# spaceml-org/STARCOP

Measured on AMD Instinct MI355X. Metric: 512x512 hyperspectral tiles/sec (train fwd+bwd), higher is better.
Workload: dtype f32; 1 GPU; configs[1]: HyperSTARCOP U-Net (smp.Unet mobilenet_v2, 4ch mag1c+RGB) train step fwd+loss+bwd+Adam, 512x512 tiles, fp32 HIP kernels (3x3 convs: fp32 operands split exactly into 16-bit terms on the matrix cores, fp32 accumulation; see config.precision and DESIGN.md section 2); batch_per_gpu=16, global_batch=16, parallelism=dp1, hipgraph=False, precision=fp32

## Files before the change

### include/starcop_hip.h

```cpp
#ifndef STARCOP_HIP_H
#define STARCOP_HIP_H

#include <stddef.h>
#include <stdint.h>

#ifdef __cplusplus
extern "C" {
#endif

typedef void* sc_stream;

enum sc_status {
  SC_OK = 0,
  SC_ERR_ARG = -1,
  SC_ERR_LAUNCH = -2,
  SC_ERR_NOTPD = -3,
  SC_ERR_NODEV = -4
};

enum sc_src_mode {
  SC_SRC_RAW = 0,
  SC_SRC_AFFINE = 1,
  SC_SRC_BNBWD = 2,
  SC_SRC_NORM = 3
// ... 18 lines not shown
const char* sc_last_error(void);
int sc_version(void);
int sc_device_check(void);

int sc_pack_weights(const float* w_oihw, float* wpk, int Cout, int Cin, int ks,
                    int co_t, int transpose_flip, sc_stream stream);
size_t sc_packed_weight_floats(int Cout, int Cin, int ks, int co_t, int transpose_flip);

typedef struct sc_pack_desc {
  const float* w; float* wpk;
  int32_t Cout, Cin, ks, co_t, transpose_flip, bx3;
  uint64_t total;
} sc_pack_desc;
size_t sc_pack_work_items(int Cout, int Cin, int ks, int co_t, int transpose_flip, int bx3);
int sc_pack_weights_batch(const sc_pack_desc* descs_dev, const uint32_t* block_starts_dev, int n, uint32_t total_blocks,
                          sc_stream stream);

typedef struct sc_bnr_args {
  const float* y;
  const float* cst;
  int32_t act;
  float* rows;
  float* absmax;
} sc_bnr_args;
#define SC_TERMS_F16X2 4
typedef struct sc_conv_args {
  sc_src src[2];
  int32_t nsrc;
  const float* wpk;
  int32_t N, H, W;
  int32_t Cout;
  int32_t ks;
  int32_t co_t;
  float* out0; float* out1;
  int32_t csplit;
  int32_t accum0, accum1;
  const float* add0;
  const float* add1;
  float* stats;
  int32_t terms;
  int32_t down0;
  const float* absmax;
  const float* xbound[2];
  const sc_bnr_args* bnr;
} sc_conv_args;
int sc_conv2d_mfma(const sc_conv_args* a, sc_stream stream);
int sc_pw_stream_variant(const sc_conv_args* a);
int sc_conv1x1_ksplit(const sc_conv_args* a, sc_stream stream);

int sc_pack_weights_bx3(const float* w_oihw, float* wpk, int Cout, int Cin, int co_t, int transpose_flip, int terms,
                        sc_stream stream);
size_t sc_packed_weight_floats_bx3(int Cout, int Cin, int co_t, int transpose_flip, int terms);
int sc_conv3x3_bx3(const sc_conv_args* a, sc_stream stream);

typedef struct sc_wgrad_args {
  sc_src dy;
  sc_src src[2];
  int32_t nsrc;
  int32_t N, H, W, Cout, Cin, ks;
  float* part; size_t part_floats;
  float* dw;
  int32_t terms;
  const float* absmax;
  const float* xbound[2];
} sc_wgrad_args;
size_t sc_wgrad_workspace_floats(int N, int H, int W, int Cout, int Cin, int ks);
int sc_conv2d_wgrad_mfma(const sc_wgrad_args* a, sc_stream stream);
typedef struct sc_wgrad_pending {
  const float* part; float* dw;
  int32_t nparts, taps, Cout, Cin, CoP, CiP;
  uint64_t total;
} sc_wgrad_pending;
int sc_conv2d_wgrad_mfma_deferred(const sc_wgrad_args* a, sc_wgrad_pending* pending_host, sc_stream stream);
int sc_wgrad_reduce_batch(const sc_wgrad_pending* descs_dev, const uint32_t* block_starts_dev, int n, uint32_t total_blocks,
                          sc_stream stream);
#define SC_PACK_THIN16 5
#define SC_PACK_PW3 6
size_t sc_packed_weight_floats_thin16(int Cout, int Cin, int transpose_flip);
int sc_pack_weights_thin16(const float* w_oihw, float* wpk, int Cout, int Cin, int transpose_flip, sc_stream stream);
int sc_conv3x3_thin16(const sc_conv_args* a, sc_stream stream);

#define SC_PACK_SP 7
size_t sc_packed_weight_floats_sp(int Cout, int Cup, int Cskip);
int sc_pack_weights_sp(const float* w_oihw, float* wpk, int Cout, int Cup, int Cskip, int terms, sc_stream stream);
int sc_sp_stat_rows(int N, int H, int W, int Cout);
int sc_conv3x3_sp(const sc_conv_args* a, sc_stream stream);
#define SC_PACK_SPD 8
size_t sc_packed_weight_floats_spd(int Cout, int Cup, int Cskip_tiles );
int sc_spd_vskip_ok(int Cup, int Cskip);
int sc_pack_weights_spd(const float* w_oihw, float* wpk, int Cout, int CinTotal, int Cup, int vskip, int terms, sc_stream stream);
int sc_conv3x3_sp_dgrad(const sc_conv_args* a, sc_stream stream);
size_t sc_sp_wgrad_workspace_bytes(int N, int H, int W, int Cout, int Cup);
int sc_conv3x3_sp_wgrad(const sc_wgrad_args* a, void* ws, size_t ws_bytes, sc_stream stream);
int sc_wgrad_scatter_cols(const float* src, float* dw, int Cout, int Ccols, int CinTotal, int col_off, sc_stream stream);
int sc_sp_variant(const sc_conv_args* a);
int sc_spd_variant(const sc_conv_args* a);
int sc_sp_wgrad_variant(const sc_wgrad_args* a);

size_t sc_wgrad_thin16_workspace_floats(int N, int H, int W, int Cout, int Cin);
int sc_conv3x3_wgrad_thin16(const sc_wgrad_args* a, sc_stream stream);

size_t sc_packed_weight_floats_pw3(int Cout, int Cin, int transpose_flip);
int sc_conv1x1_pw3(const sc_conv_args* a, sc_stream stream);
int sc_conv1x1_pw3_variant(int N, int H, int W, int Cout);
size_t sc_wgrad_pw3_workspace_floats(int N, int H, int W, int Cout, int Cin);
int sc_conv1x1_wgrad_pw3(const sc_wgrad_args* a, sc_wgrad_pending* pending_host, sc_stream stream);
int sc_wgrad_pw3_variant(int N, int H, int W, int Cout, int Cin);

typedef struct sc_irb_args {
  sc_src x;
  const float* wpk_expand;
  const float* cst_expand;
  const float* w_dw;
  const float* cst_dw;
  const float* wpk_project;
  const float* cst_project;
  float* out;
  float* z_absmax;
  int32_t N, Cin, hidden, Cout, H, W, stride, residual;
} sc_irb_args;
int sc_irb_supported(int Cin, int hidden, int Cout, int H, int W, int stride);
int sc_irb_variant(int Cin, int hidden, int Cout, int stride);
int sc_irb_eval(const sc_irb_args* a, sc_stream stream);

typedef struct sc_irt_args {
  sc_src x;
  const float* w_expand;
  const float* w_dw;
  const float* cst_expand;
  int32_t N, Cin, hidden, H, W, stride;
} sc_irt_args;
int sc_irt_supported(int Cin, int hidden, int H, int W, int stride);
int sc_irt_rows(int stage, int N, int H, int W, int stride);
int sc_irt_bwd_rows(int N, int hidden, int H, int W);
size_t sc_irt_bwd_workspace_floats(int N, int Cin, int hidden, int H, int W);
#define SC_IRT_GEO_FIELDS 14
int sc_irt_geometry(int N, int Cin, int hidden, int H, int W, int stride, int* out);
int sc_irt_expand_stats(const sc_irt_args* a, float* stats , sc_stream stream);
int sc_irt_fwd(const sc_irt_args* a, float* d_out , float* stats_d , sc_stream stream);
int sc_irt_bwd(const sc_irt_args* a, const sc_src* dy_d, double* e_sums , double* dw_acc ,
               float* work, sc_stream stream);
int sc_irt_xmoments(const sc_irt_args* a, float* work, sc_stream stream);
int sc_irt_bwd_fix(const sc_irt_args* a, const float* cst_bwd_expand, float* work, float* dx, const float* add0, int accum,
                   sc_stream stream);
int sc_irt_wgrad_finalize(const sc_irt_args* a, const float* cst_bwd_expand, float* work, float* dw_expand, sc_stream stream);

size_t sc_wgrad_bx3_workspace_floats(int N, int H, int W, int Cout, int Cin);
int sc_conv3x3_wgrad_bx3(const sc_wgrad_args* a, sc_stream stream);

int sc_conv3_variant(const sc_conv_args* a);
int sc_thin16_variant(const sc_conv_args* a);
int sc_wgrad3_variant(const sc_wgrad_args* a);
int sc_wgrad_thin16_variant(const sc_wgrad_args* a);

int sc_dwconv3x3_fwd(const sc_src* in, const float* w , float* out,
                     int N, int C, int Hin, int Win, int stride, float* stats ,
                     sc_stream stream);
typedef struct sc_bn_tail {
  const float* gamma; const float* beta;
  float* running_mean; float* running_var;
  float momentum, eps;
  float* cst;
  float* act_bound;
  uint32_t* tickets;
} sc_bn_tail;
int sc_dwconv3x3_fwd_bn(const sc_src* in, const float* w, float* out, int N, int C, int Hin, int Win, int stride, float* stats,
                        const sc_bn_tail* bn, sc_stream stream);
int sc_dwconv3x3_dgrad(const sc_src* dy, const float* w, float* dx, int accum,
                       int N, int C, int Hin, int Win, int stride, sc_stream stream);
int sc_dwconv3x3_wgrad(const sc_src* dy, const sc_src* in, double* dw_acc ,
                       int N, int C, int Hin, int Win, int stride, sc_stream stream);
int sc_dwconv3x3_bwd_fused(const sc_src* dy, const sc_src* in, const float* w, float* dx, double* dw_acc, double* in_sums,
                           int N, int C, int Hin, int Win, int stride, sc_stream stream);
int sc_dw_variant(int op, int N, int C, int Hin, int Win, int stride, int aligned16);
int sc_cast_f64_f32(const double* in, float* out, size_t n, sc_stream stream);
typedef struct sc_cast_desc { const double* in; float* out; uint64_t n; } sc_cast_desc;
int sc_cast_f64_f32_batch(const sc_cast_desc* descs_dev, int n_descs, sc_stream stream);

int sc_stem_conv_fwd(const sc_src* in, const float* w , float* out,
                     int N, int Cin, int Hin, int Win, float* stats ,
                     sc_stream stream);
enum sc_stem_kernel { SC_STEM_K_MFMA4 = 0, SC_STEM_K_VALU4 = 1, SC_STEM_K_VALU8 = 2, SC_STEM_K_VALU16 = 3 };
int sc_stem_fwd_kernel(int Cin, int Win, int out_aligned16);
int sc_stem_wgrad_njb(int Cin);
int sc_stem_wgrad_rows(int N, int Hin, int Win);
size_t sc_stem_wgrad_workspace_floats(int N, int Cin, int Hin, int Win);
int sc_stem_conv_wgrad(const sc_src* dy, const sc_src* in, float* part, size_t part_floats,
                       float* dw, int N, int Cin, int Hin, int Win, sc_stream stream);

int sc_head_conv_fwd(const sc_src* in, const float* w , const float* bias,
                     float* out, int N, int Cin, int H, int W, sc_stream stream);
enum sc_head_kernel { SC_HEAD_K_GENERIC = 0, SC_HEAD_K_FWD16 = 1, SC_HEAD_K_FWD16V = 2 };
int sc_head_fwd_kernel(int Cin, int W, int in_aligned16, int out_aligned16);
int sc_head_conv_fwd_k(const sc_src* in, const float* w , const float* bias ,
                       float* logits , uint8_t* classes ,
                       int N, int Cin, int K, int H, int W, sc_stream stream);
int sc_head_conv_dgrad(const float* dlogits, const float* w, float* gin,
                       int N, int Cin, int H, int W, sc_stream stream);
size_t sc_head_wgrad_workspace_floats(int N, int Cin, int H, int W);
int sc_head_conv_wgrad(const float* dlogits, const sc_src* in, float* part, size_t part_floats,
                       float* dw, float* dbias, int N, int Cin, int H, int W, sc_stream stream);
int sc_head_bwd_bn_rows(int N, int H, int W);
int sc_head_conv_bwd(const float* dlogits, const sc_src* in, const float* w, float* gin, float* part, size_t part_floats,
                     float* dw, float* dbias, int N, int Cin, int H, int W, double* bn_sums, float* bn_absmax, sc_stream stream);

int sc_stat_rows(int kind, int N, int H, int W);
#define SC_BN_FINALIZE_SCRATCH_DOUBLES(C) (64 * 2 * (size_t)(C))
int sc_bn_finalize(const float* stats, int nrows, double count, const float* gamma, const float* beta,
                   float* running_mean, float* running_var, float momentum, float eps,
                   int training, float* cst_fwd, int C, double* scratch, float* act_bound, sc_stream stream);
int sc_bn_bwd_reduce(const float* g, const float* y, const float* cst_fwd, int act,
                     double* sums, int N, int C, int HW, float* absmax, float* act_absmax, sc_stream stream);
int sc_bn_bwd_finalize(const double* sums, int nrows, double count, const float* cst_fwd,
                       float* dgamma, float* dbeta, float* cst_bwd, int C, sc_stream stream);
int sc_bn_bwd_finalize_rows32(const float* rows, int nrows, double count, const float* cst_fwd,
                       float* dgamma, float* dbeta, float* cst_bwd, int C, double* scratch , sc_stream stream);
int sc_bn_bwd_small(const float* g, const float* y, const float* cst_fwd, int act, int N, int C, int HW,
                    float* dgamma, float* dbeta, float* cst_bwd, float* absmax, float* act_absmax, sc_stream stream);
int sc_add_srcs(const sc_src* a, const sc_src* b, float* out, int N, int C, int HW, sc_stream stream);
int sc_stream_wait_stream(sc_stream waiter, sc_stream signaller);

int sc_add_srcs_absmax(const sc_src* a, const sc_src* b, float* out, int N, int C, int HW, float* absmax, sc_stream stream);
int sc_downsum2x2(const float* in, float* out, int accum, int N, int C, int Hout, int Wout,
                  sc_stream stream);
int sc_maxpool2x2(const sc_src* in, float* out, int N, int C, int Hout, int Wout, sc_stream stream);
int sc_upsample_bilinear2x(const sc_src* in, float* out, int N, int C, int Hin, int Win, sc_stream stream);
int sc_maxpool2x2_bwd(const sc_src* in, const float* gpool, float* gin, int accum, int N, int C, int Hout, int Wout,
                      sc_stream stream);
int sc_upsample_bilinear2x_bwd(const float* gout, float* gin, int N, int C, int Hin, int Win, sc_stream stream);
int sc_fill_f64(double* p, double v, size_t n, sc_stream stream);
int sc_apply_src(const sc_src* a, float* out, int N, int C, int HW, sc_stream stream);

int sc_bce_logits_weighted(const float* logits, const float* target, const float* weight,
                           float pos_weight, size_t n, double* loss_sum, float* dlogits,
                           float* loss_px, sc_stream stream);

int sc_adam_step(float* param, const float* grad, float* exp_avg, float* exp_avg_sq, size_t n,
                 float lr, float beta1, float beta2, float eps, float weight_decay,
                 float bias_correction1, float bias_correction2_sqrt, float grad_scale,
                 const float* hp_dev ,
                 sc_stream stream);
int sc_adam_prepare(int64_t* step, const float* lr_dev, float beta1, float beta2, float* hp_dev,
                    sc_stream stream);

int sc_threshold_masks(const float* logits, const float* target, int ge0, float* prediction,
                       int64_t* pred_binary, int64_t* differences, int64_t* tile_count,
                       int N, int HW, sc_stream stream);
int sc_pred_classification(const int64_t* tile_count, int64_t* cls, int N, int H, int W,
                           sc_stream stream);

typedef struct sc_mag1c_args {
  const void* x;
  int32_t x_is_f64;
  const int64_t* xoff;
  const int32_t* P;
  const int32_t* Ppad;
  const int64_t* poff;
  const uint8_t* statmask;
  int32_t G, S;
  int64_t npix;
  const double* templ;
  int32_t num_iter;
  double alpha;
  double cov_update_scaling;
  int32_t albedo_override, zero_override, sparse_override, apply_scaling;
// ... 504 lines not shown
```

### starcop_amd/_lib.py

```python
import ctypes as C
import os
import subprocess

import torch

_HERE = os.path.dirname(os.path.abspath(__file__))
LIB_PATH = os.path.join(_HERE, "libstarcop_hip.so")
CSRC = os.path.join(_HERE, "csrc")

SC_CST = 8
STAT_CONV3, STAT_CONV1, STAT_DW, STAT_STEM, STAT_BNBWD, STAT_CONV1K, STAT_PW3 = 0, 1, 2, 3, 4, 5, 6

SRC_RAW, SRC_AFFINE, SRC_BNBWD, SRC_NORM = 0, 1, 2, 3
ACT_NONE, ACT_RELU, ACT_RELU6 = 0, 1, 2


class StarcopHipError(RuntimeError):
    pass


class sc_src(C.Structure):
    _fields_ = [("x", C.c_void_p), ("aux", C.c_void_p), ("cst", C.c_void_p),
                ("C", C.c_int32), ("mode", C.c_int32), ("act", C.c_int32), ("up", C.c_int32)]

# ... 398 lines not shown
    "sc_dw_variant": (_i, [_i, _i, _i, _i, _i, _i, _i]),
    "sc_wgrad_thin16_workspace_floats": (_sz, [_i, _i, _i, _i, _i]),
    "sc_conv3x3_wgrad_thin16": (_i, [C.POINTER(sc_wgrad_args), _vp]),
    "sc_conv2d_wgrad_mfma_deferred": (_i, [C.POINTER(sc_wgrad_args), C.POINTER(sc_wgrad_pending), _vp]),
    "sc_wgrad_reduce_batch": (_i, [_vp, _vp, _i, C.c_uint32, _vp]),
    "sc_packed_weight_floats_pw3": (_sz, [_i, _i, _i]),
    "sc_conv1x1_pw3": (_i, [C.POINTER(sc_conv_args), _vp]),
    "sc_conv1x1_pw3_variant": (_i, [_i, _i, _i, _i]),
    "sc_wgrad_pw3_workspace_floats": (_sz, [_i, _i, _i, _i, _i]),
    "sc_wgrad_pw3_variant": (_i, [_i, _i, _i, _i, _i]),
    "sc_conv1x1_wgrad_pw3": (_i, [C.POINTER(sc_wgrad_args), C.POINTER(sc_wgrad_pending), _vp]),
    "sc_irb_supported": (_i, [_i, _i, _i, _i, _i, _i]),
    "sc_irb_variant": (_i, [_i, _i, _i, _i]),
    "sc_irb_eval": (_i, [C.POINTER(sc_irb_args), _vp]),
    "sc_irt_supported": (_i, [_i, _i, _i, _i, _i]),
    "sc_irt_rows": (_i, [_i, _i, _i, _i, _i]),
    "sc_irt_bwd_rows": (_i, [_i, _i, _i, _i]),
    "sc_irt_bwd_workspace_floats": (_sz, [_i, _i, _i, _i, _i]),
    "sc_irt_geometry": (_i, [_i, _i, _i, _i, _i, _i, C.POINTER(_i)]),
    "sc_irt_expand_stats": (_i, [C.POINTER(sc_irt_args), _vp, _vp]),
    "sc_irt_fwd": (_i, [C.POINTER(sc_irt_args), _vp, _vp, _vp]),
    "sc_irt_bwd": (_i, [C.POINTER(sc_irt_args), C.POINTER(sc_src), _vp, _vp, _vp, _vp]),
    "sc_irt_xmoments": (_i, [C.POINTER(sc_irt_args), _vp, _vp]),
    "sc_irt_bwd_fix": (_i, [C.POINTER(sc_irt_args), _vp, _vp, _vp, _vp, _i, _vp]),
    "sc_irt_wgrad_finalize": (_i, [C.POINTER(sc_irt_args), _vp, _vp, _vp, _vp]),
    "sc_maxpool2x2": (_i, [C.POINTER(sc_src), _vp, _i, _i, _i, _i, _vp]),
    "sc_upsample_bilinear2x": (_i, [C.POINTER(sc_src), _vp, _i, _i, _i, _i, _vp]),
    "sc_maxpool2x2_bwd": (_i, [C.POINTER(sc_src), _vp, _vp, _i, _i, _i, _i, _i, _vp]),
    "sc_upsample_bilinear2x_bwd": (_i, [_vp, _vp, _i, _i, _i, _i, _vp]),
    "sc_pwreg_param_floats": (_sz, [_i, _i, _i, _i]),
    "sc_pwreg_fwd": (_i, [_vp, _vp, _i, _i, _i, _i, _i, _i, _i, _vp, _vp]),
    "sc_reg_loss": (_i, [_vp, _vp, _sz, _i, _vp, _vp, _vp, _vp]),
    "sc_pwreg_sweep_blocks": (_i, [_i, _i, _i]),
    "sc_pwreg_train_sweep": (_i, [_vp, _vp, _vp, _i, _i, _i, _i, _i, _i, _i, _i, _vp, _vp]),
    "sc_pwreg_finalize": (_i, [_vp, _i, _vp, _i, _i, _i, _i, _d, _vp, _vp, _vp]),
    "sc_panel_minmax": (_i, [_vp, C.POINTER(sc_panel), _i, _vp, _vp]),
    "sc_render_panels": (_i, [_vp, C.POINTER(sc_panel), _i, _vp, _vp, _i, _i, _vp]),
    "sc_component_stats_workspace_bytes": (_sz, [_i, _i, _i, _i, _i]),
    "sc_component_stats": (_i, [C.POINTER(sc_cstats_args), _vp, _sz, _vp]),
    "sc_component_outlines_workspace_bytes": (_sz, [_i, _i, C.c_int64]),
    "sc_component_outlines_rounds": (_i, [C.c_int64]),
    "sc_component_outlines": (_i, [C.POINTER(sc_outline_args), _i, _vp]),
    "sc_rasterize_polygons": (_i, [C.POINTER(sc_rast_args), _vp]),
    "sc_overview_reduce": (_i, [C.POINTER(sc_overview_args), _vp]),
    "sc_tiff_tile_flags": (_i, [C.POINTER(sc_cog_image), _i, _vp, _vp]),
    "sc_tiff_pack_tiles": (_i, [C.POINTER(sc_tiff_pack_args), _vp]),
    "sc_edt_workspace_bytes": (_sz, [_i, _i, _i]),
    "sc_edt": (_i, [C.POINTER(sc_edt_args), _vp, _sz, _vp]),
    "sc_edt_call_workspace_bytes": (_sz, [C.POINTER(sc_edt_args)]),
    "sc_edt_variant": (_i, [_i, _i, _i, _i]),
    "sc_label_keep": (_i, [_vp, _vp, _vp, _i, _i, _i, _i, _vp]),
    "sc_tiff_lzw_decode": (_i, [_vp, _sz, _vp, _sz, C.POINTER(C.c_size_t)]),
    "sc_tiff_unpredict": (_i, [_vp, _i, _i, _i, _i, _i, _i, _vp]),
}
REG_L1, REG_MSE, PWREG_G_FROM_MEMORY = 0, 1, 2
PWREG_MAXC, PWREG_PART_DOUBLES, REG_LOSS_PARTS = 16, 273, 256
PACK_SPD = 8
PACK_SP = 7
PACK_PW3 = 6
PACK_THIN16 = 5
TERMS_F16X2 = 4
SE_CROSS = 0xBA

_lib = None


def build(force=False):
    if force:
        subprocess.run(["make", "-C", CSRC, "clean"], check=True, stdout=subprocess.DEVNULL)
    r = subprocess.run(["make", "-C", CSRC, "-j", "4"], capture_output=True, text=True)
    if r.returncode != 0:
        raise StarcopHipError("building libstarcop_hip.so failed:\n" + r.stdout[-4000:] + r.stderr[-4000:])
    return LIB_PATH


def load():
    global _lib
    if _lib is not None:
        return _lib
    path = os.environ.get("STARCOP_HIP_LIB", LIB_PATH)
    if not os.path.exists(path):
        raise StarcopHipError(
            f"{LIB_PATH} is missing: run `python -c 'import __graft_entry__ as g; g.build()'` "
            "(or `make -C starcop_amd/csrc`).  starcop_amd has no CPU/torch fallback.")
    lib = C.CDLL(path)
    for name, (res, args) in SIGNATURES.items():
        fn = getattr(lib, name)
        fn.restype = res
        fn.argtypes = args
    _lib = lib
    return lib


_EXC = {-1: ValueError, -2: RuntimeError, -3: torch.linalg.LinAlgError, -4: RuntimeError}


def check(rc):
    if rc != 0:
        msg = load().sc_last_error().decode("utf-8", "replace")
        raise _EXC.get(rc, StarcopHipError)(f"libstarcop_hip: {msg} (status {rc})")


_device_ok = {}


def require_device(t=None):
# ... 58 lines not shown
```

### starcop_amd/csrc/conv_bx3.hip

```cpp
#include "sc_split.h"
#include "conv_sp_pack.h"
#include <cstdlib>
#include <type_traits>


namespace {

struct ConvXP {
  SrcD s0, s1;
  const uintx4* wpk;
  int N, H, W, Cout;
  float* out0; float* out1;
  int csplit, accum0, accum1;
  const float* add0; const float* add1;
  float* stats;
  int down0;
  const float* absmax;
  const float* xb0; const float* xb1;
  int xcdmap;
  const float* bnr_y; const float* bnr_cst; float* bnr_rows; float* bnr_absmax; int bnr_act;
};

static inline void set_bnr(ConvXP& p, const sc_bnr_args* b) {
  p.bnr_y = b ? b->y : nullptr; p.bnr_cst = b ? b->cst : nullptr; p.bnr_rows = b ? b->rows : nullptr;
  p.bnr_absmax = b ? b->absmax : nullptr; p.bnr_act = b ? b->act : SC_ACT_NONE;
}

__device__ __forceinline__ void wave_absmax_to(float mx, float* slot) {
#pragma unroll
  for (int o = 32; o > 0; o >>= 1) mx = fmaxf(mx, __shfl_xor(mx, o, 64));
  if ((threadIdx.x & 63) == 0 && mx > __builtin_nontemporal_load(slot)) atomicMax(reinterpret_cast<unsigned*>(slot), __builtin_bit_cast(unsigned, mx));
}

template <int Q, bool HF>
__device__ __forceinline__ void bx3_epilogue_bnr(const ConvXP& p, const floatx16 (&acc)[2][Q], float hinv, int n, int cot, int ty, int tx, int y0,
                                                 int x0, int tiles_x, int wave, int l31, int lhi, int tid, float (&s_red)[4][32 * Q][2]) {
  constexpr int CO_T = 32 * Q;
  const int H = p.H, W = p.W, Cs = p.csplit, c0 = cot * CO_T;
  const int ox = x0 + l31;
  const float blo = sc_act_lo(p.bnr_act), bhi = sc_act_hi(p.bnr_act);
  const float* const bc = p.bnr_cst + (size_t)c0 * SC_CST;
  float mx = 0.f;
  if (p.down0) {
    const unsigned hq32 = (unsigned)((H >> 1) * (W >> 1));
    const size_t cbase = ((size_t)n * Cs + c0) * hq32;
    float* const ob = p.out0 + cbase;
    const float* const yb = p.bnr_y + cbase;
    const int oy = y0 + 2 * wave;
    const bool st = !(l31 & 1) && oy < H && ox < W;
    const unsigned loff = (unsigned)(4 * lhi) * hq32 + (unsigned)(st ? (oy >> 1) * (W >> 1) + (ox >> 1) : 0);
#pragma unroll
    for (int q = 0; q < Q; ++q) {
      float yv[16];
#pragma unroll
      for (int r = 0; r < 16; ++r) {
        const int cu = q * 32 + (r & 3) + 8 * (r >> 2);
        yv[r] = (st && c0 + cu + 4 * lhi < Cs) ? yb[loff + (unsigned)cu * hq32] : 0.f;
      }
#pragma unroll
      for (int r = 0; r < 16; ++r) {
        const int cu = q * 32 + (r & 3) + 8 * (r >> 2);
        const int col = cu + 4 * lhi;
        const bool okc = c0 + col < Cs;
        float v = ((oy < H) && (ox < W)) ? acc[0][q][r] : 0.f;
        v += ((oy + 1 < H) && (ox < W)) ? acc[1][q][r] : 0.f;
        if (HF) v *= hinv;
        v += __builtin_bit_cast(float, __builtin_amdgcn_update_dpp(0, __builtin_bit_cast(int, v), 0xB1, 0xF, 0xF, false));
        const bool ok = st && okc;
        if (ok) ob[loff + (unsigned)cu * hq32] = v;
        const float4 cc = *reinterpret_cast<const float4*>(bc + (size_t)(okc ? col : 0) * SC_CST);
        const float yh = fmaf(yv[r], cc.x, cc.y);
        const float gq = (ok && yh > blo && yh < bhi) ? v : 0.f;
// ... 62 lines not shown
    if (co < Cs && t4 < rows4) {
      const size_t row = ((size_t)n * rows4 + t4) * tiles_x + tx;
      p.bnr_rows[(row * Cs + co) * 2 + k] = s_red[2 * hh][col][k] + s_red[2 * hh + 1][col][k];
    }
  }
}

template <int Q, bool BNB, int NT, bool HF = false>
__global__ __launch_bounds__(256, Q == 2 ? 2 : 3) void k_conv3_bx3(const ConvXP p) {
  static_assert(!HF || NT == 2, "the fp16 mode has two terms");
  constexpr int PR = 10, PC = 34, NPX = PR * PC;
  constexpr bool PAD = (Q == 2);
  constexpr int NPXP = PAD ? 384 : NPX;
  constexpr int CO_T = 32 * Q;
  constexpr int WENT = 6 * NT * CO_T;
  constexpr int NWV = (WENT + 255) / 256;
  constexpr int WENTP = PAD ? NWV * 256 : WENT;
  constexpr int NR = 3;
  constexpr bool W2 = (NT != 3) && !(Q == 1 && BNB);

  __shared__ uintx4 s_p[NT][2][NPXP];
  __shared__ uintx4 s_w[2][WENTP];
  __shared__ float s_red[4][CO_T][2];

  const int tid = threadIdx.x;
  const int lane = tid & 63, wave = tid >> 6;
  const int l31 = lane & 31, lhi = lane >> 5;
  const int H = p.H, W = p.W;
  const int tiles_x = (W + 31) >> 5;
  int n, cot, tile;
  if (p.xcdmap) {
    const int ncot = (p.Cout + CO_T - 1) / CO_T;
    const int per_img = tiles_x * ((H + 7) >> 3);
    const int slot = blockIdx.x >> 3, xcd = blockIdx.x & 7;
    int pt;
    if (p.xcdmap == 3) {
      const int total = per_img * p.N;
      if (ncot >= 8) {
        const int mine = (ncot - xcd + 7) >> 3;
        const int k = slot / total;
        if (k >= mine) return;
        cot = xcd + 8 * k; pt = slot - k * total;
      } else {
        const int g = 8 / ncot;
        const int per = (total + g - 1) / g;
        cot = xcd / g; pt = (xcd - cot * g) * per + slot;
        if (slot >= per || pt >= total) return;
      }
      n = pt / per_img; tile = pt - n * per_img;
    } else {
    if (p.xcdmap == 2) {
      const int total = per_img * p.N, per_xcd = (total + 7) >> 3;
      const int j = slot / ncot;
      pt = xcd * per_xcd + j;
      if (j >= per_xcd || pt >= total) return;
    } else {
      pt = (slot / ncot) * 8 + xcd;
      if (pt >= per_img * p.N) return;
    }
    cot = slot % ncot;
    n = pt / per_img; tile = pt - n * per_img;
    }
  } else {
    n = blockIdx.z; cot = blockIdx.y; tile = blockIdx.x;
  }
  n = __builtin_amdgcn_readfirstlane(n); cot = __builtin_amdgcn_readfirstlane(cot); tile = __builtin_amdgcn_readfirstlane(tile);
  const int ty = __builtin_amdgcn_readfirstlane(tile / tiles_x), tx = tile - ty * tiles_x;
  const int y0 = ty * 8, x0 = tx * 32;
  const int C0 = p.s0.C;
  const int Cin = C0 + p.s1.C;
  const int nk = (Cin + 15) >> 4;
  const uintx4* wbase = p.wpk + (size_t)cot * nk * 3 * WENT;

  const float hsx = !HF ? 1.f : (BNB ? h_grad_scale(p.absmax) : h_act_scale(p.xb0, p.xb1));
  const float hinv = !HF ? 1.f : 1.f / (hsx * SC_H_SW);

  floatx16 acc[2][Q];
#pragma unroll
  for (int pp = 0; pp < 2; ++pp)
#pragma unroll
    for (int q = 0; q < Q; ++q)
#pragma unroll
      for (int r = 0; r < 16; ++r) acc[pp][q][r] = 0.f;

  const int hw = __builtin_amdgcn_readfirstlane(wave >> 1);
  const int sidx = tid & 127;
  unsigned off0[NR], off1[NR];
  unsigned inb = 0;
  {
    const int up0 = p.s0.up, up1 = p.s1.up;
    const int Ws0 = W >> up0, Ws1 = W >> up1;
#pragma unroll
    for (int r = 0; r < NR; ++r) {
      const int e = sidx + 128 * r;
      const int pr = e / PC, pc = e - pr * PC;
      const int y = y0 - 1 + pr, x = x0 - 1 + pc;
      const bool ok = (e < NPX) && (y >= 0) && (y < H) && (x >= 0) && (x < W);
      off0[r] = ok ? (unsigned)((y >> up0) * Ws0 + (x >> up0)) : 0u;
      off1[r] = ok ? (unsigned)((y >> up1) * Ws1 + (x >> up1)) : 0u;
      inb |= ok ? (1u << r) : 0u;
    }
  }
  float xv[NR][8], av[BNB ? NR : 1][8];
  uintx4 wvA[NWV], wvB[W2 ? NWV : 1];
  const float* xb = nullptr; const float* ab = nullptr; const float* cb = nullptr;
  size_t plane = 0; int nch = 0; bool second = false;
  float slo = 0.f, shi = 0.f;
// ... 410 lines not shown
      }
    }
  }
}

template <int Q, bool BNB>
__global__ __launch_bounds__(512, 4) void k_conv3_ws(const ConvXP p) {
  constexpr int NT = 2;
  constexpr bool HF = true;
  constexpr int PR = 10, PC = 34, NPX = PR * PC;
  constexpr int NPXP = NPX;
  constexpr int CO_T = 32 * Q;
  constexpr int WENT = 6 * NT * CO_T;
  constexpr int NWV = (WENT + 255) / 256;
  constexpr int WENTP = NWV * 256;
  constexpr int NR = 3;

  __shared__ uintx4 s_p[2][NT][2][NPXP];
  __shared__ uintx4 s_w[2][WENTP];
  __shared__ float s_red[4][CO_T][2];
  constexpr int WS_BNB_MAXC = 256;
  __shared__ __attribute__((aligned(16))) float s_cst[BNB ? WS_BNB_MAXC * SC_CST : 4];

  const int role = __builtin_amdgcn_readfirstlane((int)threadIdx.x >> 8);
  const int tid = threadIdx.x & 255;
  const int lane = tid & 63, wave = tid >> 6;
  const int l31 = lane & 31, lhi = lane >> 5;
  const int H = p.H, W = p.W;
  const int tiles_x = (W + 31) >> 5;
  int n, cot, tile;
  if (p.xcdmap) {
    const int ncot = (p.Cout + CO_T - 1) / CO_T;
    const int per_img = tiles_x * ((H + 7) >> 3);
    const int slot = blockIdx.x >> 3, xcd = blockIdx.x & 7;
    int pt;
    if (p.xcdmap == 3) {
      const int total = per_img * p.N;
      if (ncot >= 8) {
        const int mine = (ncot - xcd + 7) >> 3;
        const int k = slot / total;
        if (k >= mine) return;
        cot = xcd + 8 * k; pt = slot - k * total;
      } else {
        const int g = 8 / ncot;
        const int per = (total + g - 1) / g;
        cot = xcd / g; pt = (xcd - cot * g) * per + slot;
        if (slot >= per || pt >= total) return;
      }
      n = pt / per_img; tile = pt - n * per_img;
    } else {
    if (p.xcdmap == 2) {
      const int total = per_img * p.N, per_xcd = (total + 7) >> 3;
      const int j = slot / ncot;
      pt = xcd * per_xcd + j;
      if (j >= per_xcd || pt >= total) return;
    } else {
      pt = (slot / ncot) * 8 + xcd;
      if (pt >= per_img * p.N) return;
    }
    cot = slot % ncot;
    n = pt / per_img; tile = pt - n * per_img;
    }
  } else {
    n = blockIdx.z; cot = blockIdx.y; tile = blockIdx.x;
  }
  n = __builtin_amdgcn_readfirstlane(n); cot = __builtin_amdgcn_readfirstlane(cot); tile = __builtin_amdgcn_readfirstlane(tile);
  const int ty = __builtin_amdgcn_readfirstlane(tile / tiles_x), tx = tile - ty * tiles_x;
  const int y0 = ty * 8, x0 = tx * 32;
  const int C0 = p.s0.C;
  const int Cin = C0 + p.s1.C;
  const int nk = (Cin + 15) >> 4;
  const uintx4* wbase = p.wpk + (size_t)cot * nk * 3 * WENT;

  const float hsx = !HF ? 1.f : (BNB ? h_grad_scale(p.absmax) : h_act_scale(p.xb0, p.xb1));
  const float hinv = !HF ? 1.f : 1.f / (hsx * SC_H_SW);

  const int nst = 3 * nk;
  const bool want_stats = p.stats != nullptr;
  if constexpr (BNB) {
    for (int i = (int)threadIdx.x; i < p.s0.C * SC_CST; i += 512) {
      const int f = i & (SC_CST - 1);
      s_cst[i] = p.s0.cst[i] * ((HF && f >= 2 && f <= 4) ? hsx : 1.f);
    }
    __syncthreads();
  }
  if (role == 1) {
  const int hw = __builtin_amdgcn_readfirstlane(wave >> 1);
  const int sidx = tid & 127;
  unsigned off0[NR], off1[NR];
  unsigned inb = 0;
  {
    const int up0 = p.s0.up, up1 = p.s1.up;
    const int Ws0 = W >> up0, Ws1 = W >> up1;
#pragma unroll
    for (int r = 0; r < NR; ++r) {
      const int e = sidx + 128 * r;
      const int pr = e / PC, pc = e - pr * PC;
      const int y = y0 - 1 + pr, x = x0 - 1 + pc;
      const bool ok = (e < NPX) && (y >= 0) && (y < H) && (x >= 0) && (x < W);
      off0[r] = ok ? (unsigned)((y >> up0) * Ws0 + (x >> up0)) : 0u;
      off1[r] = ok ? (unsigned)((y >> up1) * Ws1 + (x >> up1)) : 0u;
      inb |= ok ? (1u << r) : 0u;
    }
  }
  float xv[NR][8], av[BNB ? NR : 1][8];
  uintx4 wr[3][NWV];
  struct Chunk { const float* xb; const float* ab; const float* cb; size_t plane; int nch, cbase; bool second, raw; float slo, shi; };
// ... 306 lines not shown
    }
  }

  if (want_stats) {
    __syncthreads();
    const int rows4 = (H + 3) >> 2;
    for (int i = tid; i < 2 * CO_T * 2; i += 256) {
      const int hh = i / (CO_T * 2), rem = i - hh * (CO_T * 2);
      const int col = rem >> 1, k = rem & 1;
      const int co = cot * CO_T + col;
      const int t4 = 2 * ty + hh;
      if (co < p.Cout && t4 < rows4) {
        const float t = s_red[2 * hh][col][k] + s_red[2 * hh + 1][col][k];
        const size_t row = ((size_t)n * rows4 + t4) * tiles_x + tx;
        p.stats[(row * p.Cout + co) * 2 + k] = t;
      }
    }
  }
}

__device__ __forceinline__ void split_filter(float v, bool half, unsigned short (&t)[3]) {
  if (half) {
    const float vs = __builtin_amdgcn_fmed3f(v * SC_H_SW, -SC_H_MAX, SC_H_MAX);
    const _Float16 h0 = (_Float16)vs;
    const _Float16 h1 = (_Float16)(vs - (float)h0);
    t[0] = __builtin_bit_cast(unsigned short, h0); t[1] = __builtin_bit_cast(unsigned short, h1); t[2] = 0;
    return;
  }
  const __bf16 t0 = (__bf16)v;
  float rr = v - (float)t0;
  const __bf16 t1 = (__bf16)rr;
  rr -= (float)t1;
  const __bf16 t2 = (__bf16)rr;
  t[0] = __builtin_bit_cast(unsigned short, t0); t[1] = __builtin_bit_cast(unsigned short, t1); t[2] = __builtin_bit_cast(unsigned short, t2);
}

template <int CIN, bool BNB, bool UPS = false>
__global__ __launch_bounds__(256, 2) void k_conv3_thin_h(const ConvXP p) {
  constexpr int TW = CIN == 16 ? 64 : 32, PBW = TW / 16, NPB = 2 * PBW;
  constexpr int PR = UPS ? 6 : 10, PC = UPS ? TW / 2 + 2 : TW + 2, NPX = PR * PC;
  constexpr int NH = CIN / 8;
  constexpr int NG = 9 * NH, NS = (NG + 3) / 4;
  constexpr int NPXP = (NPX + 15) & ~15;
  __shared__ uintx4 s_p[2][NH][NPXP];
  __shared__ float s_red[4][TW / 32][16][2];

  const int tid = threadIdx.x, lane = tid & 63, wave = tid >> 6;
  const int l15 = lane & 15, lg = lane >> 4;
  const int H = p.H, W = p.W;
  const int tiles_x = (W + TW - 1) / TW;
  int n, tile;
  if (p.xcdmap) {
    const int per_img = tiles_x * ((H + 7) >> 3), total = per_img * p.N, per_xcd = (total + 7) >> 3;
    const int j = blockIdx.x >> 3, pt = (blockIdx.x & 7) * per_xcd + j;
    if (j >= per_xcd || pt >= total) return;
    n = pt / per_img; tile = pt - n * per_img;
  } else {
    n = blockIdx.z; tile = blockIdx.x;
  }
  n = __builtin_amdgcn_readfirstlane(n); tile = __builtin_amdgcn_readfirstlane(tile);
  const int ty = __builtin_amdgcn_readfirstlane(tile / tiles_x), tx = tile - ty * tiles_x;
  const int y0 = ty * 8, x0 = tx * TW;
  const float hsx = BNB ? h_grad_scale(p.absmax) : h_act_scale(p.xb0, p.xb1);
  const float hinv = 1.f / (hsx * SC_H_SW);

  const SrcD& src = p.s0;
  uintx4 A[NS][2];
#pragma unroll
  for (int s = 0; s < NS; ++s)
#pragma unroll
    for (int t = 0; t < 2; ++t) A[s][t] = p.wpk[(s * 2 + t) * 64 + lane];

  constexpr int WPG = 4 / NH, TPG = 64 * WPG, NR = (NPX + TPG - 1) / TPG;
  const int grp = __builtin_amdgcn_readfirstlane(wave / WPG);
  const int g8 = grp * 8;
  const int e0 = tid - grp * TPG;
  const int up = UPS ? 1 : src.up;
  const int Ws = W >> up;
  const size_t plane = (size_t)(H >> up) * Ws;
  const float slo = BNB ? sc_act_lo(src.act) : h_lo(sc_act_lo(src.act), hsx), shi = BNB ? sc_act_hi(src.act) : h_hi(sc_act_hi(src.act), hsx);
  float xv[NR][8], av[BNB ? NR : 1][8];
  bool okv[NR];
  const float* const xg = src.x + ((size_t)n * CIN + g8) * plane;
  const float* const ag = BNB ? src.aux + ((size_t)n * CIN + g8) * plane : nullptr;
#pragma unroll
  for (int r = 0; r < NR; ++r) {
    const int e = e0 + TPG * r;
    const int pr = e / PC, pc = e - pr * PC;
    const int y = UPS ? (y0 >> 1) - 1 + pr : y0 - 1 + pr, x = UPS ? (x0 >> 1) - 1 + pc : x0 - 1 + pc;
    const bool ok = UPS ? ((e < NPX) && y >= 0 && y < (H >> 1) && x >= 0 && x < Ws) : ((e < NPX) && y >= 0 && y < H && x >= 0 && x < W);
    okv[r] = ok;
    const unsigned off = ok ? (UPS ? (unsigned)(y * Ws + x) : (unsigned)((y >> up) * Ws + (x >> up))) : 0u;
#pragma unroll
    for (int j = 0; j < 8; ++j) {
      xv[r][j] = xg[(size_t)j * plane + off];
      if (BNB) av[r][j] = ag[(size_t)j * plane + off];
    }
  }
  __builtin_amdgcn_sched_barrier(0);
  float4 cc[8]; float c4[8];
#pragma unroll
  for (int j = 0; j < 8; ++j) { cc[j] = make_float4(BNB ? 1.f : hsx, 0.f, 0.f, 0.f); c4[j] = 0.f; }
  if (src.mode != SC_SRC_RAW) {
#pragma unroll
    for (int j = 0; j < 8; ++j) {
      cc[j] = *reinterpret_cast<const float4*>(src.cst + (size_t)(g8 + j) * SC_CST);
      if (BNB) c4[j] = src.cst[(size_t)(g8 + j) * SC_CST + 4];
// ... 106 lines not shown
        }
      }
      return;
    }
  }
#pragma unroll
  for (int r = 0; r < 4; ++r) {
    const int co = 4 * lg + r;
    float sv[TW / 32], sq[TW / 32];
#pragma unroll
    for (int h = 0; h < TW / 32; ++h) { sv[h] = 0.f; sq[h] = 0.f; }
#pragma unroll
    for (int pb = 0; pb < NPB; ++pb) {
      const int oy = y0 + 2 * wave + pb / PBW, ox = x0 + 16 * (pb % PBW) + l15;
      const bool ok = oy < H && ox < W && co < p.Cout;
      const float v = ok ? acc[pb][r] * hinv : 0.f;
      sv[(pb % PBW) >> 1] += v; sq[(pb % PBW) >> 1] = fmaf(v, v, sq[(pb % PBW) >> 1]);
      if (ok) *reinterpret_cast<float*>(reinterpret_cast<char*>(outn) + ((unsigned)co * HWu + (unsigned)(oy * W + ox)) * 4u) = v;
    }
    if (want_stats) {
#pragma unroll
      for (int h = 0; h < TW / 32; ++h) {
#pragma unroll
        for (int o = 8; o > 0; o >>= 1) { sv[h] += __shfl_xor(sv[h], o, 64); sq[h] += __shfl_xor(sq[h], o, 64); }
        if (l15 == 0) { s_red[wave][h][co][0] = sv[h]; s_red[wave][h][co][1] = sq[h]; }
      }
    }
  }
  if (want_stats) {
    __syncthreads();
    const int rows4 = (H + 3) >> 2, tiles32 = (W + 31) >> 5;
    if (tid < 2 * (TW / 32) * 16 * 2) {
      const int hh = tid / ((TW / 32) * 32), h = (tid >> 5) % (TW / 32), col = (tid >> 1) & 15, k = tid & 1;
      const int t4 = 2 * ty + hh, t32 = tx * (TW / 32) + h;
      if (col < p.Cout && t4 < rows4 && t32 < tiles32) {
        const size_t row = ((size_t)n * rows4 + t4) * tiles32 + t32;
        p.stats[(row * p.Cout + col) * 2 + k] = s_red[2 * hh][h][col][k] + s_red[2 * hh + 1][h][col][k];
      }
    }
  }
}

__global__ __launch_bounds__(256, 2) void k_conv3_thin_sp(const ConvXP p) {
  constexpr int PC = 34, NPX = 6 * PC, NPXP = (NPX + 15) & ~15, NH = 4, NR = (NPX + 63) / 64, STEPS3 = 9;
  __shared__ uintx4 s_p[2][NH][NPXP];
  __shared__ float s_red[4][2][16][2];
  const int tid = threadIdx.x, lane = tid & 63, wave = tid >> 6;
  const int l15 = lane & 15, lg = lane >> 4;
  const int H = p.H, W = p.W, Hs = H >> 1, Ws = W >> 1;
  const int tiles_x = (W + 63) >> 6;
  int n, tile;
  if (p.xcdmap) {
    const int per_img = tiles_x * ((H + 7) >> 3), total = per_img * p.N, per_xcd = (total + 7) >> 3;
    const int j = blockIdx.x >> 3, pt = (blockIdx.x & 7) * per_xcd + j;
    if (j >= per_xcd || pt >= total) return;
    n = pt / per_img; tile = pt - n * per_img;
  } else {
    n = blockIdx.z; tile = blockIdx.x;
  }
  n = __builtin_amdgcn_readfirstlane(n); tile = __builtin_amdgcn_readfirstlane(tile);
  const int ty = __builtin_amdgcn_readfirstlane(tile / tiles_x), tx = tile - ty * tiles_x;
  const int y0 = ty * 8, x0 = tx * 64;
  const float hsx = h_act_scale(p.xb0, p.xb1);
  const float hinv = 1.f / (hsx * SC_H_SW);
  const SrcD& src = p.s0;

  const int g8 = wave * 8;
  const size_t plane = (size_t)Hs * Ws;
  const float slo = h_lo(sc_act_lo(src.act), hsx), shi = h_hi(sc_act_hi(src.act), hsx);
  float xv[NR][8];
  bool okv[NR];
  const float* const xg = src.x + ((size_t)n * 32 + g8) * plane;
#pragma unroll
  for (int r = 0; r < NR; ++r) {
    const int e = lane + 64 * r;
    const int pr = e / PC, pc = e - pr * PC;
    const int y = (y0 >> 1) - 1 + pr, x = (x0 >> 1) - 1 + pc;
    const bool ok = (e < NPX) && y >= 0 && y < Hs && x >= 0 && x < Ws;
    okv[r] = ok;
    const unsigned off = ok ? (unsigned)(y * Ws + x) : 0u;
#pragma unroll
    for (int j = 0; j < 8; ++j) xv[r][j] = xg[(size_t)j * plane + off];
  }
  __builtin_amdgcn_sched_barrier(0);
  float2 cc[8];
#pragma unroll
  for (int j = 0; j < 8; ++j) cc[j] = make_float2(hsx, 0.f);
  if (src.mode != SC_SRC_RAW) {
#pragma unroll
    for (int j = 0; j < 8; ++j) {
      cc[j] = *reinterpret_cast<const float2*>(src.cst + (size_t)(g8 + j) * SC_CST);
      cc[j].x *= hsx; cc[j].y *= hsx;
    }
  }
#pragma unroll
  for (int r = 0; r < NR; ++r) {
    const int e = lane + 64 * r;
    uintx4 t0, t1;
#pragma unroll
    for (int jp = 0; jp < 4; ++jp) {
      const float v0 = okv[r] ? sc_pro_affine_h(xv[r][2 * jp], cc[2 * jp].x, cc[2 * jp].y, slo, shi) : 0.f;
      const float v1 = okv[r] ? sc_pro_affine_h(xv[r][2 * jp + 1], cc[2 * jp + 1].x, cc[2 * jp + 1].y, slo, shi) : 0.f;
      unsigned a0, a1;
      split2h<false>(v0, v1, a0, a1);
      t0[jp] = a0; t1[jp] = a1;
    }
    if (e < NPX) { s_p[0][wave][e] = t0; s_p[1][wave][e] = t1; }
// ... 37 lines not shown
        }
      }

  const size_t HWs = (size_t)H * W;
  const bool want_stats = p.stats != nullptr;
  float* const outn = p.out0 + (size_t)n * p.Cout * HWs;
  const unsigned HWu = (unsigned)HWs;
#pragma unroll
  for (int r = 0; r < 4; ++r) {
    const int co = 4 * lg + r;
#pragma unroll
    for (int q = 0; q < 2; ++q) {
      float sv = 0.f, sq = 0.f;
      const int ox = x0 + 32 * q + 2 * l15;
#pragma unroll
      for (int py = 0; py < 2; ++py) {
        const int oy = y0 + 2 * wave + py;
        const bool ok = oy < H && ox < W && co < p.Cout;
        const float v0 = ok ? acc[q][2 * py][r] * hinv : 0.f, v1 = ok ? acc[q][2 * py + 1][r] * hinv : 0.f;
        sv += v0 + v1; sq = fmaf(v0, v0, fmaf(v1, v1, sq));
        if (ok) *reinterpret_cast<float2*>(reinterpret_cast<char*>(outn) + ((unsigned)co * HWu + (unsigned)(oy * W + ox)) * 4u) = make_float2(v0, v1);
      }
      if (want_stats) {
        sv = row_sum16(sv); sq = row_sum16(sq);
        if (l15 == 0) { s_red[wave][q][co][0] = sv; s_red[wave][q][co][1] = sq; }
      }
    }
  }
  if (want_stats) {
    __syncthreads();
    const int rows4 = (H + 3) >> 2, tiles32 = (W + 31) >> 5;
    if (tid < 2 * 2 * 16 * 2) {
      const int hh = tid / 64, h = (tid >> 5) & 1, col = (tid >> 1) & 15, k = tid & 1;
      const int t4 = 2 * ty + hh, t32 = 2 * tx + h;
      if (col < p.Cout && t4 < rows4 && t32 < tiles32) {
        const size_t row = ((size_t)n * rows4 + t4) * tiles32 + t32;
        p.stats[(row * p.Cout + col) * 2 + k] = s_red[2 * hh][h][col][k] + s_red[2 * hh + 1][h][col][k];
      }
    }
  }
}

__global__ __launch_bounds__(256, 2) void k_conv3_thin_spd(const ConvXP p) {
  constexpr int PR = 10, PC = 66, NPX = PR * PC, PCH = 34, NPL = PR * PCH, NPLP = (NPL + 15) & ~15;
  constexpr int TPG = 128, NR = (NPX + TPG - 1) / TPG;
  __shared__ uintx4 s_p[2][2][2][NPLP];
  const int tid = threadIdx.x, lane = tid & 63, wave = tid >> 6;
  const int l15 = lane & 15, lg = lane >> 4;
  const int H = p.H, W = p.W, Hs = H >> 1, Ws = W >> 1;
  const int tiles_x = (W + 63) >> 6;
  int n, tile;
  if (p.xcdmap) {
    const int per_img = tiles_x * ((H + 7) >> 3), total = per_img * p.N, per_xcd = (total + 7) >> 3;
    const int j = blockIdx.x >> 3, pt = (blockIdx.x & 7) * per_xcd + j;
    if (j >= per_xcd || pt >= total) return;
    n = pt / per_img; tile = pt - n * per_img;
  } else {
    n = blockIdx.z; tile = blockIdx.x;
  }
  n = __builtin_amdgcn_readfirstlane(n); tile = __builtin_amdgcn_readfirstlane(tile);
  const int ty = __builtin_amdgcn_readfirstlane(tile / tiles_x), tx = tile - ty * tiles_x;
  const int y0 = ty * 8, x0 = tx * 64;
  const float hsx = h_grad_scale(p.absmax);
  const float hinv = 1.f / (hsx * SC_H_SW);
  const SrcD& src = p.s0;

  const int grp = __builtin_amdgcn_readfirstlane(wave >> 1);
  const int g8 = grp * 8;
  const int e0 = tid - grp * TPG;
  const size_t plane = (size_t)H * W;
  const float slo = sc_act_lo(src.act), shi = sc_act_hi(src.act);
  float xv[NR][8], av[NR][8];
  bool okv[NR];
  const float* const xg = src.x + ((size_t)n * 16 + g8) * plane;
  const float* const ag = src.aux + ((size_t)n * 16 + g8) * plane;
#pragma unroll
  for (int r = 0; r < NR; ++r) {
    const int e = e0 + TPG * r;
    const int pr = e / PC, pc = e - pr * PC;
    const int y = y0 - 1 + pr, x = x0 - 1 + pc;
    const bool ok = (e < NPX) && y >= 0 && y < H && x >= 0 && x < W;
    okv[r] = ok;
    const unsigned off = ok ? (unsigned)(y * W + x) : 0u;
#pragma unroll
    for (int j = 0; j < 8; ++j) { xv[r][j] = xg[(size_t)j * plane + off]; av[r][j] = ag[(size_t)j * plane + off]; }
  }
  __builtin_amdgcn_sched_barrier(0);
  float4 cc[8]; float c4[8];
#pragma unroll
  for (int j = 0; j < 8; ++j) {
    cc[j] = *reinterpret_cast<const float4*>(src.cst + (size_t)(g8 + j) * SC_CST);
    c4[j] = src.cst[(size_t)(g8 + j) * SC_CST + 4];
  }
#pragma unroll
  for (int r = 0; r < NR; ++r) {
    const int e = e0 + TPG * r;
    const int pr = e / PC, pc = e - pr * PC;
    uintx4 t0, t1;
#pragma unroll
    for (int jp = 0; jp < 4; ++jp) {
      float v[2];
#pragma unroll
      for (int h = 0; h < 2; ++h) {
        const int j = 2 * jp + h;
        const float t = sc_pro_bnbwd(xv[r][j], av[r][j], cc[j].x, cc[j].y, cc[j].z, cc[j].w, c4[j], slo, shi);
        v[h] = okv[r] ? t * hsx : 0.f;
      }
// ... 907 lines not shown
  const int blocks = (int)((total + 255) / 256 > 4096 ? 4096 : (total + 255) / 256);
  hipLaunchKernelGGL(k_pack_weights_bx3, dim3(blocks), dim3(256), 0, (hipStream_t)stream, w,
                     reinterpret_cast<unsigned short*>(wpk), Cout, Cin, co_t, transpose_flip, nchunk,
                     terms == SC_TERMS_F16X2 ? 2 : terms, terms == SC_TERMS_F16X2 ? 1 : 0, total);
  SC_LAUNCH_OK("sc_pack_weights_bx3");
  return SC_OK;
}

static int conv3_bx3_check(const sc_conv_args* a) {
  SC_REQUIRE(a != nullptr, "sc_conv3x3_bx3: null args");
  SC_REQUIRE(a->ks == 3, "sc_conv3x3_bx3: ks must be 3 (got %d)", a->ks);
  SC_REQUIRE(a->co_t == 32 || a->co_t == 64, "sc_conv3x3_bx3: co_t must be 32 or 64 (got %d)", a->co_t);
  SC_REQUIRE(a->nsrc == 1 || a->nsrc == 2, "sc_conv3x3_bx3: nsrc must be 1 or 2");
  const int C0 = a->src[0].C, C1 = a->nsrc == 2 ? a->src[1].C : 0;
  SC_REQUIRE(C0 > 0 && C1 >= 0 && (a->nsrc == 1 || (C0 % 16 == 0 && C1 > 0)),
             "sc_conv3x3_bx3: a concat needs the first source's channels to be a multiple of 16 (got %d,%d)", C0, C1);
  SC_REQUIRE(a->N > 0 && a->H > 0 && a->W > 0 && a->Cout > 0, "sc_conv3x3_bx3: bad shape");
  SC_REQUIRE(a->csplit > 0 && a->csplit <= a->Cout, "sc_conv3x3_bx3: bad csplit");
  SC_REQUIRE(a->csplit == a->Cout || (a->add0 == nullptr && a->add1 == nullptr), "sc_conv3x3_bx3: add tensors need a single output");
  SC_REQUIRE(((uintptr_t)a->wpk & 15) == 0, "sc_conv3x3_bx3: packed filters must be 16-byte aligned");
  for (int s = 0; s < a->nsrc; ++s) {
    SC_REQUIRE(a->src[s].up == 0 || (a->H % 2 == 0 && a->W % 2 == 0), "sc_conv3x3_bx3: upsampled source needs even H,W");
    SC_REQUIRE(a->src[s].up == 0 || a->src[s].up == 1, "sc_conv3x3_bx3: up must be 0 or 1");
    SC_REQUIRE(a->src[s].mode == SC_SRC_RAW || a->src[s].cst != nullptr, "sc_conv3x3_bx3: source %d needs constants", s);
    SC_REQUIRE(a->src[s].mode != SC_SRC_NORM, "sc_conv3x3_bx3: NORM sources are the stem's");
    SC_REQUIRE(a->src[s].mode != SC_SRC_BNBWD || a->src[s].aux != nullptr, "sc_conv3x3_bx3: BNBWD source needs aux");
    SC_REQUIRE(a->src[s].mode != SC_SRC_BNBWD || a->nsrc == 1, "sc_conv3x3_bx3: a BNBWD source cannot be part of a concat");
  }
  SC_REQUIRE(!a->down0 || (a->H % 2 == 0 && a->W % 2 == 0 && a->stats == nullptr && a->add0 == nullptr && a->add1 == nullptr),
             "sc_conv3x3_bx3: down0 (2x2-summed half-resolution out0) needs even H, W and no stats/add tensors");
  SC_REQUIRE(a->terms >= 0 && a->terms <= 4, "sc_conv3x3_bx3: terms must be 0 (= 3), 1, 2, 3 or SC_TERMS_F16X2 (got %d)", a->terms);
  if (a->bnr) {
    SC_REQUIRE(a->src[0].mode == SC_SRC_BNBWD && a->bnr->y && a->bnr->cst && a->bnr->rows, "sc_conv3x3_bx3: bnr needs a BNBWD source and y / cst / rows");
    SC_REQUIRE(!a->accum0 && !a->add0 && !a->add1 && !a->stats, "sc_conv3x3_bx3: bnr: out0 must receive the complete gradient (no accum0 / add / stats)");
    SC_REQUIRE(a->csplit == a->Cout || a->csplit % a->co_t == 0, "sc_conv3x3_bx3: bnr: csplit must fall on a cout-tile boundary");
  }
  return SC_OK;
}

static int conv3_bx3_variant_of(const sc_conv_args* a) {
  const int C0 = a->src[0].C, C1 = a->nsrc == 2 ? a->src[1].C : 0;
  const int bnb = a->src[0].mode == SC_SRC_BNBWD ? 1 : 0;
  const int m = a->terms == SC_TERMS_F16X2 ? 4 : (a->terms == 1 || a->terms == 2 ? a->terms : 3);
  constexpr int ws_env = 1;
  static const int ws_env_min = [] { const char* e = getenv("STARCOP_BX3_WS_MINCHUNKS"); return e ? atoi(e) : 16; }();
  const int ws = (m == 4 && ws_env && (C0 + C1 + 15) / 16 >= ws_env_min && (!bnb || a->src[0].C <= 256) && !a->bnr) ? 1 : 0;
  return 1000 * ws + 100 * (a->co_t / 32) + 10 * bnb + m;
}

extern "C" int sc_conv3_variant(const sc_conv_args* a) {
  return conv3_bx3_check(a) == SC_OK ? conv3_bx3_variant_of(a) : -1;
}

extern "C" int sc_conv3x3_bx3(const sc_conv_args* a, sc_stream stream) {
  if (const int rc = conv3_bx3_check(a)) return rc;
  const int C0 = a->src[0].C, C1 = a->nsrc == 2 ? a->src[1].C : 0;
  ConvXP p;
  p.s0 = to_srcd(a->src[0]);
  p.s1 = a->nsrc == 2 ? to_srcd(a->src[1]) : empty_srcd();
  p.wpk = reinterpret_cast<const uintx4*>(a->wpk); p.N = a->N; p.H = a->H; p.W = a->W; p.Cout = a->Cout;
  p.out0 = a->out0; p.out1 = a->out1; p.csplit = a->csplit; p.accum0 = a->accum0; p.accum1 = a->accum1;
  p.add0 = a->add0; p.add1 = a->add1; p.stats = a->stats;
  p.down0 = a->down0 ? 1 : 0;
  const int co_tiles = (a->Cout + a->co_t - 1) / a->co_t;
  dim3 grid(((a->W + 31) / 32) * ((a->H + 7) / 8), co_tiles, a->N);
  constexpr int xcdmap_env = 2;
  p.xcdmap = xcdmap_env >= 2 ? 2 : ((xcdmap_env && co_tiles > 1) ? 1 : 0);
  {
    constexpr long big_env = 0L;
    const long nkc = (C0 + C1 + 15) / 16;
    const long wbytes = (long)co_tiles * nkc * 3 * 6 * (a->terms == SC_TERMS_F16X2 || a->terms == 2 ? 2 : (a->terms == 1 ? 1 : 3)) * a->co_t * 16;
    if (xcdmap_env >= 2 && big_env > 0 && wbytes > big_env && (co_tiles >= 8 || co_tiles == 1 || co_tiles == 2 || co_tiles == 4)) p.xcdmap = 3;
  }
  if (p.xcdmap == 3) {
    const long total = (long)grid.x * a->N;
    const long slots = co_tiles >= 8 ? (long)((co_tiles + 7) / 8) * total : (total + (8 / co_tiles) - 1) / (8 / co_tiles);
    SC_REQUIRE(slots * 8 < (1L << 31), "sc_conv3x3_bx3: grid too large");
    grid = dim3((unsigned)(slots * 8));
  } else if (p.xcdmap) {
    const long pt8 = ((long)grid.x * a->N + 7) / 8 * 8;
    SC_REQUIRE(pt8 * co_tiles < (1L << 31), "sc_conv3x3_bx3: grid too large");
    grid = dim3((unsigned)(pt8 * co_tiles));
  }
  hipStream_t st = (hipStream_t)stream;
  p.absmax = a->absmax; p.xb0 = a->xbound[0]; p.xb1 = a->xbound[1];
  set_bnr(p, a->bnr);
#define SC_BX3_CASE(Q, B, M, NT, HF) \
  case 100 * Q + 10 * B + M: hipLaunchKernelGGL((k_conv3_bx3<Q, B != 0, NT, HF>), grid, dim3(256), 0, st, p); break;
#define SC_BX3_CASES(M, NT, HF) SC_BX3_CASE(1, 0, M, NT, HF) SC_BX3_CASE(1, 1, M, NT, HF) SC_BX3_CASE(2, 0, M, NT, HF) SC_BX3_CASE(2, 1, M, NT, HF)
#define SC_BX3_WS_CASE(Q, B) \
  case 1000 + 100 * Q + 10 * B + 4: hipLaunchKernelGGL((k_conv3_ws<Q, B != 0>), grid, dim3(512), 0, st, p); break;
  switch (conv3_bx3_variant_of(a)) {
    SC_BX3_CASES(1, 1, false)
    SC_BX3_CASES(2, 2, false)
    SC_BX3_CASES(3, 3, false)
    SC_BX3_CASES(4, 2, true)
    SC_BX3_WS_CASE(1, 0) SC_BX3_WS_CASE(1, 1) SC_BX3_WS_CASE(2, 0) SC_BX3_WS_CASE(2, 1)
    default: SC_REQUIRE(false, "sc_conv3x3_bx3: no kernel for variant %d", conv3_bx3_variant_of(a));
  }
#undef SC_BX3_WS_CASE
#undef SC_BX3_CASES
#undef SC_BX3_CASE
  SC_LAUNCH_OK("sc_conv3x3_bx3");
  return SC_OK;
}

static bool wgrad3_pipe_reduces(const WgradXPlan& pl) {
  const int npair = pl.nci * pl.wm, cit = 32 * pl.nci, xcp = 8 * 40 + 8;
  return pl.kp == 1 || 3 * npair * 3072 <= 2 * cit * xcp / 2;
}

static size_t wgrad_bx3_workspace_of(const WgradXPlan& pl) {
  const size_t E = (size_t)9 * pl.CoP * pl.CiP;
  const int nparts = pl.nsl * pl.kp;
  return (size_t)nparts * E + sc_reduce_scratch_floats(nparts, E);
}
extern "C" size_t sc_wgrad_bx3_workspace_floats(int N, int H, int W, int Cout, int Cin) {
  const size_t a = wgrad_bx3_workspace_of(plan_wgrad_bx3(N, H, W, Cout, Cin, false));
  const size_t b = wgrad_bx3_workspace_of(plan_wgrad_bx3(N, H, W, Cout, Cin, true));
  return a > b ? a : b;
}

static int wgrad3_bx3_check(const sc_wgrad_args* a) {
  SC_REQUIRE(a != nullptr, "sc_conv3x3_wgrad_bx3: null args");
  SC_REQUIRE(a->ks == 3, "sc_conv3x3_wgrad_bx3: ks must be 3");
  SC_REQUIRE(a->nsrc == 1 || a->nsrc == 2, "sc_conv3x3_wgrad_bx3: nsrc must be 1 or 2");
// ... 141 lines not shown
  SC_REQUIRE(w && wpk && ((uintptr_t)wpk & 15) == 0, "sc_pack_weights_thin16: bad pointer");
  SC_REQUIRE(thin16_shape_ok(Cout, Cin, transpose_flip), "sc_pack_weights_thin16: needs <= 16 output and 16 or 32 input channels (got %d, %d, flip %d)",
             Cout, Cin, transpose_flip);
  const size_t total = (size_t)thin_steps(Cout, Cin, transpose_flip) * 512;
  hipLaunchKernelGGL(k_pack_weights_thin, dim3((unsigned)((total + 255) / 256)), dim3(256), 0, (hipStream_t)stream, w,
                     reinterpret_cast<unsigned short*>(wpk), Cout, Cin, transpose_flip, total);
  SC_LAUNCH_OK("sc_pack_weights_thin16");
  return SC_OK;
}

static int thin16_check(const sc_conv_args* a) {
  SC_REQUIRE(a != nullptr && a->ks == 3 && a->nsrc == 1, "sc_conv3x3_thin16: one source, ks = 3");
  const int Cin = a->src[0].C;
  const sc_src& s = a->src[0];
  if (a->down0) {
    SC_REQUIRE(Cin == 16 && a->Cout == 32 && a->csplit == 32 && s.mode == SC_SRC_BNBWD && s.aux && s.cst && s.up == 0,
               "sc_conv3x3_thin16(down0): needs a 16-channel BatchNorm-backward source and 32 output channels (got %d, %d)", Cin, a->Cout);
    SC_REQUIRE(a->H % 2 == 0 && a->W % 2 == 0 && a->N > 0 && a->N <= 65535 && a->out0 && !a->add0 && !a->add1 && !a->stats && !a->bnr && !a->out1,
               "sc_conv3x3_thin16(down0): even H, W; one output, no add / statistics / bnr epilogue");
    SC_REQUIRE(a->terms == SC_TERMS_F16X2 && ((uintptr_t)a->wpk & 15) == 0, "sc_conv3x3_thin16(down0): terms must be SC_TERMS_F16X2, filters 16-byte aligned");
    SC_REQUIRE((size_t)16 * a->H * a->W < ((size_t)1 << 30), "sc_conv3x3_thin16(down0): one image of the gradient must stay below 2^30 elements");
    return SC_OK;
  }
  SC_REQUIRE(a->Cout >= 1 && a->Cout <= 16 && (Cin == 16 || Cin == 32), "sc_conv3x3_thin16: needs <= 16 output and 16 or 32 input channels (got %d, %d)",
             a->Cout, Cin);
  SC_REQUIRE(a->N > 0 && a->N <= 65535 && a->H > 0 && a->W > 0, "sc_conv3x3_thin16: bad shape");
  SC_REQUIRE(a->csplit == a->Cout && !a->accum0 && !a->add0 && !a->add1 && !a->down0 && a->out0,
             "sc_conv3x3_thin16: a single plain output only (no split / add / accumulate / down-sum epilogue)");
  SC_REQUIRE(a->terms == SC_TERMS_F16X2, "sc_conv3x3_thin16: terms must be SC_TERMS_F16X2");
  SC_REQUIRE(((uintptr_t)a->wpk & 15) == 0, "sc_conv3x3_thin16: packed filters must be 16-byte aligned");
  SC_REQUIRE(s.up == 0 || (s.up == 1 && a->H % 2 == 0 && a->W % 2 == 0), "sc_conv3x3_thin16: upsampled source needs even H, W");
  SC_REQUIRE(s.mode == SC_SRC_RAW || s.cst != nullptr, "sc_conv3x3_thin16: source needs constants");
  SC_REQUIRE(s.mode != SC_SRC_NORM && (s.mode != SC_SRC_BNBWD || s.aux != nullptr), "sc_conv3x3_thin16: unsupported source");
  SC_REQUIRE((size_t)a->Cout * a->H * a->W < ((size_t)1 << 30), "sc_conv3x3_thin16: one image of the output must stay below 2^30 elements");
  SC_REQUIRE(!a->bnr || (s.mode == SC_SRC_BNBWD && a->bnr->y && a->bnr->cst && a->bnr->rows && !a->stats),
             "sc_conv3x3_thin16: bnr needs a BNBWD source, y / cst / rows and no stats");
  return SC_OK;
}

static int thin16_variant_of(const sc_conv_args* a) {
  const sc_src& s = a->src[0];
  if (a->down0) return 2110;
  static const bool sp_off = [] { const char* e = getenv("STARCOP_THIN_SP"); return e && atoi(e) == 0; }();
  static const bool ups_off = [] { const char* e = getenv("STARCOP_THIN_UPS"); return e && atoi(e) == 0; }();
  const bool bnb = s.mode == SC_SRC_BNBWD;
  if (s.C == 32 && s.up == 1 && !bnb && !sp_off) return 1200;
  return 100 * (s.C / 16) + 10 * (bnb ? 1 : 0) + (s.C == 32 && s.up == 1 && !bnb && !ups_off ? 1 : 0);
}

extern "C" int sc_thin16_variant(const sc_conv_args* a) {
  return thin16_check(a) == SC_OK ? thin16_variant_of(a) : -1;
}

extern "C" int sc_conv3x3_thin16(const sc_conv_args* a, sc_stream stream) {
  if (const int rc = thin16_check(a)) return rc;
  const int Cin = a->src[0].C;
  const sc_src& s = a->src[0];
  const int variant = thin16_variant_of(a);
  if (variant == 2110) {
    ConvXP p{};
    p.s0 = to_srcd(s); p.s1 = empty_srcd();
    p.wpk = reinterpret_cast<const uintx4*>(a->wpk); p.N = a->N; p.H = a->H; p.W = a->W; p.Cout = a->Cout;
    p.out0 = a->out0; p.csplit = a->Cout; p.accum0 = a->accum0; p.absmax = a->absmax;
    set_bnr(p, nullptr);
    const long total = (long)((a->W + 63) / 64) * ((a->H + 7) / 8) * a->N, per_xcd = (total + 7) / 8;
    p.xcdmap = 2;
    hipLaunchKernelGGL(k_conv3_thin_spd, dim3((unsigned)(per_xcd * 8)), dim3(256), 0, (hipStream_t)stream, p);
    SC_LAUNCH_OK("sc_conv3x3_thin16(down0)");
    return SC_OK;
  }
  ConvXP p{};
  p.s0 = to_srcd(s); p.s1 = empty_srcd();
  p.wpk = reinterpret_cast<const uintx4*>(a->wpk); p.N = a->N; p.H = a->H; p.W = a->W; p.Cout = a->Cout;
  p.out0 = a->out0; p.csplit = a->Cout; p.stats = a->stats; p.absmax = a->absmax; p.xb0 = a->xbound[0]; p.xb1 = a->xbound[1];
  set_bnr(p, a->bnr);
  const int tw = (Cin == 16 || variant == 1200) ? 64 : 32;
  dim3 grid(((a->W + tw - 1) / tw) * ((a->H + 7) / 8), 1, a->N);
  constexpr int xcdmap_env = 2;
  p.xcdmap = xcdmap_env ? 2 : 0;
  if (p.xcdmap) {
    const long total = (long)grid.x * a->N, per_xcd = (total + 7) / 8;
    grid = dim3((unsigned)(per_xcd * 8));
  }
  hipStream_t st = (hipStream_t)stream;
  switch (variant) {
    case 1200: hipLaunchKernelGGL(k_conv3_thin_sp, grid, dim3(256), 0, st, p); break;
    case 100: hipLaunchKernelGGL((k_conv3_thin_h<16, false>), grid, dim3(256), 0, st, p); break;
    case 110: hipLaunchKernelGGL((k_conv3_thin_h<16, true>), grid, dim3(256), 0, st, p); break;
    case 201: hipLaunchKernelGGL((k_conv3_thin_h<32, false, true>), grid, dim3(256), 0, st, p); break;
    case 200: hipLaunchKernelGGL((k_conv3_thin_h<32, false>), grid, dim3(256), 0, st, p); break;
    case 210: hipLaunchKernelGGL((k_conv3_thin_h<32, true>), grid, dim3(256), 0, st, p); break;
    default: SC_REQUIRE(false, "sc_conv3x3_thin16: no kernel for variant %d", variant);
  }
  SC_LAUNCH_OK("sc_conv3x3_thin16");
  return SC_OK;
}

extern "C" size_t sc_pack_work_items(int Cout, int Cin, int ks, int co_t, int transpose_flip, int bx3) {
  if (bx3 == SC_PACK_THIN16) return (size_t)thin_steps(Cout, Cin, transpose_flip) * 512;
  if (bx3 == SC_PACK_SPD) return spd_pack_items(Cout, co_t, (transpose_flip & 3) == 3 ? Cin - co_t : 0);
  if (bx3 == SC_PACK_SP) return sp_pack_items(Cout, co_t, Cin - co_t);
  if (bx3 == SC_PACK_PW3) {
    const int M = transpose_flip ? Cin : Cout, K = transpose_flip ? Cout : Cin;
    return (size_t)(((M + 31) / 32 + 3) / 4 * 4) * ((K + 15) / 16) * 512;
  }
  if (bx3) {
    const int M = transpose_flip ? Cin : Cout, K = transpose_flip ? Cout : Cin;
    return (size_t)((M + co_t - 1) / co_t) * ((K + 15) / 16) * 9 * 2 * co_t * 8;
  }
  return sc_packed_weight_floats(Cout, Cin, ks, co_t, transpose_flip);
}

extern "C" int sc_pack_weights_batch(const sc_pack_desc* descs_dev, const uint32_t* block_starts_dev, int n, uint32_t total_blocks,
                                     sc_stream stream) {
  SC_REQUIRE(descs_dev && block_starts_dev && n > 0 && total_blocks > 0, "sc_pack_weights_batch: bad argument");
  hipLaunchKernelGGL(k_pack_batch, dim3(total_blocks), dim3(256), 0, (hipStream_t)stream,
                     reinterpret_cast<const PackDesc*>(descs_dev), block_starts_dev, n);
  SC_LAUNCH_OK("sc_pack_weights_batch");
  return SC_OK;
}
```

### starcop_amd/csrc/conv_sp.hip

```cpp
#include "sc_split.h"
#include "conv_sp_pack.h"
#include <cstdlib>
#include <type_traits>

namespace {

#ifndef SP_INTERLEAVE
#define SP_INTERLEAVE 4
#endif

struct ConvSPP {
  SrcD s0, s1;
  const uintx4* wpk;
  int N, Hl, Wl, Cout;
  float* out;
  float* stats;
  const float* xb0; const float* xb1;
};

constexpr int SP_SMEM_W = 2 * SP_WST * 16;
#ifndef SP_PC16
#define SP_PC16 18
#endif
template <int TW> constexpr int sp_pc() { return TW == 16 ? SP_PC16 : TW + 2; }
template <int TW> constexpr int sp_npx() { return (256 / TW + 2) * sp_pc<TW>(); }
template <int TW> constexpr int sp_smem_bytes() { return SP_SMEM_W + 2 * 2 * 2 * sp_npx<TW>() * 16 + 8 * 32 * 2 * 4; }

template <int TW, bool BF, int NPP = 2>
__global__ __launch_bounds__(512, 2) void k_conv3_sp(const ConvSPP p) {
  static_assert(NPP == 1 || NPP == 2, "one or two pixel groups per wave");
  constexpr int NT = BF ? 1 : 2;
  constexpr int NM = BF ? 4 : 12;
  constexpr int TH = 128 * NPP / TW;
  constexpr int PC = sp_pc<TW>(), NPX = sp_npx<TW>();
  constexpr int NPXU = (TH + 2) * PC;
  constexpr int NR = (NPXU + 127) / 128;
  constexpr int WST = SP_WST / 2 * NT;
  constexpr int NWV = WST / 512;
  static_assert(NPXU <= NPX && NPXU <= 128 * NR, "staging rounds of 128 threads per channel quarter");

  extern __shared__ __attribute__((aligned(16))) unsigned char smem[];
  uintx4* const s_w = reinterpret_cast<uintx4*>(smem);
  uintx4* const s_p = reinterpret_cast<uintx4*>(smem + SP_SMEM_W);
  float* const s_red = reinterpret_cast<float*>(smem + SP_SMEM_W + 2 * NT * 2 * NPX * 16);

  const int tid = threadIdx.x;
  const int lane = tid & 63, wave = __builtin_amdgcn_readfirstlane(tid >> 6);
  const int l31 = lane & 31, lhi = lane >> 5;
  const int py = wave >> 2, wq = wave & 3;
  const int Hl = p.Hl, Wl = p.Wl;
  const int tiles_x = (Wl + TW - 1) / TW, tiles_y = (Hl + TH - 1) / TH;
  const int ncot = (p.Cout + 31) >> 5;
  int n, cot, tile;
  {
    const int per_img = tiles_x * tiles_y;
    const int total = per_img * p.N, per_xcd = (total + 7) >> 3;
    const int slot = blockIdx.x >> 3, xcd = blockIdx.x & 7;
    const int j = slot / ncot;
    const int pt = xcd * per_xcd + j;
    if (j >= per_xcd || pt >= total) return;
    cot = slot - j * ncot;
    n = pt / per_img; tile = pt - n * per_img;
  }
  n = __builtin_amdgcn_readfirstlane(n); cot = __builtin_amdgcn_readfirstlane(cot); tile = __builtin_amdgcn_readfirstlane(tile);
  const int ty = __builtin_amdgcn_readfirstlane(tile / tiles_x), tx = tile - ty * tiles_x;
  const int y0 = ty * TH, x0 = tx * TW;
  const int C0 = p.s0.C, C1 = p.s1.C;
  const int nku = (C0 + 15) >> 4, nkt = nku + 4 * ((C1 + 15) >> 4);
  const uintx4* wbase = p.wpk + (size_t)cot * nkt * WST;

  const float hsx = BF ? 1.f : h_act_scale(p.xb0, p.xb1);
  const float hinv = BF ? 1.f : 1.f / (hsx * SP_SW);

  floatx16 acc[NPP][2];
#pragma unroll
  for (int i = 0; i < 2 * NPP; ++i)
#pragma unroll
    for (int r = 0; r < 16; ++r) acc[i >> 1][i & 1][r] = 0.f;

  const int q4 = __builtin_amdgcn_readfirstlane(tid >> 7);
  const int hw = q4 >> 1, sub = q4 & 1;
  const int sidx = tid & 127;
  unsigned pyx[NR];
#pragma unroll
  for (int r = 0; r < NR; ++r) {
    const int e = sidx + 128 * r;
    const int pr = e / PC, pc = e - pr * PC;
    const int y = y0 - 1 + pr, x = x0 - 1 + pc;
    const bool ok = (e < NPXU) && (y >= 0) && (y < Hl) && (x >= 0) && (x < Wl);
    pyx[r] = ok ? ((unsigned)y << 16) | (unsigned)x : 0xFFFFFFFFu;
  }
  float xv[NR][4];
  uintx4 wv[NWV];
  float cs0[4], cs1[4];
  float slo = 0.f, shi = 0.f;
  int nch = 0;

  auto request = [&](int kc) __attribute__((always_inline)) {
    const uintx4* wsrc = wbase + (size_t)kc * WST;
#pragma unroll
    for (int j = 0; j < NWV; ++j) wv[j] = wsrc[tid + 512 * j];
    const bool second = kc >= nku;
    const int c4 = kc - nku;
    const SrcD& s = second ? p.s1 : p.s0;
    const int cbase = (second ? (c4 >> 2) : kc) * 16 + hw * 8 + sub * 4;
    const size_t plane = second ? (size_t)4 * Hl * Wl : (size_t)Hl * Wl;
    const unsigned qoff = second ? (unsigned)(((c4 >> 1) & 1) * 2 * Wl + (c4 & 1)) : 0u;
    nch = s.C - cbase;
    const int cb0 = nch > 0 ? cbase : 0;
    const float* xb = s.x + ((size_t)n * s.C + cb0) * plane;
    const int jmax = nch > 0 ? nch - 1 : 0;
#pragma unroll
// ... 149 lines not shown
#pragma unroll
  for (int pp = 0; pp < NPP; ++pp) {
    const int g = NPP * wq + pp;
    const int i = y0 + (TW == 32 ? g : 2 * g + (l31 >> 4)), j = x0 + (TW == 32 ? l31 : (l31 & 15));
    okp[pp] = i < Hl && j < Wl;
    loff[pp] = (unsigned)(4 * lhi) * hw32 + (unsigned)(okp[pp] ? (2 * i + py) * W + 2 * j : 0);
  }
#pragma unroll
  for (int r = 0; r < 16; ++r) {
    const int cu = (r & 3) + 8 * (r >> 2);
    const int col = cu + 4 * lhi;
    const bool okc = cot * 32 + col < p.Cout;
    float sv = 0.f, sq = 0.f;
#pragma unroll
    for (int pp = 0; pp < NPP; ++pp) {
      floatx2 v = {acc[pp][0][r] * hinv, acc[pp][1][r] * hinv};
      if (okp[pp] && okc) *reinterpret_cast<floatx2*>(ob + loff[pp] + (unsigned)cu * hw32) = v;
      else v = floatx2{0.f, 0.f};
      sv += v[0] + v[1];
      sq = fmaf(v[0], v[0], fmaf(v[1], v[1], sq));
    }
    if (want_stats) {
      const float s = half_sum32(sv);
      const float ss = half_sum32(sq);
      if (l31 == SC_HALF_SUM_LANE) { s_red[(wave * 32 + col) * 2 + 0] = s; s_red[(wave * 32 + col) * 2 + 1] = ss; }
    }
  }
  if (want_stats) {
    __syncthreads();
    if (tid < 64) {
      const int col = tid >> 1, k = tid & 1;
      const int co = cot * 32 + col;
      if (co < p.Cout) {
        float t = 0.f;
#pragma unroll
        for (int w8 = 0; w8 < 8; ++w8) t += s_red[(w8 * 32 + col) * 2 + k];
        const size_t row = (size_t)n * (tiles_x * tiles_y) + tile;
        p.stats[(row * p.Cout + co) * 2 + k] = t;
      }
    }
  }
}

struct ConvSPD {
  SrcD dy;
  const uintx4* wpk;
  int N, Hl, Wl, Cup;
  float* out;
  int accum;
  const float* absmax;
  float* out_skip;
  int Cskip, accum_skip;
  int skip_mode, ntu, nts;
};

template <int TW, bool BF, int NPP = 2>
__global__ __launch_bounds__(512, 2) void k_conv3_spd(const ConvSPD p) {
  static_assert(NPP == 1 || NPP == 2, "one or two pixel groups per wave (see k_conv3_sp)");
  constexpr int NT = BF ? 1 : 2;
  constexpr int NM = BF ? 4 : 12;
  constexpr int TH = 128 * NPP / TW;
  constexpr int PC = sp_pc<TW>(), NPX = sp_npx<TW>();
  constexpr int NPXU = (TH + 2) * PC;
  constexpr int NR = (NPXU + 127) / 128;
  static_assert(NPXU <= NPX && (NPP == 2 || NR == 2), "staging rounds");
  constexpr int WST = SP_WST / 2 * NT;
  constexpr int NWV = WST / 512;

  extern __shared__ __attribute__((aligned(16))) unsigned char smem[];
  uintx4* const s_w = reinterpret_cast<uintx4*>(smem);
  uintx4* const s_p = reinterpret_cast<uintx4*>(smem + SP_SMEM_W);

  const int tid = threadIdx.x;
  const int lane = tid & 63, wave = __builtin_amdgcn_readfirstlane(tid >> 6);
  const int l31 = lane & 31, lhi = lane >> 5;
  const int hh = wave >> 2, wq = wave & 3;
  const int Hl = p.Hl, Wl = p.Wl;
  const int tiles_x = (Wl + TW - 1) / TW, tiles_y = (Hl + TH - 1) / TH;
  const int ncot = p.ntu + p.nts;
  int n, cot, tile;
  {
    const int per_img = tiles_x * tiles_y;
    const int total = per_img * p.N, per_xcd = (total + 7) >> 3;
    const int slot = blockIdx.x >> 3, xcd = blockIdx.x & 7;
    const int j = slot / ncot;
    const int pt = xcd * per_xcd + j;
    if (j >= per_xcd || pt >= total) return;
    cot = slot - j * ncot;
    n = pt / per_img; tile = pt - n * per_img;
  }
  n = __builtin_amdgcn_readfirstlane(n); cot = __builtin_amdgcn_readfirstlane(cot); tile = __builtin_amdgcn_readfirstlane(tile);
  const int ty = __builtin_amdgcn_readfirstlane(tile / tiles_x), tx = tile - ty * tiles_x;
  const int y0 = ty * TH, x0 = tx * TW;
  const int Co = p.dy.C;
  const int nkt = 4 * ((Co + 15) >> 4);
  const uintx4* wbase = p.wpk + (size_t)cot * nkt * WST;

  const float hsx = BF ? 1.f : h_grad_scale(p.absmax);
  const float hinv = BF ? 1.f : 1.f / (hsx * SP_SW);

  floatx16 acc[NPP][2];
#pragma unroll
  for (int i = 0; i < 2 * NPP; ++i)
#pragma unroll
    for (int r = 0; r < 16; ++r) acc[i >> 1][i & 1][r] = 0.f;

  const int q4 = __builtin_amdgcn_readfirstlane(tid >> 7);
  const int hw = q4 >> 1, sub = q4 & 1;
  const int sidx = tid & 127;
  unsigned pyx[NR];
#pragma unroll
  for (int r = 0; r < NR; ++r) {
    const int e = sidx + 128 * r;
    const int pr = e / PC, pc = e - pr * PC;
    const int y = y0 - 1 + pr, x = x0 - 1 + pc;
    const bool ok = (e < NPXU) && (y >= 0) && (y < Hl) && (x >= 0) && (x < Wl);
    pyx[r] = ok ? ((unsigned)y << 16) | (unsigned)x : 0xFFFFFFFFu;
  }
  float xv[NR][4], av[NR][4];
  uintx4 wv[NWV];
  float cs0[4], cs1[4], cs2[4], cs3[4], cs4[4];
  const float slo = sc_act_lo(p.dy.act), shi = sc_act_hi(p.dy.act);
  int nch = 0;
  const size_t plane = (size_t)4 * Hl * Wl;

  auto request = [&](int kc) __attribute__((always_inline)) {
    const uintx4* wsrc = wbase + (size_t)kc * WST;
#pragma unroll
    for (int j = 0; j < NWV; ++j) wv[j] = wsrc[tid + 512 * j];
    const int cbase = (kc >> 2) * 16 + hw * 8 + sub * 4;
    const unsigned qoff = (unsigned)(((kc >> 1) & 1) * 2 * Wl + (kc & 1));
    nch = Co - cbase;
    const int cb0 = nch > 0 ? cbase : 0;
    const size_t o0 = ((size_t)n * Co + cb0) * plane;
    const float* xb = p.dy.x + o0;
    const float* ab = p.dy.aux + o0;
    const int jmax = nch > 0 ? nch - 1 : 0;
#pragma unroll
    for (int r = 0; r < NR; ++r) {
// ... 232 lines not shown
                     reinterpret_cast<unsigned short*>(wpk), Cout, Cup, Cskip, terms == 1 ? 1 : 0, total);
  SC_LAUNCH_OK("sc_pack_weights_sp");
  return SC_OK;
}

static inline int sp_groups_per_wave(int N, int Hl, int Wl, int ctiles) {
  const long wgs2 = Wl >= 32 ? (long)N * ((Wl + 31) / 32) * ((Hl + 7) / 8) * ctiles : (long)N * ((Wl + 15) / 16) * ((Hl + 15) / 16) * ctiles;
  static const int force = [] { const char* e = getenv("STARCOP_SP_NPP"); return e ? atoi(e) : 0; }();
  if (force == 1 || force == 2) return force;
  return wgs2 <= 128 ? 1 : 2;
}

extern "C" int sc_sp_stat_rows(int N, int H, int W, int Cout) {
  const int Hl = H / 2, Wl = W / 2;
  const int TW = Wl >= 32 ? 32 : 16, TH = 128 * sp_groups_per_wave(N, Hl, Wl, (Cout + 31) / 32) / TW;
  return N * ((Wl + TW - 1) / TW) * ((Hl + TH - 1) / TH);
}

static int conv3_sp_check(const sc_conv_args* a) {
  SC_REQUIRE(a != nullptr, "sc_conv3x3_sp: null args");
  SC_REQUIRE(a->ks == 3 && (a->nsrc == 1 || a->nsrc == 2), "sc_conv3x3_sp: ks = 3, one (up-sampled) or two (up-sampled, skip) sources");
  SC_REQUIRE(a->src[0].up == 1, "sc_conv3x3_sp: src[0] must be the half-resolution tensor (up = 1)");
  SC_REQUIRE(a->nsrc == 1 || a->src[1].up == 0, "sc_conv3x3_sp: src[1] is the full-resolution skip tensor (up = 0)");
  for (int s = 0; s < a->nsrc; ++s) {
    SC_REQUIRE(a->src[s].mode == SC_SRC_RAW || a->src[s].mode == SC_SRC_AFFINE, "sc_conv3x3_sp: RAW or AFFINE sources");
    SC_REQUIRE(a->src[s].mode == SC_SRC_RAW || a->src[s].cst != nullptr, "sc_conv3x3_sp: source %d needs constants", s);
    SC_REQUIRE(a->src[s].C > 0, "sc_conv3x3_sp: source %d has no channels", s);
  }
  SC_REQUIRE(a->N > 0 && a->H > 0 && a->W > 0 && a->Cout > 0, "sc_conv3x3_sp: bad shape");
  SC_REQUIRE(a->H % 2 == 0 && a->W % 2 == 0, "sc_conv3x3_sp: even output size");
  SC_REQUIRE(a->terms == SC_TERMS_F16X2 || a->terms == 1, "sc_conv3x3_sp: terms = SC_TERMS_F16X2 (two fp16 terms) or 1 (one bf16 term)");
  SC_REQUIRE(a->csplit == a->Cout && a->out1 == nullptr && a->add0 == nullptr && a->add1 == nullptr && !a->down0 && !a->accum0,
             "sc_conv3x3_sp: a single plain output");
  SC_REQUIRE(((uintptr_t)a->wpk & 15) == 0 && ((uintptr_t)a->out0 & 7) == 0, "sc_conv3x3_sp: alignment");
  SC_REQUIRE((size_t)32 * a->H * a->W < (1ull << 32), "sc_conv3x3_sp: plane too large");
  return SC_OK;
}

static int sp_variant_code(int N, int Hl, int Wl, int ctiles, int terms) {
  return 100 * (Wl >= 32 ? 2 : 1) + 10 * sp_groups_per_wave(N, Hl, Wl, ctiles) + (terms == 1 ? 1 : 4);
}
static int conv3_sp_variant_of(const sc_conv_args* a) { return sp_variant_code(a->N, a->H / 2, a->W / 2, (a->Cout + 31) / 32, a->terms); }

extern "C" int sc_sp_variant(const sc_conv_args* a) {
  return conv3_sp_check(a) == SC_OK ? conv3_sp_variant_of(a) : -1;
}

#define SC_SP_CASE(K, TW, NPP, M) \
  case 100 * (TW / 16) + 10 * NPP + M: kern = K<TW, M == 1, NPP>; break;
#define SC_SP_CASES(K) \
  SC_SP_CASE(K, 16, 1, 1) SC_SP_CASE(K, 16, 1, 4) SC_SP_CASE(K, 16, 2, 1) SC_SP_CASE(K, 16, 2, 4) \
  SC_SP_CASE(K, 32, 1, 1) SC_SP_CASE(K, 32, 1, 4) SC_SP_CASE(K, 32, 2, 1) SC_SP_CASE(K, 32, 2, 4)

extern "C" int sc_conv3x3_sp(const sc_conv_args* a, sc_stream stream) {
  if (const int rc = conv3_sp_check(a)) return rc;
  ConvSPP p;
  p.s0 = to_srcd(a->src[0]);
  p.s1 = a->nsrc == 2 ? to_srcd(a->src[1]) : p.s0;
  if (a->nsrc != 2) p.s1.C = 0;
  if (p.s0.mode == SC_SRC_RAW) p.s0.cst = sc_identity_cst_table(p.s0.C);
  if (p.s1.mode == SC_SRC_RAW) p.s1.cst = sc_identity_cst_table(p.s1.C);
  SC_REQUIRE(p.s0.cst != nullptr && p.s1.cst != nullptr, "sc_conv3x3_sp: identity constants unavailable");
  p.wpk = reinterpret_cast<const uintx4*>(a->wpk);
  p.N = a->N; p.Hl = a->H / 2; p.Wl = a->W / 2; p.Cout = a->Cout;
  p.out = a->out0; p.stats = a->stats;
  p.xb0 = a->xbound[0]; p.xb1 = a->nsrc == 2 ? a->xbound[1] : nullptr;
  const int variant = conv3_sp_variant_of(a);
  const int TW = 16 * (variant / 100), TH = 128 * ((variant / 10) % 10) / TW;
  const long tiles = (long)((p.Wl + TW - 1) / TW) * ((p.Hl + TH - 1) / TH) * a->N;
  const long ncot = (a->Cout + 31) / 32;
  const long grid = (tiles + 7) / 8 * 8 * ncot;
  SC_REQUIRE(grid < (1L << 31), "sc_conv3x3_sp: grid too large");
  void (*kern)(ConvSPP) = nullptr;
  switch (variant) {
    SC_SP_CASES(k_conv3_sp)
    default: SC_REQUIRE(false, "sc_conv3x3_sp: no kernel for variant %d", variant);
  }
  const int lds = TW == 32 ? sp_smem_bytes<32>() : sp_smem_bytes<16>();
  if (int rc = sc_lds_limit(kern, lds, "sc_conv3x3_sp")) return rc;
  hipLaunchKernelGGL(kern, dim3((unsigned)grid), dim3(512), lds, (hipStream_t)stream, p);
  SC_LAUNCH_OK("sc_conv3x3_sp");
  return SC_OK;
}

extern "C" size_t sc_packed_weight_floats_spd(int Cout, int Cup, int Cskip_tiles) {
  return (size_t)((Cup + 127) / 128 + (Cskip_tiles + 31) / 32) * 4 * ((Cout + 15) / 16) * SP_WST * 4;
}

extern "C" int sc_spd_vskip_ok(int Cup, int Cskip) { return Cup > 0 && Cup <= 64 && Cskip > 0 && Cskip <= 16; }

extern "C" int sc_pack_weights_spd(const float* w, float* wpk, int Cout, int CinTotal, int Cup, int vskip, int terms, sc_stream stream) {
  SC_REQUIRE(w && wpk && Cout > 0 && Cup > 0 && Cup <= CinTotal, "sc_pack_weights_spd: bad argument");
  SC_REQUIRE(terms == SC_TERMS_F16X2 || terms == 1, "sc_pack_weights_spd: terms must be SC_TERMS_F16X2 or 1 (one bf16 term)");
  SC_REQUIRE(vskip >= 0 && vskip <= 2, "sc_pack_weights_spd: vskip must be 0 (up-sampled channels only), 1 (virtual skip channels) or 2 (skip tiles)");
  SC_REQUIRE(vskip != 1 || sc_spd_vskip_ok(Cup, CinTotal - Cup), "sc_pack_weights_spd: virtual skip channels need Cup <= 64 and 1..16 skip channels");
  SC_REQUIRE(vskip != 2 || CinTotal > Cup, "sc_pack_weights_spd: skip tiles need skip channels");
  SC_REQUIRE(((uintptr_t)wpk & 15) == 0, "sc_pack_weights_spd: destination must be 16-byte aligned");
  const size_t total = spd_pack_items(Cout, Cup, vskip == 2 ? CinTotal - Cup : 0);
  hipLaunchKernelGGL(k_pack_weights_spd, dim3((unsigned)((total + 255) / 256)), dim3(256), 0, (hipStream_t)stream, w,
                     reinterpret_cast<unsigned short*>(wpk), Cout, CinTotal, Cup, vskip, terms == 1 ? 1 : 0, total);
  SC_LAUNCH_OK("sc_pack_weights_spd");
  return SC_OK;
}

static int conv3_spd_check(const sc_conv_args* a) {
  SC_REQUIRE(a != nullptr, "sc_conv3x3_sp_dgrad: null args");
  SC_REQUIRE(a->ks == 3 && a->nsrc == 1, "sc_conv3x3_sp_dgrad: ks = 3, one source (the layer's output gradient)");
  SC_REQUIRE(a->src[0].mode == SC_SRC_BNBWD && a->src[0].aux != nullptr && a->src[0].cst != nullptr && a->src[0].up == 0,
             "sc_conv3x3_sp_dgrad: the source is the full-resolution SC_SRC_BNBWD operand (g, y, constants)");
  SC_REQUIRE(a->N > 0 && a->H > 0 && a->W > 0 && a->Cout > 0 && a->src[0].C > 0, "sc_conv3x3_sp_dgrad: bad shape");
  SC_REQUIRE(a->H % 2 == 0 && a->W % 2 == 0, "sc_conv3x3_sp_dgrad: even gradient size");
  SC_REQUIRE(a->terms == SC_TERMS_F16X2 || a->terms == 1, "sc_conv3x3_sp_dgrad: terms = SC_TERMS_F16X2 (two fp16 terms) or 1 (one bf16 term)");
  SC_REQUIRE(a->add0 == nullptr && a->add1 == nullptr && a->stats == nullptr && a->csplit > 0 && a->csplit <= a->Cout,
             "sc_conv3x3_sp_dgrad: outputs are out0 [N, csplit, H/2, W/2] (+ out1 [N, Cout - csplit, H, W]); no add / stats");
  SC_REQUIRE((a->csplit == a->Cout) == (a->out1 == nullptr), "sc_conv3x3_sp_dgrad: out1 exactly when csplit < Cout");
  SC_REQUIRE(((uintptr_t)a->wpk & 15) == 0, "sc_conv3x3_sp_dgrad: alignment");
  SC_REQUIRE((size_t)128 * (a->H / 2) * (a->W / 2) < (1ull << 32) && (size_t)a->H * a->W < (1ull << 31), "sc_conv3x3_sp_dgrad: plane too large");
  return SC_OK;
}

static int spd_skip_mode(const sc_conv_args* a) {
  return a->out1 == nullptr ? 0 : (sc_spd_vskip_ok(a->csplit, a->Cout - a->csplit) ? 1 : 2);
}
static int spd_skip_tiles(const sc_conv_args* a) { return spd_skip_mode(a) == 2 ? (a->Cout - a->csplit + 31) / 32 : 0; }

static int conv3_spd_variant_of(const sc_conv_args* a) {
  return 1000 * spd_skip_mode(a) + sp_variant_code(a->N, a->H / 2, a->W / 2, (a->csplit + 127) / 128 + spd_skip_tiles(a), a->terms);
}

extern "C" int sc_spd_variant(const sc_conv_args* a) {
  return conv3_spd_check(a) == SC_OK ? conv3_spd_variant_of(a) : -1;
}

extern "C" int sc_conv3x3_sp_dgrad(const sc_conv_args* a, sc_stream stream) {
  if (const int rc = conv3_spd_check(a)) return rc;
  ConvSPD p;
  p.dy = to_srcd(a->src[0]);
  p.wpk = reinterpret_cast<const uintx4*>(a->wpk);
  p.N = a->N; p.Hl = a->H / 2; p.Wl = a->W / 2; p.Cup = a->csplit;
  p.out = a->out0; p.accum = a->accum0; p.absmax = a->absmax;
  p.out_skip = a->out1; p.Cskip = a->Cout - a->csplit; p.accum_skip = a->accum1;
  const int variant = conv3_spd_variant_of(a);
  p.skip_mode = variant / 1000;
  p.ntu = (a->csplit + 127) / 128;
  p.nts = spd_skip_tiles(a);
  const int TW = 16 * ((variant / 100) % 10), TH = 128 * ((variant / 10) % 10) / TW;
  const long tiles = (long)((p.Wl + TW - 1) / TW) * ((p.Hl + TH - 1) / TH) * a->N;
  const long ncot = p.ntu + p.nts;
  const long grid = (tiles + 7) / 8 * 8 * ncot;
  SC_REQUIRE(grid < (1L << 31), "sc_conv3x3_sp_dgrad: grid too large");
  void (*kern)(ConvSPD) = nullptr;
  switch (variant % 1000) {
    SC_SP_CASES(k_conv3_spd)
    default: SC_REQUIRE(false, "sc_conv3x3_sp_dgrad: no kernel for variant %d", variant);
  }
  const int lds = TW == 32 ? sp_smem_bytes<32>() : sp_smem_bytes<16>();
  if (int rc = sc_lds_limit(kern, lds, "sc_conv3x3_sp_dgrad")) return rc;
  hipLaunchKernelGGL(kern, dim3((unsigned)grid), dim3(512), lds, (hipStream_t)stream, p);
  SC_LAUNCH_OK("sc_conv3x3_sp_dgrad");
  return SC_OK;
}
#undef SC_SP_CASES
#undef SC_SP_CASE
```

### starcop_amd/csrc/conv_valu.hip

```cpp
#include <type_traits>
#include "sc_common.h"
#include "sc_scene.h"
#ifndef SC_HEAD_RB
#define SC_HEAD_RB 18
#endif

namespace {

__device__ __forceinline__ float load_src(const SrcD& s, size_t idx, int c) {
  const float x = s.x[idx];
  if (s.mode == SC_SRC_RAW) return x;
  const float4 c0 = *reinterpret_cast<const float4*>(s.cst + (size_t)c * SC_CST);
  const float c4 = s.cst[(size_t)c * SC_CST + 4];
  const float au = (s.mode == SC_SRC_BNBWD) ? s.aux[idx] : 0.f;
  return sc_prologue(s.mode, s.act, x, au, c0, c4);
}

template <int NV>
__device__ __forceinline__ void block_sum(float (&v)[NV], float* s_tmp ) {
  const int lane = threadIdx.x & 63, wave = threadIdx.x >> 6;
#pragma unroll
  for (int k = 0; k < NV; ++k) {
    const float s = wave_sum(v[k]);
    if (lane == 0) s_tmp[wave * NV + k] = s;
// ... 1281 lines not shown
          const int ci = rc / PR, r = rc - ci * PR;
          const int y = y0 - 1 + r;
          const bool oky = (y >= 0) && (y < H);
          const float* row = in.x + ((size_t)n * CIN + pass * CP + ci) * H * W + (size_t)(oky ? y : 0) * W;
          va[u] = row[oka ? xa : 0];
          vb[u] = row[okb ? xb : 0];
        }
#pragma unroll
        for (int u = 0; u < RB; ++u) {
          const int rr = rr0 + 4 * u;
          if (rr < NROW) {
            const int ci = rr / PR, r = rr - ci * PR;
            const int y = y0 - 1 + r;
            const bool oky = (y >= 0) && (y < H);
            const int cg = pass * CP + ci;
            const float sc = s_sc[cg * 2], sh = s_sc[cg * 2 + 1];
            s_in[(ci * PR + r) * PC + lane] = (oky && oka) ? sc_pro_affine(va[u], sc, sh, lo, hi) : 0.f;
            if (lane < 2) s_in[(ci * PR + r) * PC + 64 + lane] = (oky && okb) ? sc_pro_affine(vb[u], sc, sh, lo, hi) : 0.f;
          }
        }
      }
    }
    __syncthreads();
#pragma unroll 2
    for (int ci = 0; ci < CP; ++ci) {
      const float4* wp = reinterpret_cast<const float4*>(&s_w[(pass * CP + ci) * 12]);
      const float4 w0 = wp[0], w1 = wp[1], w2 = wp[2];
      const float wk[9] = {w0.x, w0.y, w0.z, w0.w, w1.x, w1.y, w1.z, w1.w, w2.x};
#pragma unroll
      for (int kh = 0; kh < 3; ++kh) {
        const float* rp = &s_in[(ci * PR + py + kh) * PC + 4 * pxg];
        const float4 a = *reinterpret_cast<const float4*>(rp);
        const float2 b = *reinterpret_cast<const float2*>(rp + 4);
        const float v[6] = {a.x, a.y, a.z, a.w, b.x, b.y};
#pragma unroll
        for (int kw = 0; kw < 3; ++kw)
#pragma unroll
          for (int o = 0; o < 4; ++o) acc[o] = fmaf(wk[kh * 3 + kw], v[o + kw], acc[o]);
      }
    }
  }
  const int y = y0 + py, x = x0 + 4 * pxg;
  if (y >= H) return;
  float* op = out + (size_t)n * H * W + (size_t)y * W + x;
  if (x + 3 < W && ((W & 3) == 0) && ((uintptr_t)op & 15) == 0) {
    *reinterpret_cast<float4*>(op) = make_float4(acc[0], acc[1], acc[2], acc[3]);
  } else {
#pragma unroll
    for (int o = 0; o < 4; ++o) if (x + o < W) op[o] = acc[o];
  }
}

__global__ __launch_bounds__(256, 4) void k_head_fwd16v(const SrcD in, const float* __restrict__ w, const float* __restrict__ bias,
                                                      float* __restrict__ out, int H, int W) {
  constexpr int CIN = 16, CP = 8, TR = 16, TC = 64, PR = TR + 2, PC = 68, NROW = CP * PR, QW = NROW / 16, NHALO = NROW * 2;
  static_assert(NROW % 16 == 0 && NHALO <= 512, "four waves x QW requests of four rows; two halo elements per thread");
  __shared__ __attribute__((aligned(16))) float s_in[NROW * PC + 4];
  __shared__ __attribute__((aligned(16))) float s_w[CIN * 12];
  __shared__ float s_sc[CIN * 2];
  const int n = blockIdx.z;
  const int tiles_x = (W + TC - 1) / TC;
  const int ty = blockIdx.x / tiles_x, tx = blockIdx.x - ty * tiles_x;
  const int y0 = ty * TR, x0 = tx * TC;
  const float lo = sc_act_lo(in.act), hi = sc_act_hi(in.act);
  const bool raw = in.mode == SC_SRC_RAW;
  const int lane = threadIdx.x & 63, wave = threadIdx.x >> 6;
  const int lr = lane >> 4, xg = x0 + 4 * (lane & 15);
  const bool okx = xg < W;
  const float* plane0 = in.x + (size_t)n * CIN * H * W;
  float4 v[QW];
  float hv[2];
  auto issue = [&](int pass) {
#pragma unroll
    for (int u = 0; u < QW; ++u) {
      const int rr = 4 * (wave + 4 * u) + lr, ci = rr / PR, y = y0 - 1 + rr - ci * PR;
      const bool oky = (y >= 0) && (y < H);
      v[u] = *reinterpret_cast<const float4*>(plane0 + ((size_t)(pass * CP + ci) * H + (oky ? y : 0)) * W + (okx ? xg : 0));
    }
#pragma unroll
    for (int h = 0; h < 2; ++h) {
      const int e = threadIdx.x + 256 * h, ec = e < NHALO ? e : 0, rr = ec >> 1, ci = rr / PR, y = y0 - 1 + rr - ci * PR;
      const int x = (ec & 1) ? x0 + TC : x0 - 1;
      const bool ok = (y >= 0) && (y < H) && (x >= 0) && (x < W);
      hv[h] = plane0[((size_t)(pass * CP + ci) * H + (ok ? y : 0)) * W + (ok ? x : 0)];
    }
  };
  auto commit = [&](int pass) {
#pragma unroll
    for (int u = 0; u < QW; ++u) {
      const int rr = 4 * (wave + 4 * u) + lr, ci = rr / PR, y = y0 - 1 + rr - ci * PR;
      const bool ok = (y >= 0) && (y < H) && okx;
      const float sc = s_sc[(pass * CP + ci) * 2], sh = s_sc[(pass * CP + ci) * 2 + 1];
      float4 t;
      t.x = ok ? sc_pro_affine(v[u].x, sc, sh, lo, hi) : 0.f; t.y = ok ? sc_pro_affine(v[u].y, sc, sh, lo, hi) : 0.f;
      t.z = ok ? sc_pro_affine(v[u].z, sc, sh, lo, hi) : 0.f; t.w = ok ? sc_pro_affine(v[u].w, sc, sh, lo, hi) : 0.f;
      *reinterpret_cast<float4*>(&s_in[rr * PC + 4 + 4 * (lane & 15)]) = t;
    }
#pragma unroll
    for (int h = 0; h < 2; ++h) {
      const int e = threadIdx.x + 256 * h;
      if (e < NHALO) {
        const int rr = e >> 1, ci = rr / PR, y = y0 - 1 + rr - ci * PR;
        const int x = (e & 1) ? x0 + TC : x0 - 1;
        const bool ok = (y >= 0) && (y < H) && (x >= 0) && (x < W);
        const float sc = s_sc[(pass * CP + ci) * 2], sh = s_sc[(pass * CP + ci) * 2 + 1];
        s_in[rr * PC + ((e & 1) ? PC : 3)] = ok ? sc_pro_affine(hv[h], sc, sh, lo, hi) : 0.f;
      }
    }
  };
  issue(0);
  if (threadIdx.x < CIN * 12) { const int c = threadIdx.x / 12, t = threadIdx.x - 12 * c; s_w[threadIdx.x] = t < 9 ? w[c * 9 + t] : 0.f; }
  if (threadIdx.x >= 224 && threadIdx.x < 224 + CIN * 2) {
    const int i = threadIdx.x - 224, c = i >> 1, h = i & 1;
    s_sc[i] = raw ? (h ? 0.f : 1.f) : in.cst[(size_t)c * SC_CST + h];
  }
// ... 373 lines not shown
  if constexpr (MO::prob_out) {
    long long off;
    if (head_mosaic_px(mo, core, y, x, off)) {
      const long long r = (long long)core.dst_row + y - core.core_y0, c = (long long)core.dst_col + x - core.core_x0;
      float p;
      uint32_t m;
      head_prob_px(mo, acc[0], r, c, p, m);
      if (mo.prob) mo.prob[r * mo.prob_pitch + c] = p;
      if (mo.mosaic) mo.mosaic[off] = (uint8_t)m;
    }
  } else if (MOS) {
    long long off;
    if (head_mosaic_px(mo, core, y, x, off)) mo.mosaic[off] = (uint8_t)head_argmax<KT, 1>(acc, K);
  } else if (classes) {
    classes[(size_t)n * HW + pix] = (uint8_t)head_argmax<KT, 1>(acc, K);
  }
}

__global__ __launch_bounds__(256) void k_head_dgrad(const float* __restrict__ dl, const float* __restrict__ w,
                                                    float* __restrict__ gin, int Cin, int H, int W) {
  constexpr int PR = HT_R + 2, PC = HT_C + 2;
  __shared__ float s_dl[PR * PC];
  __shared__ float s_w[HEAD_MAXCI * 9];
  const int n = blockIdx.z;
  const int tiles_x = (W + HT_C - 1) / HT_C;
  const int ty = blockIdx.x / tiles_x, tx = blockIdx.x - ty * tiles_x;
  const int y0 = ty * HT_R, x0 = tx * HT_C;
  for (int i = threadIdx.x; i < Cin * 9; i += 256) s_w[i] = w[i];
  for (int i = threadIdx.x; i < PR * PC; i += 256) {
    const int r = i / PC, cc = i - r * PC;
    const int y = y0 - 1 + r, x = x0 - 1 + cc;
    s_dl[i] = (y >= 0 && y < H && x >= 0 && x < W) ? dl[(size_t)n * H * W + (size_t)y * W + x] : 0.f;
  }
  __syncthreads();
  const int py = threadIdx.x >> 5, px = threadIdx.x & 31;
  const int y = y0 + py, x = x0 + px;
  if (y >= H || x >= W) return;
  float d[9];
#pragma unroll
  for (int t = 0; t < 9; ++t) d[t] = s_dl[(py + 2 - t / 3) * PC + px + 2 - (t % 3)];
  for (int ci = 0; ci < Cin; ++ci) {
    float acc = 0.f;
#pragma unroll
    for (int t = 0; t < 9; ++t) acc = fmaf(s_w[ci * 9 + t], d[t], acc);
    gin[((size_t)n * Cin + ci) * H * W + (size_t)y * W + x] = acc;
  }
}

constexpr int HB_ROW = 16 * 9 + 1, HB_MAXWG = 1024;
constexpr int HB_R = 32, HB_PF = 4;
template <bool BNS>
__global__ __launch_bounds__(256) void k_head_bwd16(const float* __restrict__ dl, const SrcD in, const float* __restrict__ w,
                                                    float* __restrict__ gin, float* __restrict__ rows, int N, int H, int W,
                                                    double* __restrict__ bn_sums, float* __restrict__ bn_absmax) {
  constexpr int CIN = 16, PR = HB_R + 2, PC = 64 + 2;
  __shared__ float s_dl[PR * PC];
  const int wave = __builtin_amdgcn_readfirstlane(threadIdx.x >> 6), lane = threadIdx.x & 63;
  const int c0 = wave * 4;
  float wk[4][9], sc[4], sh[4], mu[4], is[4];
  float b1[4] = {0.f, 0.f, 0.f, 0.f}, b2[4] = {0.f, 0.f, 0.f, 0.f}, bmx = 0.f;
#pragma unroll
  for (int j = 0; j < 4; ++j) {
    sc[j] = 1.f; sh[j] = 0.f; mu[j] = 0.f; is[j] = 1.f;
    if (in.mode != SC_SRC_RAW) { sc[j] = in.cst[(size_t)(c0 + j) * SC_CST]; sh[j] = in.cst[(size_t)(c0 + j) * SC_CST + 1]; }
    if (BNS) { mu[j] = in.cst[(size_t)(c0 + j) * SC_CST + 2]; is[j] = in.cst[(size_t)(c0 + j) * SC_CST + 3]; }
#pragma unroll
    for (int t = 0; t < 9; ++t) wk[j][t] = w[(c0 + j) * 9 + t];
  }
  const float lo = sc_act_lo(in.act), hi = sc_act_hi(in.act);
  float prod[4][9], bsum = 0.f;
#pragma unroll
  for (int j = 0; j < 4; ++j)
#pragma unroll
    for (int t = 0; t < 9; ++t) prod[j][t] = 0.f;
  const int tiles_x = (W + 63) / 64, tiles_y = (H + HB_R - 1) / HB_R;
  const int T = N * tiles_x * tiles_y;
  const size_t HW = (size_t)H * W;
  for (int tile = blockIdx.x; tile < T; tile += gridDim.x) {
    const int n = tile / (tiles_x * tiles_y), tt = tile - n * tiles_x * tiles_y;
    const int y0 = (tt / tiles_x) * HB_R, x0 = (tt % tiles_x) * 64;
    __syncthreads();
    for (int i = threadIdx.x; i < PR * PC; i += 256) {
      const int r = i / PC, cc = i - r * PC;
      const int y = y0 - 1 + r, x = x0 - 1 + cc;
      s_dl[i] = (y >= 0 && y < H && x >= 0 && x < W) ? dl[(size_t)n * HW + (size_t)y * W + x] : 0.f;
    }
    __syncthreads();
    const int x = x0 + lane;
    const bool xok = x < W;
    const float* xb = in.x + ((size_t)n * CIN + c0) * HW + (xok ? x : 0);
    float* gb = gin + ((size_t)n * CIN + c0) * HW + x;
    float xq[HB_PF][4];
#pragma unroll
    for (int u = 0; u < HB_PF; ++u) {
      const int yc = (y0 + u < H) ? y0 + u : H - 1;
#pragma unroll
      for (int j = 0; j < 4; ++j) xq[u][j] = xb[(size_t)j * HW + (size_t)yc * W];
    }
    for (int r0 = 0; r0 < HB_R; r0 += HB_PF) {
#pragma unroll
      for (int u = 0; u < HB_PF; ++u) {
        const int r = r0 + u, y = y0 + r;
        float d[9];
#pragma unroll
        for (int kh = 0; kh < 3; ++kh)
#pragma unroll
          for (int kw = 0; kw < 3; ++kw) d[kh * 3 + kw] = s_dl[(r + 2 - kh) * PC + lane + 2 - kw];
        const bool ok = xok && y < H;
        if (wave == 0) bsum += ok ? d[4] : 0.f;
        const int yn = (y + HB_PF < H) ? y + HB_PF : H - 1;
#pragma unroll
        for (int j = 0; j < 4; ++j) {
          float g = 0.f;
#pragma unroll
          for (int t = 0; t < 9; ++t) g = fmaf(wk[j][t], d[t], g);
          if (ok) gb[(size_t)j * HW + (size_t)y * W] = g;
          if (BNS) {
            const float yh = fmaf(xq[u][j], sc[j], sh[j]);
            const float gq = (ok && yh > lo && yh < hi) ? g : 0.f;
            b1[j] += gq;
            b2[j] = fmaf(gq, (xq[u][j] - mu[j]) * is[j], b2[j]);
            bmx = fmaxf(bmx, fabsf(gq * sc[j]));
          }
          const float xa = ok ? sc_pro_affine(xq[u][j], sc[j], sh[j], lo, hi) : 0.f;
#pragma unroll
          for (int t = 0; t < 9; ++t) prod[j][t] = fmaf(xa, d[t], prod[j][t]);
          xq[u][j] = xb[(size_t)j * HW + (size_t)yn * W];
        }
      }
    }
  }
#pragma unroll
  for (int j = 0; j < 4; ++j)
#pragma unroll
    for (int t = 0; t < 9; ++t) {
      const float v = wave_sum(prod[j][t]);
      if (lane == 0) rows[(size_t)blockIdx.x * HB_ROW + (c0 + j) * 9 + t] = v;
    }
  if (wave == 0) {
    bsum = wave_sum(bsum);
    if (lane == 0) rows[(size_t)blockIdx.x * HB_ROW + CIN * 9] = bsum;
  }
  if (BNS) {
#pragma unroll
    for (int j = 0; j < 4; ++j) {
      const float s1 = wave_sum(b1[j]), s2 = wave_sum(b2[j]);
      if (lane == 0) {
        bn_sums[((size_t)blockIdx.x * CIN + c0 + j) * 2] = (double)s1;
        bn_sums[((size_t)blockIdx.x * CIN + c0 + j) * 2 + 1] = (double)s2;
      }
    }
    if (bn_absmax) {
#pragma unroll
      for (int o = 32; o > 0; o >>= 1) bmx = fmaxf(bmx, __shfl_xor(bmx, o, 64));
      if (lane == 0 && bmx > __builtin_nontemporal_load(bn_absmax)) atomicMax(reinterpret_cast<unsigned*>(bn_absmax), __builtin_bit_cast(unsigned, bmx));
    }
  }
}
__global__ __launch_bounds__(256) void k_head_bwd_reduce(const float* __restrict__ rows, int nrows, float* __restrict__ dw, float* __restrict__ dbias) {
  __shared__ double s_tmp[4];
  const int col = blockIdx.x;
  double v = 0.0;
  for (int r = threadIdx.x; r < nrows; r += 256) v += (double)rows[(size_t)r * HB_ROW + col];
  v = wave_sum_d(v);
  if ((threadIdx.x & 63) == 0) s_tmp[threadIdx.x >> 6] = v;
  __syncthreads();
  if (threadIdx.x == 0) {
    v = (s_tmp[0] + s_tmp[1]) + (s_tmp[2] + s_tmp[3]);
    if (col < 16 * 9) dw[col] = (float)v;
    else if (dbias) dbias[0] = (float)v;
  }
}

__global__ __launch_bounds__(256) void k_sum_f32_to_f64(const float* __restrict__ x, size_t n, double* acc) {
  __shared__ float s_tmp[4];
  float v[1] = {0.f};
  for (size_t i = blockIdx.x * (size_t)256 + threadIdx.x; i < n; i += (size_t)gridDim.x * 256) v[0] += x[i];
  block_sum<1>(v, s_tmp);
  if (threadIdx.x == 0) atomicAdd(acc, (double)v[0]);
}

__global__ void k_cast_f64_f32(const double* __restrict__ in, float* __restrict__ out, size_t n) {
  for (size_t i = blockIdx.x * (size_t)blockDim.x + threadIdx.x; i < n; i += (size_t)gridDim.x * blockDim.x) out[i] = (float)in[i];
}

int stem_blocks(int N, int Hout, int Wout) {
  long T = (long)N * ((Wout + 31) / 32) * ((Hout + 3) / 4);
  return (int)(T < 1024 ? T : 1024);
}
int head_blocks(int N, int H, int W) {
  long T = (long)N * ((W + HT_C - 1) / HT_C) * ((H + HT_R - 1) / HT_R);
  return (int)(T < 1024 ? T : 1024);
}

}

#define SC_DW_DISPATCH4(KERNEL, CODE_, GRID, ...)                                                                       \
  do {                                                                                                                  \
    switch (CODE_) {                                                                                                    \
      case 1641: hipLaunchKernelGGL((KERNEL<1, 64, 8, true>), GRID, dim3(256), 0, st, __VA_ARGS__); break;              \
      case 1640: hipLaunchKernelGGL((KERNEL<1, 64, 8, false>), GRID, dim3(256), 0, st, __VA_ARGS__); break;             \
      case 1321: hipLaunchKernelGGL((KERNEL<1, 32, 4, true>), GRID, dim3(256), 0, st, __VA_ARGS__); break;              \
// ... 102 lines not shown
}

extern "C" int sc_dwconv3x3_wgrad(const sc_src* dy, const sc_src* in, double* dw_acc, int N, int C, int Hin, int Win,
                                  int stride, sc_stream stream) {
  SC_REQUIRE(dy && in && dy->C == C && in->C == C, "sc_dwconv3x3_wgrad: source channels != C");
  SC_REQUIRE(stride == 1 || stride == 2, "sc_dwconv3x3_wgrad: stride must be 1 or 2");
  SC_REQUIRE((in->mode == SC_SRC_RAW || in->mode == SC_SRC_AFFINE) && in->up == 0 && dy->mode != SC_SRC_NORM && dy->up == 0,
             "sc_dwconv3x3_wgrad: unsupported source mode");
  const int Hout = (Hin - 1) / stride + 1, Wout = (Win - 1) / stride + 1;
  hipStream_t st = (hipStream_t)stream;
  const long T = (long)N * dw_tiles(Hout, Wout);
  const long want = 4096 / C > 0 ? 4096 / C : 1;
  dim3 grid((unsigned)(T < want ? T : want), C);
  SC_DW_DISPATCH(k_dw_wgrad, dw_variant(2, N, C, Hin, Win, stride, true, true), grid, to_srcd(*dy), to_srcd(*in), dw_acc, N, C, Hin, Win, Hout, Wout, 0);
  SC_LAUNCH_OK("sc_dwconv3x3_wgrad");
  return SC_OK;
}

extern "C" int sc_dwconv3x3_bwd_fused(const sc_src* dy, const sc_src* in, const float* w, float* dx, double* dw_acc,
                                      double* in_sums, int N, int C, int Hin, int Win, int stride, sc_stream stream) {
  SC_REQUIRE(dy && in && w && dx && dw_acc && dy->C == C && in->C == C, "sc_dwconv3x3_bwd_fused: bad argument");
  SC_REQUIRE(stride == 1 || stride == 2, "sc_dwconv3x3_bwd_fused: stride must be 1 or 2");
  SC_REQUIRE((in->mode == SC_SRC_RAW || in->mode == SC_SRC_AFFINE) && in->up == 0 && dy->mode != SC_SRC_NORM && dy->up == 0,
             "sc_dwconv3x3_bwd_fused: unsupported source mode");
  SC_REQUIRE(dy->mode != SC_SRC_BNBWD || dy->aux != nullptr, "sc_dwconv3x3_bwd_fused: BNBWD source needs aux");
  SC_REQUIRE(!in_sums || in->mode == SC_SRC_AFFINE, "sc_dwconv3x3_bwd_fused: BatchNorm-backward sums need an affine (BatchNorm'd) input");
  SC_REQUIRE(stride == 1 || (Hin % 2 == 0 && Win % 2 == 0), "sc_dwconv3x3_bwd_fused: stride 2 needs even input sizes");
  const int Hout = (Hin - 1) / stride + 1, Wout = (Win - 1) / stride + 1;
  hipStream_t st = (hipStream_t)stream;
  const long planes8 = ((long)N * C + 7) / 8 * 8;
  SC_REQUIRE(planes8 * dw_tiles(Hin, Win) < (1L << 31), "sc_dwconv3x3_bwd_fused: grid too large");
  dim3 grid((unsigned)(planes8 * dw_tiles(Hin, Win)));
  const int variant = dw_variant(3, N, C, Hin, Win, stride, ((((uintptr_t)dy->x) | ((uintptr_t)dy->aux) | ((uintptr_t)in->x)) & 15) == 0,
                                 ((uintptr_t)dx & 15) == 0);
  if (variant >= 9000) {
    if (variant == 9016) hipLaunchKernelGGL(k_dw_bwd_plane<16>, dim3((unsigned)((long)N * C / 4)), dim3(256), 0, st, to_srcd(*dy), to_srcd(*in), w, dx, dw_acc, in_sums, C);
    else hipLaunchKernelGGL(k_dw_bwd_plane<32>, dim3((unsigned)((long)N * C / 4)), dim3(256), 0, st, to_srcd(*dy), to_srcd(*in), w, dx, dw_acc, in_sums, C);
    SC_LAUNCH_OK("sc_dwconv3x3_bwd_fused");
    return SC_OK;
  }
  SC_DW_DISPATCH4(k_dw_bwd, variant, grid, to_srcd(*dy), to_srcd(*in), w, dx, dw_acc, in_sums, N * C, C, Hin, Win, Hout, Wout);
  SC_LAUNCH_OK("sc_dwconv3x3_bwd_fused");
  return SC_OK;
}

extern "C" int sc_head_bwd_bn_rows(int N, int H, int W) {
  const long T = (long)N * ((W + 63) / 64) * ((H + HB_R - 1) / HB_R);
  return (int)(T < HB_MAXWG ? T : HB_MAXWG);
}

extern "C" int sc_head_conv_bwd(const float* dlogits, const sc_src* in, const float* w, float* gin, float* part, size_t part_floats,
                                float* dw, float* dbias, int N, int Cin, int H, int W, double* bn_sums, float* bn_absmax,
                                sc_stream stream) {
  SC_REQUIRE(dlogits && in && w && gin && part && dw && in->C == Cin, "sc_head_conv_bwd: bad argument");
  SC_REQUIRE(Cin == 16, "sc_head_conv_bwd: Cin must be 16 (use sc_head_conv_dgrad + sc_head_conv_wgrad otherwise)");
  SC_REQUIRE((in->mode == SC_SRC_RAW || in->mode == SC_SRC_AFFINE) && in->up == 0, "sc_head_conv_bwd: unsupported source mode");
  SC_REQUIRE(part_floats >= sc_head_wgrad_workspace_floats(N, Cin, H, W), "sc_head_conv_bwd: workspace too small");
  SC_REQUIRE(N > 0 && H > 0 && W > 0, "sc_head_conv_bwd: bad shape");
  hipStream_t st = (hipStream_t)stream;
  const long T = (long)N * ((W + 63) / 64) * ((H + HB_R - 1) / HB_R);
  const int nwg = (int)(T < HB_MAXWG ? T : HB_MAXWG);
  SC_REQUIRE(!bn_sums || in->mode == SC_SRC_AFFINE, "sc_head_conv_bwd: the fused BatchNorm-backward sums need the AFFINE source of that BatchNorm");
  if (bn_sums) hipLaunchKernelGGL(k_head_bwd16<true>, dim3(nwg), dim3(256), 0, st, dlogits, to_srcd(*in), w, gin, part, N, H, W, bn_sums, bn_absmax);
  else hipLaunchKernelGGL(k_head_bwd16<false>, dim3(nwg), dim3(256), 0, st, dlogits, to_srcd(*in), w, gin, part, N, H, W, (double*)nullptr, (float*)nullptr);
  SC_LAUNCH_OK("sc_head_conv_bwd");
  hipLaunchKernelGGL(k_head_bwd_reduce, dim3(HB_ROW), dim3(256), 0, st, part, nwg, dw, dbias);
  SC_LAUNCH_OK("sc_head_conv_bwd(reduce)");
  return SC_OK;
}

__global__ __launch_bounds__(256) void k_cast_f64_f32_batch(const sc_cast_desc* __restrict__ descs) {
  const sc_cast_desc d = descs[blockIdx.x];
  for (size_t i = (size_t)blockIdx.y * 256 + threadIdx.x; i < d.n; i += (size_t)gridDim.y * 256) d.out[i] = (float)d.in[i];
}
extern "C" int sc_cast_f64_f32_batch(const sc_cast_desc* descs_dev, int n_descs, sc_stream stream) {
  SC_REQUIRE(descs_dev != nullptr && n_descs > 0, "sc_cast_f64_f32_batch: no descriptors");
  hipLaunchKernelGGL(k_cast_f64_f32_batch, dim3(n_descs, 8), dim3(256), 0, (hipStream_t)stream, descs_dev);
  SC_LAUNCH_OK("sc_cast_f64_f32_batch");
  return SC_OK;
}

extern "C" int sc_cast_f64_f32(const double* in, float* out, size_t n, sc_stream stream) {
  if (n == 0) return SC_OK;
  const int blocks = (int)((n + 255) / 256 > 1024 ? 1024 : (n + 255) / 256);
  hipLaunchKernelGGL(k_cast_f64_f32, dim3(blocks), dim3(256), 0, (hipStream_t)stream, in, out, n);
  SC_LAUNCH_OK("sc_cast_f64_f32");
  return SC_OK;
}

extern "C" int sc_stem_conv_fwd(const sc_src* in, const float* w, float* out, int N, int Cin, int Hin, int Win,
                                float* stats, sc_stream stream) {
  SC_REQUIRE(in && in->C == Cin, "sc_stem_conv_fwd: source channels != Cin");
  SC_REQUIRE(Cin >= 1 && Cin <= STEM_MAXCI_FWD, "sc_stem_conv_fwd: Cin must be in [1,%d] (got %d)", STEM_MAXCI_FWD, Cin);
  SC_REQUIRE(!stats || Cin <= STEM_MAXCI, "sc_stem_conv_fwd: statistics rows need Cin <= %d (got %d): the wide stem is inference only", STEM_MAXCI, Cin);
  SC_REQUIRE(in->mode != SC_SRC_BNBWD && in->up == 0, "sc_stem_conv_fwd: unsupported source mode");
  const int Hout = (Hin - 1) / 2 + 1, Wout = (Win - 1) / 2 + 1;
  dim3 grid(((Wout + 31) / 32) * ((Hout + 7) / 8), 1, N);
  switch (sc_stem_fwd_kernel(Cin, Win, ((uintptr_t)out & 15) == 0)) {
    case SC_STEM_K_MFMA4: hipLaunchKernelGGL(k_stem_fwd4m, grid, dim3(256), 0, (hipStream_t)stream, to_srcd(*in), w, out, Cin, Hin, Win, Hout, Wout, stats); break;
    case SC_STEM_K_VALU4: hipLaunchKernelGGL(k_stem_fwd<4>, grid, dim3(256), 0, (hipStream_t)stream, to_srcd(*in), w, out, Cin, Hin, Win, Hout, Wout, stats); break;
    case SC_STEM_K_VALU8: hipLaunchKernelGGL(k_stem_fwd<STEM_MAXCI>, grid, dim3(256), 0, (hipStream_t)stream, to_srcd(*in), w, out, Cin, Hin, Win, Hout, Wout, stats); break;
    default: hipLaunchKernelGGL(k_stem_fwd16, grid, dim3(256), 0, (hipStream_t)stream, to_srcd(*in), w, out, Cin, Hin, Win, Hout, Wout); break;
  }
  SC_LAUNCH_OK("sc_stem_conv_fwd");
  return SC_OK;
}

extern "C" int sc_stem_fwd_kernel(int Cin, int Win, int out_aligned16) {
  if (Cin < 1 || Cin > STEM_MAXCI_FWD) return SC_ERR_ARG;
  const int Wout = (Win - 1) / 2 + 1;
  static const bool mfma_off = [] { const char* e = getenv("STARCOP_STEM_MFMA"); return e && atoi(e) == 0; }();
  if (Cin <= 4) return (!mfma_off && Wout % 4 == 0 && out_aligned16) ? SC_STEM_K_MFMA4 : SC_STEM_K_VALU4;
  return Cin <= STEM_MAXCI ? SC_STEM_K_VALU8 : SC_STEM_K_VALU16;
}

extern "C" int sc_stem_wgrad_njb(int Cin) {
  if (Cin < 1 || Cin > STEM_MAXCI) return SC_ERR_ARG;
  return (Cin * 9 + 15) / 16 <= 3 ? 3 : 5;
}

extern "C" int sc_stem_wgrad_rows(int N, int Hin, int Win) {
  if (N < 1 || Hin < 1 || Win < 1) return SC_ERR_ARG;
  return stem_blocks(N, (Hin - 1) / 2 + 1, (Win - 1) / 2 + 1);
}

extern "C" size_t sc_stem_wgrad_workspace_floats(int N, int Cin, int Hin, int Win) {
  const int nb = sc_stem_wgrad_rows(N, Hin, Win);
  if (nb < 0) return 0;
  const size_t E = (size_t)STEM_CO * Cin * 9;
  return (size_t)nb * E + sc_reduce_scratch_floats(nb, E);
}

extern "C" int sc_stem_conv_wgrad(const sc_src* dy, const sc_src* in, float* part, size_t part_floats, float* dw, int N,
                                  int Cin, int Hin, int Win, sc_stream stream) {
  SC_REQUIRE(dy && in && in->C == Cin && dy->C == STEM_CO, "sc_stem_conv_wgrad: bad source channels");
  SC_REQUIRE(Cin >= 1 && Cin <= STEM_MAXCI, "sc_stem_conv_wgrad: Cin must be in [1,%d]", STEM_MAXCI);
  SC_REQUIRE(N > 0 && Hin > 0 && Win > 0, "sc_stem_conv_wgrad: bad shape");
  SC_REQUIRE(part_floats >= sc_stem_wgrad_workspace_floats(N, Cin, Hin, Win), "sc_stem_conv_wgrad: workspace too small");
  const int Hout = (Hin - 1) / 2 + 1, Wout = (Win - 1) / 2 + 1;
  const int nb = sc_stem_wgrad_rows(N, Hin, Win);
  const size_t E = (size_t)STEM_CO * Cin * 9;
  hipStream_t st = (hipStream_t)stream;
  if (sc_stem_wgrad_njb(Cin) == 3) hipLaunchKernelGGL((k_stem_wgrad<3>), dim3(nb), dim3(256), 0, st, to_srcd(*dy), to_srcd(*in), part, N, Cin, Hin, Win, Hout, Wout);
  else hipLaunchKernelGGL((k_stem_wgrad<5>), dim3(nb), dim3(256), 0, st, to_srcd(*dy), to_srcd(*in), part, N, Cin, Hin, Win, Hout, Wout);
  SC_LAUNCH_OK("sc_stem_conv_wgrad");
  return sc_reduce_rows(part, nb, E, part + (size_t)nb * E, dw, st);
}

extern "C" int sc_head_fwd_kernel(int Cin, int W, int in_aligned16, int out_aligned16) {
  if (Cin < 1 || Cin > HEAD_MAXCI || W < 1) return SC_ERR_ARG;
  if (Cin != 16) return SC_HEAD_K_GENERIC;
  return (W % 4 == 0 && in_aligned16 && out_aligned16) ? SC_HEAD_K_FWD16V : SC_HEAD_K_FWD16;
}

extern "C" int sc_head_conv_fwd(const sc_src* in, const float* w, const float* bias, float* out, int N, int Cin,
                                int H, int W, sc_stream stream) {
  SC_REQUIRE(in && in->C == Cin, "sc_head_conv_fwd: source channels != Cin");
  SC_REQUIRE(Cin >= 1 && Cin <= HEAD_MAXCI, "sc_head_conv_fwd: Cin must be in [1,%d]", HEAD_MAXCI);
  SC_REQUIRE((in->mode == SC_SRC_RAW || in->mode == SC_SRC_AFFINE) && in->up == 0, "sc_head_conv_fwd: unsupported source mode");
  dim3 grid(((W + HT_C - 1) / HT_C) * ((H + HT_R - 1) / HT_R), 1, N);
  dim3 g16(((W + 63) / 64) * ((H + 15) / 16), 1, N);
  switch (sc_head_fwd_kernel(Cin, W, ((uintptr_t)in->x & 15) == 0, ((uintptr_t)out & 15) == 0)) {
    case SC_HEAD_K_FWD16V: hipLaunchKernelGGL(k_head_fwd16v, g16, dim3(256), 0, (hipStream_t)stream, to_srcd(*in), w, bias, out, H, W); break;
    case SC_HEAD_K_FWD16: hipLaunchKernelGGL(k_head_fwd16, g16, dim3(256), 0, (hipStream_t)stream, to_srcd(*in), w, bias, out, H, W); break;
    default: hipLaunchKernelGGL((k_head_fwd<0>), grid, dim3(256), 0, (hipStream_t)stream, to_srcd(*in), w, bias, out, Cin, H, W); break;
  }
  SC_LAUNCH_OK("sc_head_conv_fwd");
  return SC_OK;
}

template <int KT>
static void launch_head_fwdk16(bool vec, dim3 grid, hipStream_t st, const SrcD& s, const float* w, const float* bias, float* logits,
                               uint8_t* classes, int K, int H, int W, int lvec, int cvec, const HeadMosaic& mo) {
  if (mo.win) {
    if (vec) hipLaunchKernelGGL((k_head_fwdk16<KT, true, true>), grid, dim3(256), 0, st, s, w, bias, logits, classes, K, H, W, lvec, cvec, mo);
    else hipLaunchKernelGGL((k_head_fwdk16<KT, false, true>), grid, dim3(256), 0, st, s, w, bias, logits, classes, K, H, W, lvec, cvec, mo);
  } else {
    if (vec) hipLaunchKernelGGL((k_head_fwdk16<KT, true, false>), grid, dim3(256), 0, st, s, w, bias, logits, classes, K, H, W, lvec, cvec, mo);
    else hipLaunchKernelGGL((k_head_fwdk16<KT, false, false>), grid, dim3(256), 0, st, s, w, bias, logits, classes, K, H, W, lvec, cvec, mo);
  }
}

static void launch_head_fwdk(const sc_src* in, const float* w, const float* bias, float* logits, uint8_t* classes, const HeadMosaic& mo,
                             int N, int Cin, int K, int H, int W, hipStream_t st) {
  if (Cin == 16) {
    dim3 g16(((W + 63) / 64) * ((H + 15) / 16), 1, N);
    const bool w4 = W % 4 == 0;
    const bool vec = w4 && ((uintptr_t)in->x & 15) == 0;
    const int lvec = w4 && ((uintptr_t)logits & 15) == 0, cvec = w4 && ((uintptr_t)classes & 3) == 0;
    if (K <= 2) launch_head_fwdk16<2>(vec, g16, st, to_srcd(*in), w, bias, logits, classes, K, H, W, lvec, cvec, mo);
    else if (K <= 4) launch_head_fwdk16<4>(vec, g16, st, to_srcd(*in), w, bias, logits, classes, K, H, W, lvec, cvec, mo);
    else launch_head_fwdk16<8>(vec, g16, st, to_srcd(*in), w, bias, logits, classes, K, H, W, lvec, cvec, mo);
  } else {
    dim3 grid(((W + HT_C - 1) / HT_C) * ((H + HT_R - 1) / HT_R), 1, N);
    if (mo.win) hipLaunchKernelGGL(k_head_fwdk<true>, grid, dim3(256), 0, st, to_srcd(*in), w, bias, logits, classes, Cin, K, H, W, mo);
    else hipLaunchKernelGGL(k_head_fwdk<false>, grid, dim3(256), 0, st, to_srcd(*in), w, bias, logits, classes, Cin, K, H, W, mo);
  }
}

extern "C" int sc_head_conv_fwd_k(const sc_src* in, const float* w, const float* bias, float* logits, uint8_t* classes, int N,
                                  int Cin, int K, int H, int W, sc_stream stream) {
  SC_REQUIRE(in && in->C == Cin, "sc_head_conv_fwd_k: source channels != Cin");
  SC_REQUIRE(Cin >= 1 && Cin <= HEAD_MAXCI, "sc_head_conv_fwd_k: Cin must be in [1,%d]", HEAD_MAXCI);
  SC_REQUIRE(K >= 1 && K <= HEADK_MAXK, "sc_head_conv_fwd_k: K must be in [1,%d] (got %d)", HEADK_MAXK, K);
  SC_REQUIRE((in->mode == SC_SRC_RAW || in->mode == SC_SRC_AFFINE) && in->up == 0, "sc_head_conv_fwd_k: unsupported source mode");
  SC_REQUIRE(logits || classes, "sc_head_conv_fwd_k: at least one of logits / classes must be given");
  SC_REQUIRE(w && N > 0 && H > 0 && W > 0, "sc_head_conv_fwd_k: bad argument");
  hipStream_t st = (hipStream_t)stream;
  if (K == 1) {
    if (classes && hipMemsetAsync(classes, 0, (size_t)N * H * W, st) != hipSuccess) { sc_set_error("sc_head_conv_fwd_k: memset failed"); return SC_ERR_LAUNCH; }
    return logits ? sc_head_conv_fwd(in, w, bias, logits, N, Cin, H, W, stream) : SC_OK;
  }
  launch_head_fwdk(in, w, bias, logits, classes, HeadMosaic{nullptr, nullptr, 0, 0, 0}, N, Cin, K, H, W, st);
  SC_LAUNCH_OK("sc_head_conv_fwd_k");
  return SC_OK;
}
// ... 94 lines not shown
```

### starcop_amd/csrc/elementwise.hip

```cpp
#include <stdarg.h>
#include <string.h>
#include "sc_common.h"
#include <atomic>
#include <mutex>
#include <set>
#include <utility>

static thread_local char g_err[512] = "";
void sc_set_error(const char* fmt, ...) {
  va_list ap;
  va_start(ap, fmt);
  vsnprintf(g_err, sizeof(g_err), fmt, ap);
  va_end(ap);
}
extern "C" const char* sc_last_error(void) { return g_err; }

int sc_lds_limit(const void* kernel, size_t bytes, const char* who) {
  if (bytes <= 64 * 1024) return SC_OK;
  static std::mutex mu;
  static std::set<std::pair<int, const void*>> done;
  int dev = 0;
  hipError_t e = hipGetDevice(&dev);
  if (e == hipSuccess) {
    std::lock_guard<std::mutex> lock(mu);
// ... 71 lines not shown
  if (training) {
    double v[2] = {0.0, 0.0};
    int r = threadIdx.x;
    for (; r + 7 * NT < nrows; r += 8 * NT) {
      TS t[8][2];
#pragma unroll
      for (int k = 0; k < 8; ++k) { t[k][0] = stats[((size_t)(r + NT * k) * C + c) * 2]; t[k][1] = stats[((size_t)(r + NT * k) * C + c) * 2 + 1]; }
#pragma unroll
      for (int k = 0; k < 8; ++k) { v[0] += (double)t[k][0]; v[1] += (double)t[k][1]; }
    }
    for (; r < nrows; r += NT) {
      v[0] += (double)stats[((size_t)r * C + c) * 2]; v[1] += (double)stats[((size_t)r * C + c) * 2 + 1];
    }
    {
      const int lane = threadIdx.x & 63, wave = threadIdx.x >> 6;
#pragma unroll
      for (int k = 0; k < 2; ++k) {
        const double sw = wave_sum_d(v[k]);
        if (lane == 0) s_tmp[wave * 2 + k] = sw;
      }
      __syncthreads();
#pragma unroll
      for (int k = 0; k < 2; ++k) {
        double t = 0.0;
#pragma unroll
        for (int w = 0; w < NW; ++w) t += s_tmp[w * 2 + k];
        v[k] = t;
      }
    }
    mean = v[0] / count;
    var = v[1] / count - mean * mean;
    if (var < 0.0) var = 0.0;
  } else {
    mean = (double)running_mean[c];
    var = (double)running_var[c];
  }
  if (threadIdx.x != 0) return;
  bn_write_channel(mean, var, count, training, gamma, beta, running_mean, running_var, momentum, eps, cst, c, act_bound);
}

__device__ __forceinline__ void block_absmax_to(float m, float factor, float* slot, float* s_m) {
#pragma unroll
  for (int o = 32; o > 0; o >>= 1) m = fmaxf(m, __shfl_xor(m, o, 64));
  if ((threadIdx.x & 63) == 0) s_m[threadIdx.x >> 6] = m;
  __syncthreads();
  if (threadIdx.x == 0) {
    const float t = fmaxf(fmaxf(s_m[0], s_m[1]), fmaxf(s_m[2], s_m[3])) * fabsf(factor);
    if (t > __builtin_nontemporal_load(slot)) atomicMax(reinterpret_cast<unsigned*>(slot), __builtin_bit_cast(unsigned, t));
  }
}

__global__ __launch_bounds__(256) void k_bn_bwd_reduce(const float* __restrict__ g, const float* __restrict__ y,
                                                       const float* __restrict__ cst, int act, double* __restrict__ sums, int C, int HW,
                                                       float* __restrict__ absmax, float* __restrict__ act_absmax) {
  __shared__ double s_tmp[8];
  __shared__ float s_m[4];
  const int c = blockIdx.y, n = blockIdx.z;
  const float scale = cst[(size_t)c * SC_CST], shift = cst[(size_t)c * SC_CST + 1];
  const float mean = cst[(size_t)c * SC_CST + 2], invstd = cst[(size_t)c * SC_CST + 3];
  const float lo = sc_act_lo(act), hi = sc_act_hi(act);
  const size_t base = ((size_t)n * C + c) * HW;
  const int start = blockIdx.x * 4096;
  const int end = min(start + 4096, HW);
  float s1 = 0.f, s2 = 0.f, mx = 0.f, ax = 0.f;
  if ((HW & 3) == 0) {
    for (int i = start + threadIdx.x * 4; i < end; i += 1024) {
      const float4 yv = *reinterpret_cast<const float4*>(y + base + i);
      const float4 gv = *reinterpret_cast<const float4*>(g + base + i);
      const float ya[4] = {yv.x, yv.y, yv.z, yv.w}, ga[4] = {gv.x, gv.y, gv.z, gv.w};
#pragma unroll
      for (int k = 0; k < 4; ++k) {
        const float yh = fmaf(ya[k], scale, shift);
        const float gb = (yh > lo && yh < hi) ? ga[k] : 0.f;
        s1 += gb;
        s2 = fmaf(gb, (ya[k] - mean) * invstd, s2);
        mx = fmaxf(mx, fabsf(gb));
        ax = fmaxf(ax, fabsf(yh));
      }
    }
  } else {
    for (int i = start + threadIdx.x; i < end; i += 256) {
      const float yv = y[base + i], gv = g[base + i];
      const float yh = fmaf(yv, scale, shift);
      const float gb = (yh > lo && yh < hi) ? gv : 0.f;
      s1 += gb;
      s2 = fmaf(gb, (yv - mean) * invstd, s2);
      mx = fmaxf(mx, fabsf(gb));
      ax = fmaxf(ax, fabsf(yh));
    }
  }
  double v[2] = {(double)s1, (double)s2};
  block_sum_d<2>(v, s_tmp);
  if (threadIdx.x < 2) sums[(stat_row() * C + c) * 2 + threadIdx.x] = v[threadIdx.x];
  if (absmax) block_absmax_to(mx, scale, absmax, s_m);
  if (act_absmax) {
    __syncthreads();
    block_absmax_to(act == SC_ACT_RELU6 ? fminf(ax, 6.f) : ax, 1.f, act_absmax, s_m);
  }
}

__global__ __launch_bounds__(256) void k_bn_bwd_small(const float* __restrict__ g, const float* __restrict__ y,
                                                      const float* __restrict__ cst, int act, int N, int C, int HW, double count,
                                                      float* __restrict__ dgamma, float* __restrict__ dbeta, float* __restrict__ cst_bwd,
                                                      float* __restrict__ absmax, float* __restrict__ act_absmax) {
  __shared__ double s_tmp[8];
  __shared__ float s_m[4];
  float mx = 0.f, ax = 0.f;
  const int c = blockIdx.x;
  const float scale = cst[(size_t)c * SC_CST], shift = cst[(size_t)c * SC_CST + 1];
  const float mean = cst[(size_t)c * SC_CST + 2], invstd = cst[(size_t)c * SC_CST + 3];
  const float lo = sc_act_lo(act), hi = sc_act_hi(act);
  double v[2] = {0.0, 0.0};
  auto acc4 = [&](const float4& yv, const float4& gv, float& s1, float& s2) {
    const float ya[4] = {yv.x, yv.y, yv.z, yv.w}, ga[4] = {gv.x, gv.y, gv.z, gv.w};
#pragma unroll
    for (int k = 0; k < 4; ++k) {
      const float yh = fmaf(ya[k], scale, shift);
      const float gb = (yh > lo && yh < hi) ? ga[k] : 0.f;
      s1 += gb;
      s2 = fmaf(gb, (ya[k] - mean) * invstd, s2);
      mx = fmaxf(mx, fabsf(gb));
      ax = fmaxf(ax, fabsf(yh));
    }
  };
  if ((HW & 3) == 0) {
    const int q = HW >> 2, total = N * q;
    int it = threadIdx.x;
    for (; it + 3 * 256 < total; it += 4 * 256) {
      float4 yv[4], gv[4];
#pragma unroll
      for (int u = 0; u < 4; ++u) {
        const int item = it + 256 * u, n = item / q, i = (item - n * q) * 4;
        const size_t o = ((size_t)n * C + c) * HW + i;
        yv[u] = *reinterpret_cast<const float4*>(y + o);
        gv[u] = *reinterpret_cast<const float4*>(g + o);
      }
      float s1 = 0.f, s2 = 0.f;
#pragma unroll
      for (int u = 0; u < 4; ++u) acc4(yv[u], gv[u], s1, s2);
      v[0] += (double)s1; v[1] += (double)s2;
    }
    for (; it < total; it += 256) {
      const int n = it / q, i = (it - n * q) * 4;
      const size_t o = ((size_t)n * C + c) * HW + i;
      float s1 = 0.f, s2 = 0.f;
      acc4(*reinterpret_cast<const float4*>(y + o), *reinterpret_cast<const float4*>(g + o), s1, s2);
// ... 332 lines not shown
  const float* cur = part;
  int np = nparts;
  while (np > max_rows) {
    const int nn = (np + 15) / 16;
    hipLaunchKernelGGL(k_reduce16, dim3((unsigned)((E + 255) / 256), nn), dim3(256), 0, st, cur, np, E, scratch);
    SC_LAUNCH_OK("sc_reduce16");
    cur = scratch; scratch += (size_t)nn * E; np = nn;
  }
  *rows_out = cur; *nrows_out = np;
  return SC_OK;
}

int sc_reduce_rows(const float* part, int nparts, size_t E, float* scratch, float* out, hipStream_t st) {
  const float* cur; int np;
  int rc = sc_reduce_rows_partial(part, nparts, E, scratch, &cur, &np, 16, st);
  if (rc != SC_OK) return rc;
  hipLaunchKernelGGL(k_reduce16, dim3((unsigned)((E + 255) / 256), 1), dim3(256), 0, st, cur, np, E, out);
  SC_LAUNCH_OK("sc_reduce16(final)");
  return SC_OK;
}

extern "C" int sc_stat_rows(int kind, int N, int H, int W) {
  switch (kind) {
    case SC_STAT_CONV3: return N * ((W + 31) / 32) * ((H + 3) / 4);
    case SC_STAT_CONV1: return N * ((H * W + 127) / 128);
    case SC_STAT_CONV1K: return N * ((H * W + 31) / 32);
    case SC_STAT_DW: return N * ((W + sc_dw_tile_w(W) - 1) / sc_dw_tile_w(W)) * ((H + sc_dw_tile_h(W) - 1) / sc_dw_tile_h(W));
    case SC_STAT_STEM: return N * ((W + 31) / 32) * ((H + 7) / 8);
    case SC_STAT_BNBWD: return N * ((H * W + 4095) / 4096);
    case SC_STAT_PW3: return (int)(((long)N * H * W + 31) / 32);
    default: return -1;
  }
}

extern "C" int sc_bn_finalize(const float* stats, int nrows, double count, const float* gamma, const float* beta,
                              float* running_mean, float* running_var, float momentum, float eps, int training,
                              float* cst_fwd, int C, double* scratch, float* act_bound, sc_stream stream) {
  SC_REQUIRE(C > 0 && cst_fwd && gamma && beta && running_mean && running_var, "sc_bn_finalize: null argument");
  SC_REQUIRE(!training || (stats && count > 0 && nrows > 0), "sc_bn_finalize: training needs stats rows and count");
  if (training && nrows >= 4096 && scratch && 2 * C <= 1024) {
    hipLaunchKernelGGL(k_bn_rows_prereduce, dim3(BN_PRE_S), dim3(1024), 0, (hipStream_t)stream, stats, nrows, C, scratch);
    hipLaunchKernelGGL((k_bn_finalize<4, double>), dim3(C), dim3(256), 0, (hipStream_t)stream, (const double*)scratch, BN_PRE_S, count, gamma,
                       beta, running_mean, running_var, momentum, eps, training, cst_fwd, C, act_bound);
  } else if (training && nrows >= 4096)
    hipLaunchKernelGGL((k_bn_finalize<16>), dim3(C), dim3(1024), 0, (hipStream_t)stream, stats, nrows, count, gamma, beta,
                       running_mean, running_var, momentum, eps, training, cst_fwd, C, act_bound);
  else
    hipLaunchKernelGGL((k_bn_finalize<4>), dim3(C), dim3(256), 0, (hipStream_t)stream, stats, nrows, count, gamma, beta,
                       running_mean, running_var, momentum, eps, training, cst_fwd, C, act_bound);
  SC_LAUNCH_OK("sc_bn_finalize");
  return SC_OK;
}

extern "C" int sc_bn_bwd_reduce(const float* g, const float* y, const float* cst_fwd, int act, double* sums, int N, int C,
                                int HW, float* absmax, float* act_absmax, sc_stream stream) {
  SC_REQUIRE(g && y && cst_fwd && sums && N > 0 && C > 0 && HW > 0, "sc_bn_bwd_reduce: bad argument");
  dim3 grid((HW + 4095) / 4096, C, N);
  hipLaunchKernelGGL(k_bn_bwd_reduce, grid, dim3(256), 0, (hipStream_t)stream, g, y, cst_fwd, act, sums, C, HW, absmax, act_absmax);
  SC_LAUNCH_OK("sc_bn_bwd_reduce");
  return SC_OK;
}

extern "C" int sc_bn_bwd_small(const float* g, const float* y, const float* cst_fwd, int act, int N, int C, int HW,
                               float* dgamma, float* dbeta, float* cst_bwd, float* absmax, float* act_absmax, sc_stream stream) {
  SC_REQUIRE(g && y && cst_fwd && cst_bwd && N > 0 && C > 0 && HW > 0, "sc_bn_bwd_small: bad argument");
  hipLaunchKernelGGL(k_bn_bwd_small, dim3(C), dim3(256), 0, (hipStream_t)stream, g, y, cst_fwd, act, N, C, HW,
                     (double)N * HW, dgamma, dbeta, cst_bwd, absmax, act_absmax);
  SC_LAUNCH_OK("sc_bn_bwd_small");
  return SC_OK;
}

extern "C" int sc_bn_bwd_finalize(const double* sums, int nrows, double count, const float* cst_fwd, float* dgamma,
                                  float* dbeta, float* cst_bwd, int C, sc_stream stream) {
  SC_REQUIRE(sums && cst_fwd && cst_bwd && C > 0 && count > 0 && nrows > 0, "sc_bn_bwd_finalize: bad argument");
  hipLaunchKernelGGL(k_bn_bwd_finalize<double>, dim3(C), dim3(256), 0, (hipStream_t)stream, sums, nrows, count, cst_fwd,
                     dgamma, dbeta, cst_bwd, C);
  SC_LAUNCH_OK("sc_bn_bwd_finalize");
  return SC_OK;
}

extern "C" int sc_bn_bwd_finalize_rows32(const float* rows, int nrows, double count, const float* cst_fwd, float* dgamma,
                                         float* dbeta, float* cst_bwd, int C, double* scratch, sc_stream stream) {
  SC_REQUIRE(rows && cst_fwd && cst_bwd && C > 0 && count > 0 && nrows > 0, "sc_bn_bwd_finalize_rows32: bad argument");
  if (nrows >= 4096 && scratch && 2 * C <= 1024) {
    hipLaunchKernelGGL(k_bn_rows_prereduce, dim3(BN_PRE_S), dim3(1024), 0, (hipStream_t)stream, rows, nrows, C, scratch);
    hipLaunchKernelGGL(k_bn_bwd_finalize<double>, dim3(C), dim3(256), 0, (hipStream_t)stream, (const double*)scratch, BN_PRE_S, count, cst_fwd,
                       dgamma, dbeta, cst_bwd, C);
  } else
  hipLaunchKernelGGL(k_bn_bwd_finalize<float>, dim3(C), dim3(256), 0, (hipStream_t)stream, rows, nrows, count, cst_fwd,
                     dgamma, dbeta, cst_bwd, C);
  SC_LAUNCH_OK("sc_bn_bwd_finalize_rows32");
  return SC_OK;
}

extern "C" int sc_stream_wait_stream(sc_stream waiter, sc_stream signaller) {
  constexpr int NEV = 64, MAXDEV = 16;
  static hipEvent_t rings[MAXDEV][NEV];
  static std::once_flag once[MAXDEV];
  static bool oks[MAXDEV] = {};
  static std::atomic<unsigned> next{0};
  int dev = 0;
  if (hipGetDevice(&dev) != hipSuccess || dev < 0 || dev >= MAXDEV) {
    sc_set_error("sc_stream_wait_stream: device index outside [0, %d)", MAXDEV);
    return SC_ERR_LAUNCH;
  }
  std::call_once(once[dev], [dev] {
    bool ok = true;
    for (int i = 0; i < NEV; ++i) ok = ok && hipEventCreateWithFlags(&rings[dev][i], hipEventDisableTiming | hipEventDisableSystemFence) == hipSuccess;
    oks[dev] = ok;
  });
  if (!oks[dev]) {
    sc_set_error("sc_stream_wait_stream: hipEventCreateWithFlags failed");
    return SC_ERR_LAUNCH;
// ... 135 lines not shown
```

### starcop_amd/network.py

```python
import collections
import ctypes as C
import math
import os

import torch
import torch.nn as nn

from . import _lib, scene
from ._lib import (ACT_NONE, ACT_RELU, ACT_RELU6, SC_CST, sc_irb_args, sc_irt_args, SRC_AFFINE, SRC_BNBWD, SRC_NORM, SRC_RAW, STAT_BNBWD, sc_wgrad_pending,
                   PACK_PW3, PACK_SP, PACK_SPD, PACK_THIN16, STAT_PW3, STAT_CONV1, STAT_CONV1K, STAT_CONV3, STAT_DW, STAT_STEM, TERMS_F16X2, check, make_src, ptr,
                   sc_conv_args, sc_wgrad_args, stream)

MBV2_SETTINGS = ((1, 16, 1, 1), (6, 24, 2, 2), (6, 32, 3, 2), (6, 64, 4, 2),
                 (6, 96, 3, 1), (6, 160, 3, 2), (6, 320, 1, 1))
DECODER_CHANNELS = (256, 128, 64, 32, 16)
BN_EPS, BN_MOMENTUM = 1e-5, 0.1
HeadMosaic = collections.namedtuple("HeadMosaic", "win win_host classes prob mask valid fill_bits nodata", defaults=(None,) * 4 + (0, 0.0))


def _conv_bn_act(cin, cout, k, stride=1, groups=1, act="relu6"):
    return nn.Sequential(nn.Conv2d(cin, cout, k, stride, (k - 1) // 2, groups=groups, bias=False),
                         nn.BatchNorm2d(cout, eps=BN_EPS, momentum=BN_MOMENTUM),
                         nn.ReLU6() if act == "relu6" else nn.ReLU())

# ... 689 lines not shown
        if tab[1] is not None:
            side = None
            if need_bwd and self.overlap_wgrad and not torch.cuda.is_current_stream_capturing():
                main = torch.cuda.current_stream()
                if self._side_stream is None or self._side_stream.device != main.device:
                    self._side_stream = torch.cuda.Stream(device=main.device)
                side = self._side_stream
            if side is not None:
                sh = C.c_void_p(side.cuda_stream)
                check(lib.sc_stream_wait_stream(sh, st))
                check(lib.sc_pack_weights_batch(ptr(tab[1][0]), ptr(tab[1][1]), tab[1][2], tab[1][3], sh))
                self._late_pack_stream = sh
            else:
                check(lib.sc_pack_weights_batch(ptr(tab[1][0]), ptr(tab[1][1]), tab[1][2], tab[1][3], st))
        self._pack_version = (ver, bool(need_bwd), need_irb)

    def _src_of(self, plan, t, up=0, x_cst=None):
        if t.kind == "input":
            if x_cst is None:
                return make_src(plan.buf["x"], t.C, SRC_RAW)
            return make_src(plan.buf["x"], t.C, SRC_NORM, cst=x_cst)
        if t.kind == "raw":
            return make_src(plan.buf[t.name], t.C, SRC_AFFINE, act=t.act, up=up, cst=plan.cst[t.name])
        return make_src(plan.buf[t.name], t.C, SRC_RAW, up=up)

    def _xbound(self, plan, t):
        if t.kind == "fin" and t.name in plan.fin_slot:
            return C.c_void_p(plan.fin_amax.data_ptr() + 4 * plan.fin_slot[t.name])
        slot = plan.act_slot.get(t.name) if t.kind == "raw" else None
        return C.c_void_p(plan.act_amax.data_ptr() + 4 * slot) if slot is not None else None

    def _dy_src(self, plan, t):
        return make_src(plan.grad[t.name], t.C, SRC_BNBWD, act=t.act, cst=plan.cstb[t.name], aux=plan.buf[t.name])

    def _forward_impl(self, x, x_cst, training, need_grad, _recheck=0, head="logits", mosaic=None):
        if training and (self.classes > self.MAX_TRAIN_CLASSES or self.in_channels > self.MAX_TRAIN_IN_CHANNELS):
            raise NotImplementedError(
                f"HyperStarcopUNet(in_channels={self.in_channels}, classes={self.classes}) runs in eval mode only: training needs two "
                f"kernels that do not exist -- the stem weight gradient above {self.MAX_TRAIN_IN_CHANNELS} input channels "
                f"(sc_stem_conv_wgrad) and the backward of the K-class head (sc_head_conv_bwd is the 1-class head's)")
        _lib.require_device(x)
        lib = _lib.load()
        if x.dim() != 4 or x.shape[1] != self.in_channels:
            raise ValueError(f"HyperStarcopUNet: expected (N,{self.in_channels},H,W) input, got {tuple(x.shape)}")
        N, _, H, W = x.shape
        if H % 32 or W % 32:
            raise RuntimeError(f"Wrong input shape height={H}, width={W}. Expected image height and width "
                               "divisible by 32.")
        self._ensure_flat()
        x = x.contiguous().float()
        plan = self._get_plan(N, H, W, need_grad, want_logits=head == "logits", want_classes=head == "classes")
        plan.buf["x"] = x
        plan.x_cst = x_cst
        plan.generation = getattr(plan, "generation", 0) + 1
        self._pack_all(need_grad)
        st = stream()
        eval_key = None
        if not training:
            eval_key = (tuple(p._version for p in self.parameters()), tuple(b._version for b in self.buffers()), self._stat_epoch)
        eval_cst_ok = (eval_key is not None and getattr(plan, "eval_cst_key", None) == eval_key
                       and not torch.cuda.is_current_stream_capturing())
        if training:
            self._stat_epoch += 1
            plan.eval_cst_key = None
        if not training and not eval_cst_ok:
            for t in self._tensors.values():
                if t.bn is not None:
                    bn = t.bn
                    check(lib.sc_bn_finalize(None, 0, 1.0, ptr(bn.weight), ptr(bn.bias), ptr(bn.running_mean), ptr(bn.running_var),
                                             float(bn.momentum), float(bn.eps), 0, ptr(plan.cst[t.name]), t.C, None, None, st))
        skip = set()
        for i, op in enumerate(self._ops):
            if i in skip:
                continue
            ty, o = op["type"], op["out"]
            Ho, Wo = H >> o.shift, W >> o.shift
            if i in plan.irt:
                if training:
                    self._irt_forward(plan, i, st)
                    skip.add(plan.irt[i])
                    continue
                a_irt = self._irt_args(plan, i)
                td = self._ops[plan.irt[i]]["out"]
                self._cur_op = td.name + ":fwd"
                tok = self._pb("k_irt_* (fused expand+dw)")
                check(lib.sc_irt_fwd(C.byref(a_irt), ptr(plan.buf[td.name]), None, st))
                self._pe(tok)
                skip.add(plan.irt[i])
                continue
            if not training and i in plan.irb:
                i_dw, i_pr, i_add = plan.irb[i]
                op_d, op_p = self._ops[i_dw], self._ops[i_pr]
                tin, te, td, tp = op["ins"][0], o, op_d["out"], op_p["out"]
                ent_e, ent_p = self._wpk[i], self._wpk[i_pr]
                pe = ent_e["pf"] if "pw3" in self._pw_need.get((i, 0), ()) else ent_e["pfi"]
                pp_ = ent_p["pf"] if "pw3" in self._pw_need.get((i_pr, 0), ()) else ent_p["pfi"]
                a = sc_irb_args()
                a.x = self._src_of(plan, tin)
                a.wpk_expand, a.cst_expand = pe.data_ptr(), plan.cst[te.name].data_ptr()
                a.w_dw, a.cst_dw = op_d["conv"].weight.data_ptr(), plan.cst[td.name].data_ptr()
                a.wpk_project = pp_.data_ptr()
                a.N, a.Cin, a.hidden, a.Cout = N, op["conv"].in_channels, op["conv"].out_channels, op_p["conv"].out_channels
                a.H, a.W, a.stride = H >> tin.shift, W >> tin.shift, self._ir_blocks[i][2]
                if i_add is not None:
                    tz = self._ops[i_add]["out"]
                    a.residual, a.cst_project = 1, plan.cst[tp.name].data_ptr()
# ... 26 lines not shown
                        cu_ = op["ins"][0].C
                        fle = 2.0 * N * (Ho // 2) * (Wo // 2) * 16 * (-(-conv.out_channels // 32) * 32) * (cu_ + 4 * (conv.in_channels - cu_))
                    tok = self._pb("k_conv3_thin_h (fwd+dgrad)" if ent["tf"] is not None else
                                   self._bx3_family("fwd") if ent["bx3_f"] else f"k_conv_mfma<{conv.kernel_size[0]}> (fwd+dgrad)",
                                   fl, 4.0 * (N * src_elems + N * o.C * Ho * Wo + conv.weight.numel()), fle)
                else:
                    tok = self._pb({"stem": "k_stem_*", "dw": "k_dw_*", "head": "k_head_*", "add": "elementwise/bn"}[ty])
            if ty == "stem":
                s = self._src_of(plan, op["ins"][0], x_cst=x_cst)
                check(lib.sc_stem_conv_fwd(C.byref(s), ptr(conv.weight), ptr(plan.buf[o.name]), N, conv.in_channels,
                                           H, W, stats, st))
            elif ty == "dw":
                tin = op["ins"][0]
                s = self._src_of(plan, tin)
                check(lib.sc_dwconv3x3_fwd(C.byref(s), ptr(conv.weight), ptr(plan.buf[o.name]), N, o.C,
                                           H >> tin.shift, W >> tin.shift, op["stride"], stats, st))
            elif ty in ("pw", "conv3"):
                if ty == "conv3" and self._late_pack_stream is not None:
                    check(lib.sc_stream_wait_stream(st, self._late_pack_stream))
                    self._late_pack_stream = None
                a = sc_conv_args()
                ins = op["ins"]
                a.nsrc = len(ins)
                a.src[0] = self._src_of(plan, ins[0], up=1 if op.get("up") else 0)
                if len(ins) == 2:
                    a.src[1] = self._src_of(plan, ins[1])
                a.wpk = ent["f"].data_ptr()
                a.N, a.H, a.W, a.Cout = N, Ho, Wo, o.C
                a.ks, a.co_t = conv.kernel_size[0], ent["cot_f"]
                a.out0 = plan.buf[o.name].data_ptr(); a.out1 = None
                a.csplit, a.accum0, a.accum1 = o.C, 0, 0
                a.add0 = None; a.add1 = None
                a.stats = plan.stats_v[o.name].data_ptr() if stats is not None else None
                a.terms = ent["terms_f"]
                if ty == "conv3":
                    for k_, t_ in enumerate(ins):
                        a.xbound[k_] = self._xbound(plan, t_)
                if ty == "pw" and _use_pw3(0, N, Ho * Wo, conv.in_channels, conv.out_channels):
                    fconv = lib.sc_conv1x1_pw3
                    a.wpk = ent["pf"].data_ptr()
                elif use_sp:
                    fconv = lib.sc_conv3x3_sp
                    a.wpk = ent["sp"].data_ptr()
                    srows = lib.sc_sp_stat_rows(N, Ho, Wo, o.C)
                elif ent["tf"] is not None:
                    fconv = lib.sc_conv3x3_thin16
                    a.wpk = ent["tf"].data_ptr()
                elif ent["bx3_f"]:
                    fconv = lib.sc_conv3x3_bx3
                elif _use_ksplit(N, Ho * Wo, conv.in_channels, conv.out_channels, a.ks):
                    fconv = lib.sc_conv1x1_ksplit
                else:
                    fconv = lib.sc_conv2d_mfma
                check(fconv(C.byref(a), st))
            elif ty == "add":
                sa = self._src_of(plan, op["ins"][0])
                sb = self._src_of(plan, op["ins"][1])
                check(lib.sc_add_srcs_absmax(C.byref(sa), C.byref(sb), ptr(plan.buf[o.name]), N, o.C, Ho * Wo,
                                             plan.fin_amax.data_ptr() + 4 * plan.fin_slot[o.name], st))
            elif ty == "head":
                s = self._src_of(plan, op["ins"][0])
                if head == "mosaic":
                    mos = mosaic.classes
                    check(lib.sc_head_conv_fwd_k_mosaic(C.byref(s), ptr(conv.weight), ptr(conv.bias), ptr(mos), mos.shape[0], mos.shape[1],
                                                        mos.stride(0), mosaic.win, mosaic.win_host,
                                                        N, conv.in_channels, self.classes, Ho, Wo, st))
                elif head == "probmosaic":
                    prob, mask, valid = mosaic.prob, mosaic.mask, mosaic.valid
                    ref = prob if prob is not None else mask
                    check(lib.sc_head_conv_fwd_mosaic_prob(
                        C.byref(s), ptr(conv.weight), ptr(conv.bias), ptr(prob), prob.stride(0) if prob is not None else 0,
                        ptr(mask), mask.stride(0) if mask is not None else 0, ref.shape[0], ref.shape[1],
                        ptr(valid), valid.stride(0) if valid is not None else 0, valid.stride(1) if valid is not None else 0,
                        mosaic.fill_bits, mosaic.nodata, mosaic.win, mosaic.win_host,
                        N, conv.in_channels, Ho, Wo, st))
                elif self.classes == 1 and head == "logits":
                    check(lib.sc_head_conv_fwd(C.byref(s), ptr(conv.weight), ptr(conv.bias), ptr(plan.buf[o.name]),
                                               N, conv.in_channels, Ho, Wo, st))
                else:
                    check(lib.sc_head_conv_fwd_k(C.byref(s), ptr(conv.weight), ptr(conv.bias),
                                                 ptr(plan.buf[o.name]) if head == "logits" else None,
                                                 ptr(plan.classes) if head == "classes" else None,
                                                 N, conv.in_channels, self.classes, Ho, Wo, st))
            self._pe(tok)
            if o.bn is not None and training:
                bn = o.bn
                check(lib.sc_bn_finalize(stats, srows, float(N * Ho * Wo), ptr(bn.weight), ptr(bn.bias),
                                         ptr(bn.running_mean), ptr(bn.running_var), float(bn.momentum), float(bn.eps),
                                         1 if training else 0, ptr(plan.cst[o.name]), o.C, ptr(plan.bn_scratch),
                                         self._xbound(plan, o), st))
        if self._late_pack_stream is not None:
            check(lib.sc_stream_wait_stream(st, self._late_pack_stream))
            self._late_pack_stream = None
        if training:
            torch._foreach_add_(self._nbt_list(), 1)
        else:
            plan.eval_cst_key = eval_key
        plan.training = training
        if (not training and self.precision == "fp32" and self.range_check_every and plan.act_slot
                and not torch.cuda.is_current_stream_capturing()):
            plan.n_eval += 1
            if _recheck or plan.n_eval % self.range_check_every == 1 or self.range_check_every == 1:
                before = plan.act_amax.clone()
                self._record_activation_range(plan)
                used = torch.where(before * 2 > self.FP16_MAX_ACT,
                                   torch.exp2(torch.floor(torch.log2(self.FP16_MAX_ACT / before.clamp_min(1e-30)))), torch.full_like(before, 2.0))
                if bool((plan.act_amax * used > 2 * self.FP16_MAX_ACT).any()):
                    import warnings
                    worst = float((plan.act_amax * used).max()) / 2.0
                    if _recheck < 6:
                        if _recheck == 0:
                            self._inference_clamped += 1
                            warnings.warn(f"HyperStarcopUNet (inference, precision='fp32'): an activation of {worst:.4g} (in units of the "
                                          f"operand scale in force) exceeded the fp16 range of the split convolutions "
                                          f"({self.FP16_MAX_ACT:g}) and was clamped; the forward is redone with the adapted scale.  "
                                          f"Forwards between two checks (range_check_every={self.range_check_every}) are not re-examined: "
                                          f"set range_check_every=1 for data of unknown range")
                        return self._forward_impl(x, x_cst, training, need_grad, _recheck=_recheck + 1, head=head, mosaic=mosaic)
                    self._inference_unrepaired += 1
                    warnings.warn(f"HyperStarcopUNet (inference, precision='fp32'): activations still outside the fp16 range after 6 "
                                  f"re-runs with adapted scales ({worst:.4g}); the returned logits carry operands clamped to "
                                  f"+-65504/scale.  split_range_report()['ok'] is now False; use precision='fp32-x3' for this input")
        return plan

    def _irt_args(self, plan, i_e):
        i_dw = plan.irt[i_e]
        op, cv_d = self._ops[i_e], self._ops[i_dw]["conv"]
        cv, tin, te = op["conv"], op["ins"][0], op["out"]
        a = sc_irt_args()
        a.x = self._src_of(plan, tin)
        a.w_expand, a.w_dw, a.cst_expand = cv.weight.data_ptr(), cv_d.weight.data_ptr(), plan.cst[te.name].data_ptr()
# ... 1 lines not shown
        a.H, a.W, a.stride = plan.H >> tin.shift, plan.W >> tin.shift, self._ops[i_dw]["stride"]
        return a

    def _irt_forward(self, plan, i_e, st):
        lib = _lib.load()
        i_dw = plan.irt[i_e]
        te, td = self._ops[i_e]["out"], self._ops[i_dw]["out"]
        a = self._irt_args(plan, i_e)
        cnt_e = float(plan.N * a.H * a.W)
        Hd_, Wd_ = plan.H >> td.shift, plan.W >> td.shift
        self._cur_op = te.name + ":fwd"
        tok = self._pb("k_irt_* (fused expand+dw)")
        check(lib.sc_irt_expand_stats(C.byref(a), ptr(plan.stats_v[te.name]), st))
        self._pe(tok)
        bn = te.bn
        check(lib.sc_bn_finalize(ptr(plan.stats_v[te.name]), plan.irt_rows[te.name], cnt_e, ptr(bn.weight), ptr(bn.bias), ptr(bn.running_mean),
                                 ptr(bn.running_var), float(bn.momentum), float(bn.eps), 1, ptr(plan.cst[te.name]), te.C,
                                 ptr(plan.bn_scratch), None, st))
        self._cur_op = td.name + ":fwd"
        tok = self._pb("k_irt_* (fused expand+dw)")
        check(lib.sc_irt_fwd(C.byref(a), ptr(plan.buf[td.name]), ptr(plan.stats_v[td.name]), st))
        self._pe(tok)
        bn = td.bn
        check(lib.sc_bn_finalize(ptr(plan.stats_v[td.name]), plan.irt_rows[td.name], float(plan.N * Hd_ * Wd_), ptr(bn.weight), ptr(bn.bias),
                                 ptr(bn.running_mean), ptr(bn.running_var), float(bn.momentum), float(bn.eps), 1, ptr(plan.cst[td.name]), td.C,
                                 ptr(plan.bn_scratch), None, st))

    def _nbt_list(self):
        nbt = getattr(self, "_nbt", None)
        if nbt is None or nbt[0].device != self._pflat.device:
            nbt = [t.bn.num_batches_tracked for t in self._tensors.values() if t.bn is not None]
            self._nbt = nbt
        return nbt

    overlap_wgrad = True
    fuse_irt = _IRT != "0"
    split_bf16 = True
    bn_small_max = 16384
    precision = "fp32"
    _TERMS = {"fp32": (TERMS_F16X2, TERMS_F16X2), "fp32-x3": (3, 3), "fp32-bwd2": (3, 2), "fp32-2": (2, 2), "bf16": (1, 1)}

    def _bx3_family(self, which):
        tf_, tb_ = self._terms
        return "k_conv3_bx3 (fwd+dgrad)" if tf_ == tb_ else f"k_conv3_bx3 ({which})"

    @property
    def _terms(self):
        if self.precision not in self._TERMS:
            raise ValueError(f"precision must be one of {sorted(self._TERMS)} (got {self.precision!r})")
        return self._TERMS[self.precision]
    _side_stream = None
    _late_pack_stream = None

    def _backward_impl(self, plan, dlogits, on_tail_ready=None, only_ops=None, exchange_follows=None):
        lib = _lib.load()
        st = stream()
        main = torch.cuda.current_stream()
        side = sd = None
        if self.overlap_wgrad:
            if self._side_stream is None or self._side_stream.device != main.device:
                self._side_stream = torch.cuda.Stream(device=main.device)
            side = self._side_stream
            sd = C.c_void_p(side.cuda_stream)

        def wgrad_launch(fn):
            if side is None:
                fn(st)
            else:
                check(lib.sc_stream_wait_stream(sd, st))
                fn(sd)

        N, H, W = plan.N, plan.H, plan.W
        if not getattr(plan, "training", False):
            raise RuntimeError("HyperStarcopUNet.backward: gradients need a train-mode forward (BatchNorm batch "
                               "statistics); call .train() first")
        dlogits = dlogits.contiguous()
        plan.dw_acc.zero_()
        half_bwd = self._terms[1] == TERMS_F16X2
        gmax_slot = {}
        if half_bwd:
            plan.gmax.zero_()
        written = set()
        res_of, n_cons, prod_idx, dw_offs, last_dw = self._res_of, self._n_cons, self._prod_idx, self._dw_offs, self._last_dw
        gv = self._grad_view
        reduced = set()
        pw_pending = []

        def bn_backward(t, slot=None):
            Ho, Wo = H >> t.shift, W >> t.shift
            amax = None
            if slot is not None:
                amax = plan.gmax.data_ptr() + 4 * slot
                gmax_slot[t.name] = amax
            if t.name in reduced:
                check(lib.sc_bn_bwd_finalize(ptr(plan.dwsums[t.name]), plan.dwrows[t.name], float(N * Ho * Wo), ptr(plan.cst[t.name]),
                                             ptr(gv(t.bn.weight)), ptr(gv(t.bn.bias)), ptr(plan.cstb[t.name]), t.C, st))
                return
            aslot = plan.act_slot.get(t.name)
            aact = plan.act_amax.data_ptr() + 4 * aslot if aslot is not None else None
            if N * Ho * Wo <= self.bn_small_max and t.C >= 64:
                check(lib.sc_bn_bwd_small(ptr(plan.grad[t.name]), ptr(plan.buf[t.name]), ptr(plan.cst[t.name]), t.act, N, t.C,
                                          Ho * Wo, ptr(gv(t.bn.weight)), ptr(gv(t.bn.bias)), ptr(plan.cstb[t.name]), amax, aact, st))
                return
            check(lib.sc_bn_bwd_reduce(ptr(plan.grad[t.name]), ptr(plan.buf[t.name]), ptr(plan.cst[t.name]), t.act,
                                       ptr(plan.bsums_v[t.name]), N, t.C, Ho * Wo, amax, aact, st))
            check(lib.sc_bn_bwd_finalize(ptr(plan.bsums_v[t.name]), plan.brows[t.name], float(N * Ho * Wo), ptr(plan.cst[t.name]),
                                         ptr(gv(t.bn.weight)), ptr(gv(t.bn.bias)), ptr(plan.cstb[t.name]), t.C, st))

        def reduce_pointwise_batch():
            if not pw_pending:
                return
            raw = b"".join(bytes(p_) for p_ in pw_pending)
            if plan.pw_table is None:
                plan.pw_table = {}
            if raw not in plan.pw_table:
                import numpy as np
                starts, nblk = [], 0
                for p_ in pw_pending:
                    starts.append(nblk)
                    nblk += -(-int(p_.total) // 256)
                plan.pw_table[raw] = (torch.from_numpy(np.frombuffer(raw, dtype=np.uint8).copy()).to(self._pflat.device),
                                      torch.tensor(starts, dtype=torch.int32).to(self._pflat.device), len(pw_pending), nblk)
            tab = plan.pw_table[raw]
            tok = self._pb("k_wgrad_mfma<1> (+reduce)")
            wgrad_launch(lambda sx: check(lib.sc_wgrad_reduce_batch(ptr(tab[0]), ptr(tab[1]), tab[2], tab[3], sx)))
            self._pe(tok)
            pw_pending.clear()

        dw_casts = []

        def cast_dw_gradients():
            if not dw_casts:
                return
            key = tuple(dw_casts)
            if getattr(plan, "dw_cast_table", None) is None:
                plan.dw_cast_table = {}
            if key not in plan.dw_cast_table:
                import numpy as np
                arr = np.array([(a, b, n) for a, b, n in dw_casts], dtype=np.uint64)
                plan.dw_cast_table[key] = (torch.from_numpy(arr.view(np.uint8).copy()).to(self._pflat.device), len(dw_casts))
            tab = plan.dw_cast_table[key]
            wgrad_launch(lambda sx, tab=tab: check(lib.sc_cast_f64_f32_batch(ptr(tab[0]), tab[1], sx)))
            dw_casts.clear()

        last_pw = min((k for k, op_ in enumerate(self._ops) if op_["type"] == "pw" and k in plan.pw_part), default=-1)
        tail_lo = self._tail_lo
        tail_pending = on_tail_ready is not None
        irt_done = set()
        for i in (range(len(self._ops) - 1, -1, -1) if only_ops is None else only_ops):
            if i in irt_done:
                continue
            op = self._ops[i]
            ty, o = op["type"], op["out"]
            Ho, Wo = H >> o.shift, W >> o.shift
            conv = op.get("conv")
            if tail_pending and (conv is None or (conv.weight.data_ptr() - self._pflat.data_ptr()) // 4 < tail_lo):
                tail_pending = False
                if side is not None:
                    side.wait_stream(main)
                    with torch.cuda.stream(side):
                        on_tail_ready(tail_lo, self._gflat.numel())
                else:
                    on_tail_ready(tail_lo, self._gflat.numel())
            self._cur_op = o.name + ":bwd"
            if ty == "head":
                tin = op["ins"][0]
                s = self._src_of(plan, tin)
                tok = self._pb("k_head_*")
                bns = bna = None
                if tin.bn is not None and tin.kind == "raw" and n_cons.get(tin.name, 0) == 1:
                    if tin.name not in plan.dwsums:
                        plan.dwrows[tin.name] = lib.sc_head_bwd_bn_rows(N, Ho, Wo)
                        plan.dwsums[tin.name] = torch.empty(plan.dwrows[tin.name] * tin.C * 2, dtype=torch.float64, device=self._pflat.device)
                    bns = ptr(plan.dwsums[tin.name])
                    if half_bwd:
                        bna = plan.gmax.data_ptr() + 4 * prod_idx[tin.name]
                    reduced.add(tin.name)
                check(lib.sc_head_conv_bwd(ptr(dlogits), C.byref(s), ptr(conv.weight), ptr(plan.grad[tin.name]), ptr(plan.ws),
                                           plan.ws_floats, ptr(gv(conv.weight)), ptr(gv(conv.bias)), N, conv.in_channels, Ho, Wo,
                                           bns, bna, st))
                self._pe(tok)
                written.add(tin.name)
                continue
            if ty == "add":
                p_t = op["ins"][1]
                plan.grad[p_t.name] = plan.grad[o.name]
                written.add(p_t.name)
                continue
            tok = self._pb("elementwise/bn")
            bn_backward(o, i if (half_bwd and ty == "conv3") else None)
            self._pe(tok)
            dy = self._dy_src(plan, o)
            if ty == "stem":
                s = self._src_of(plan, op["ins"][0], x_cst=plan.x_cst)
                tok = self._pb("k_stem_*")
                wgrad_launch(lambda sx, dy=dy, s=s, conv=conv: check(lib.sc_stem_conv_wgrad(
                    C.byref(dy), C.byref(s), ptr(plan.ws), plan.ws_floats, ptr(gv(conv.weight)), N, conv.in_channels, H, W, sx)))
                self._pe(tok)
                continue
            if ty == "dw" and i in plan.irt_of_dw:
                i_e = plan.irt_of_dw[i]
                irt_done.add(i_e)
                op_e = self._ops[i_e]
                te, tin, cv_e = op_e["out"], op_e["ins"][0], op_e["conv"]
                a_irt = self._irt_args(plan, i_e)
                acc = plan.dw_acc[dw_offs[i]:dw_offs[i] + o.C * 9]
                work, esums = plan.irt_work[te.name], plan.irt_esums[te.name]
                tok = self._pb("k_irt_* (fused expand+dw)")
                wgrad_launch(lambda sx, a_irt=a_irt, work=work: check(lib.sc_irt_xmoments(C.byref(a_irt), ptr(work), sx)))
                check(lib.sc_irt_bwd(C.byref(a_irt), C.byref(dy), ptr(esums), ptr(acc), ptr(work), st))
                dw_casts.append((acc.data_ptr(), gv(conv.weight).data_ptr(), o.C * 9))
                check(lib.sc_bn_bwd_finalize(ptr(esums), lib.sc_irt_bwd_rows(N, te.C, a_irt.H, a_irt.W), float(N * a_irt.H * a_irt.W),
                                             ptr(plan.cst[te.name]), ptr(gv(te.bn.weight)), ptr(gv(te.bn.bias)), ptr(plan.cstb[te.name]), te.C, st))
                z = res_of.get(tin.name)
                check(lib.sc_irt_bwd_fix(C.byref(a_irt), ptr(plan.cstb[te.name]), ptr(work), ptr(plan.grad[tin.name]),
                                         ptr(plan.grad[z]) if z is not None else None, 1 if tin.name in written else 0, st))
                wgrad_launch(lambda sx, a_irt=a_irt, work=work, te=te, cv_e=cv_e: check(lib.sc_irt_wgrad_finalize(
                    C.byref(a_irt), ptr(plan.cstb[te.name]), ptr(work), ptr(gv(cv_e.weight)), sx)))
                self._pe(tok)
                written.add(tin.name)
                if i == last_dw:
                    cast_dw_gradients()
                continue
            if ty == "dw":
                tin = op["ins"][0]
                Hi, Wi = H >> tin.shift, W >> tin.shift
                s = self._src_of(plan, tin)
                acc = plan.dw_acc[dw_offs[i]:dw_offs[i] + o.C * 9]
                tok = self._pb("k_dw_*")
                if (tin.name not in written and tin.bn is not None and tin.name in plan.dwsums
                        and n_cons.get(tin.name, 0) == 1):
                    check(lib.sc_dwconv3x3_bwd_fused(C.byref(dy), C.byref(s), ptr(conv.weight), ptr(plan.grad[tin.name]), ptr(acc),
                                                     ptr(plan.dwsums[tin.name]), N, o.C, Hi, Wi, op["stride"], st))
# ... 311 lines not shown
```

Measured before the change: 1446 tiles/s.

## Alternate tile traversal direction between consecutive kernels to reuse last-level cache

Adds a 'rev' parameter to the 3x3 conv, head conv and BN-backward-reduce kernels so workgroups can walk their tiles in reverse order. A host-side planner picks, for each large tensor (at least 128 MiB), the direction opposite to the kernel that last touched it. The next kernel then starts on the data the previous one left in the last-level/Infinity cache. The cost is more index arithmetic and extra planner bookkeeping. The head backward partial-row indexing is also remapped.

Result: no change. 1447 tiles/s (median of 3 runs) (+0.1%).

```diff
diff --git a/include/starcop_hip.h b/include/starcop_hip.h
--- a/include/starcop_hip.h
+++ b/include/starcop_hip.h
@@ -94,6 +94,7 @@
                         sc_stream stream);
 size_t sc_packed_weight_floats_bx3(int Cout, int Cin, int co_t, int transpose_flip, int terms);
 int sc_conv3x3_bx3(const sc_conv_args* a, sc_stream stream);
+int sc_conv3x3_bx3_dir(const sc_conv_args* a, int rev, sc_stream stream);
 
 typedef struct sc_wgrad_args {
   sc_src dy;
@@ -121,17 +122,20 @@
 size_t sc_packed_weight_floats_thin16(int Cout, int Cin, int transpose_flip);
 int sc_pack_weights_thin16(const float* w_oihw, float* wpk, int Cout, int Cin, int transpose_flip, sc_stream stream);
 int sc_conv3x3_thin16(const sc_conv_args* a, sc_stream stream);
+int sc_conv3x3_thin16_dir(const sc_conv_args* a, int rev, sc_stream stream);
 
 #define SC_PACK_SP 7
 size_t sc_packed_weight_floats_sp(int Cout, int Cup, int Cskip);
 int sc_pack_weights_sp(const float* w_oihw, float* wpk, int Cout, int Cup, int Cskip, int terms, sc_stream stream);
 int sc_sp_stat_rows(int N, int H, int W, int Cout);
 int sc_conv3x3_sp(const sc_conv_args* a, sc_stream stream);
+int sc_conv3x3_sp_dir(const sc_conv_args* a, int rev, sc_stream stream);
 #define SC_PACK_SPD 8
 size_t sc_packed_weight_floats_spd(int Cout, int Cup, int Cskip_tiles );
 int sc_spd_vskip_ok(int Cup, int Cskip);
 int sc_pack_weights_spd(const float* w_oihw, float* wpk, int Cout, int CinTotal, int Cup, int vskip, int terms, sc_stream stream);
 int sc_conv3x3_sp_dgrad(const sc_conv_args* a, sc_stream stream);
+int sc_conv3x3_sp_dgrad_dir(const sc_conv_args* a, int rev, sc_stream stream);
 size_t sc_sp_wgrad_workspace_bytes(int N, int H, int W, int Cout, int Cup);
 int sc_conv3x3_sp_wgrad(const sc_wgrad_args* a, void* ws, size_t ws_bytes, sc_stream stream);
 int sc_wgrad_scatter_cols(const float* src, float* dw, int Cout, int Ccols, int CinTotal, int col_off, sc_stream stream);
@@ -232,6 +236,8 @@
 
 int sc_head_conv_fwd(const sc_src* in, const float* w , const float* bias,
                      float* out, int N, int Cin, int H, int W, sc_stream stream);
+int sc_head_conv_fwd_dir(const sc_src* in, const float* w, const float* bias, float* out, int N, int Cin, int H, int W, int rev,
+                         sc_stream stream);
 enum sc_head_kernel { SC_HEAD_K_GENERIC = 0, SC_HEAD_K_FWD16 = 1, SC_HEAD_K_FWD16V = 2 };
 int sc_head_fwd_kernel(int Cin, int W, int in_aligned16, int out_aligned16);
 int sc_head_conv_fwd_k(const sc_src* in, const float* w , const float* bias ,
@@ -245,6 +251,9 @@
 int sc_head_bwd_bn_rows(int N, int H, int W);
 int sc_head_conv_bwd(const float* dlogits, const sc_src* in, const float* w, float* gin, float* part, size_t part_floats,
                      float* dw, float* dbias, int N, int Cin, int H, int W, double* bn_sums, float* bn_absmax, sc_stream stream);
+int sc_head_conv_bwd_dir(const float* dlogits, const sc_src* in, const float* w, float* gin, float* part, size_t part_floats,
+                         float* dw, float* dbias, int N, int Cin, int H, int W, double* bn_sums, float* bn_absmax, int rev,
+                         sc_stream stream);
 
 int sc_stat_rows(int kind, int N, int H, int W);
 #define SC_BN_FINALIZE_SCRATCH_DOUBLES(C) (64 * 2 * (size_t)(C))
@@ -253,6 +262,8 @@
                    int training, float* cst_fwd, int C, double* scratch, float* act_bound, sc_stream stream);
 int sc_bn_bwd_reduce(const float* g, const float* y, const float* cst_fwd, int act,
                      double* sums, int N, int C, int HW, float* absmax, float* act_absmax, sc_stream stream);
+int sc_bn_bwd_reduce_dir(const float* g, const float* y, const float* cst_fwd, int act,
+                         double* sums, int N, int C, int HW, float* absmax, float* act_absmax, int rev, sc_stream stream);
 int sc_bn_bwd_finalize(const double* sums, int nrows, double count, const float* cst_fwd,
                        float* dgamma, float* dbeta, float* cst_bwd, int C, sc_stream stream);
 int sc_bn_bwd_finalize_rows32(const float* rows, int nrows, double count, const float* cst_fwd,
diff --git a/starcop_amd/_lib.py b/starcop_amd/_lib.py
--- a/starcop_amd/_lib.py
+++ b/starcop_amd/_lib.py
@@ -474,6 +474,13 @@
     "sc_label_keep": (_i, [_vp, _vp, _vp, _i, _i, _i, _i, _vp]),
     "sc_tiff_lzw_decode": (_i, [_vp, _sz, _vp, _sz, C.POINTER(C.c_size_t)]),
     "sc_tiff_unpredict": (_i, [_vp, _i, _i, _i, _i, _i, _i, _vp]),
+    "sc_conv3x3_bx3_dir": (_i, [C.POINTER(sc_conv_args), _i, _vp]),
+    "sc_conv3x3_thin16_dir": (_i, [C.POINTER(sc_conv_args), _i, _vp]),
+    "sc_conv3x3_sp_dir": (_i, [C.POINTER(sc_conv_args), _i, _vp]),
+    "sc_conv3x3_sp_dgrad_dir": (_i, [C.POINTER(sc_conv_args), _i, _vp]),
+    "sc_head_conv_fwd_dir": (_i, [C.POINTER(sc_src), _vp, _vp, _vp, _i, _i, _i, _i, _i, _vp]),
+    "sc_head_conv_bwd_dir": (_i, [_vp, C.POINTER(sc_src), _vp, _vp, _vp, _sz, _vp, _vp, _i, _i, _i, _i, _vp, _vp, _i, _vp]),
+    "sc_bn_bwd_reduce_dir": (_i, [_vp, _vp, _vp, _i, _vp, _i, _i, _i, _vp, _vp, _i, _vp]),
 }
 REG_L1, REG_MSE, PWREG_G_FROM_MEMORY = 0, 1, 2
 PWREG_MAXC, PWREG_PART_DOUBLES, REG_LOSS_PARTS = 16, 273, 256
diff --git a/starcop_amd/csrc/conv_bx3.hip b/starcop_amd/csrc/conv_bx3.hip
--- a/starcop_amd/csrc/conv_bx3.hip
+++ b/starcop_amd/csrc/conv_bx3.hip
@@ -18,6 +18,7 @@
   const float* absmax;
   const float* xb0; const float* xb1;
   int xcdmap;
+  int rev;
   const float* bnr_y; const float* bnr_cst; float* bnr_rows; float* bnr_absmax; int bnr_act;
 };
 
@@ -186,7 +187,7 @@
     if (p.xcdmap == 2) {
       const int total = per_img * p.N, per_xcd = (total + 7) >> 3;
       const int j = slot / ncot;
-      pt = xcd * per_xcd + j;
+      pt = xcd * per_xcd + (p.rev ? per_xcd - 1 - j : j);
       if (j >= per_xcd || pt >= total) return;
     } else {
       pt = (slot / ncot) * 8 + xcd;
@@ -703,7 +704,7 @@
     if (p.xcdmap == 2) {
       const int total = per_img * p.N, per_xcd = (total + 7) >> 3;
       const int j = slot / ncot;
-      pt = xcd * per_xcd + j;
+      pt = xcd * per_xcd + (p.rev ? per_xcd - 1 - j : j);
       if (j >= per_xcd || pt >= total) return;
     } else {
       pt = (slot / ncot) * 8 + xcd;
@@ -1116,7 +1117,7 @@
   int n, tile;
   if (p.xcdmap) {
     const int per_img = tiles_x * ((H + 7) >> 3), total = per_img * p.N, per_xcd = (total + 7) >> 3;
-    const int j = blockIdx.x >> 3, pt = (blockIdx.x & 7) * per_xcd + j;
+    const int j = blockIdx.x >> 3, pt = (blockIdx.x & 7) * per_xcd + (p.rev ? per_xcd - 1 - j : j);
     if (j >= per_xcd || pt >= total) return;
     n = pt / per_img; tile = pt - n * per_img;
   } else {
@@ -1329,7 +1330,7 @@
   int n, tile;
   if (p.xcdmap) {
     const int per_img = tiles_x * ((H + 7) >> 3), total = per_img * p.N, per_xcd = (total + 7) >> 3;
-    const int j = blockIdx.x >> 3, pt = (blockIdx.x & 7) * per_xcd + j;
+    const int j = blockIdx.x >> 3, pt = (blockIdx.x & 7) * per_xcd + (p.rev ? per_xcd - 1 - j : j);
     if (j >= per_xcd || pt >= total) return;
     n = pt / per_img; tile = pt - n * per_img;
   } else {
@@ -1473,7 +1474,7 @@
   int n, tile;
   if (p.xcdmap) {
     const int per_img = tiles_x * ((H + 7) >> 3), total = per_img * p.N, per_xcd = (total + 7) >> 3;
-    const int j = blockIdx.x >> 3, pt = (blockIdx.x & 7) * per_xcd + j;
+    const int j = blockIdx.x >> 3, pt = (blockIdx.x & 7) * per_xcd + (p.rev ? per_xcd - 1 - j : j);
     if (j >= per_xcd || pt >= total) return;
     n = pt / per_img; tile = pt - n * per_img;
   } else {
@@ -2487,7 +2488,9 @@
   return conv3_bx3_check(a) == SC_OK ? conv3_bx3_variant_of(a) : -1;
 }
 
-extern "C" int sc_conv3x3_bx3(const sc_conv_args* a, sc_stream stream) {
+extern "C" int sc_conv3x3_bx3(const sc_conv_args* a, sc_stream stream) { return sc_conv3x3_bx3_dir(a, 0, stream); }
+
+extern "C" int sc_conv3x3_bx3_dir(const sc_conv_args* a, int rev, sc_stream stream) {
   if (const int rc = conv3_bx3_check(a)) return rc;
   const int C0 = a->src[0].C, C1 = a->nsrc == 2 ? a->src[1].C : 0;
   ConvXP p;
@@ -2507,6 +2510,7 @@
     const long wbytes = (long)co_tiles * nkc * 3 * 6 * (a->terms == SC_TERMS_F16X2 || a->terms == 2 ? 2 : (a->terms == 1 ? 1 : 3)) * a->co_t * 16;
     if (xcdmap_env >= 2 && big_env > 0 && wbytes > big_env && (co_tiles >= 8 || co_tiles == 1 || co_tiles == 2 || co_tiles == 4)) p.xcdmap = 3;
   }
+  p.rev = (rev && p.xcdmap == 2) ? 1 : 0;
   if (p.xcdmap == 3) {
     const long total = (long)grid.x * a->N;
     const long slots = co_tiles >= 8 ? (long)((co_tiles + 7) / 8) * total : (total + (8 / co_tiles) - 1) / (8 / co_tiles);
@@ -2754,7 +2758,9 @@
   return thin16_check(a) == SC_OK ? thin16_variant_of(a) : -1;
 }
 
-extern "C" int sc_conv3x3_thin16(const sc_conv_args* a, sc_stream stream) {
+extern "C" int sc_conv3x3_thin16(const sc_conv_args* a, sc_stream stream) { return sc_conv3x3_thin16_dir(a, 0, stream); }
+
+extern "C" int sc_conv3x3_thin16_dir(const sc_conv_args* a, int rev, sc_stream stream) {
   if (const int rc = thin16_check(a)) return rc;
   const int Cin = a->src[0].C;
   const sc_src& s = a->src[0];
@@ -2766,7 +2772,7 @@
     p.out0 = a->out0; p.csplit = a->Cout; p.accum0 = a->accum0; p.absmax = a->absmax;
     set_bnr(p, nullptr);
     const long total = (long)((a->W + 63) / 64) * ((a->H + 7) / 8) * a->N, per_xcd = (total + 7) / 8;
-    p.xcdmap = 2;
+    p.xcdmap = 2; p.rev = rev ? 1 : 0;
     hipLaunchKernelGGL(k_conv3_thin_spd, dim3((unsigned)(per_xcd * 8)), dim3(256), 0, (hipStream_t)stream, p);
     SC_LAUNCH_OK("sc_conv3x3_thin16(down0)");
     return SC_OK;
@@ -2780,6 +2786,7 @@
   dim3 grid(((a->W + tw - 1) / tw) * ((a->H + 7) / 8), 1, a->N);
   constexpr int xcdmap_env = 2;
   p.xcdmap = xcdmap_env ? 2 : 0;
+  p.rev = (rev && p.xcdmap == 2) ? 1 : 0;
   if (p.xcdmap) {
     const long total = (long)grid.x * a->N, per_xcd = (total + 7) / 8;
     grid = dim3((unsigned)(per_xcd * 8));
diff --git a/starcop_amd/csrc/conv_sp.hip b/starcop_amd/csrc/conv_sp.hip
--- a/starcop_amd/csrc/conv_sp.hip
+++ b/starcop_amd/csrc/conv_sp.hip
@@ -16,6 +16,7 @@
   float* out;
   float* stats;
   const float* xb0; const float* xb1;
+  int rev;
 };
 
 constexpr int SP_SMEM_W = 2 * SP_WST * 16;
@@ -57,7 +58,7 @@
     const int total = per_img * p.N, per_xcd = (total + 7) >> 3;
     const int slot = blockIdx.x >> 3, xcd = blockIdx.x & 7;
     const int j = slot / ncot;
-    const int pt = xcd * per_xcd + j;
+    const int pt = xcd * per_xcd + (p.rev ? per_xcd - 1 - j : j);
     if (j >= per_xcd || pt >= total) return;
     cot = slot - j * ncot;
     n = pt / per_img; tile = pt - n * per_img;
@@ -313,6 +314,7 @@
   float* out_skip;
   int Cskip, accum_skip;
   int skip_mode, ntu, nts;
+  int rev;
 };
 
 template <int TW, bool BF, int NPP = 2>
@@ -345,7 +347,7 @@
     const int total = per_img * p.N, per_xcd = (total + 7) >> 3;
     const int slot = blockIdx.x >> 3, xcd = blockIdx.x & 7;
     const int j = slot / ncot;
-    const int pt = xcd * per_xcd + j;
+    const int pt = xcd * per_xcd + (p.rev ? per_xcd - 1 - j : j);
     if (j >= per_xcd || pt >= total) return;
     cot = slot - j * ncot;
     n = pt / per_img; tile = pt - n * per_img;
@@ -684,9 +686,12 @@
   SC_SP_CASE(K, 16, 1, 1) SC_SP_CASE(K, 16, 1, 4) SC_SP_CASE(K, 16, 2, 1) SC_SP_CASE(K, 16, 2, 4) \
   SC_SP_CASE(K, 32, 1, 1) SC_SP_CASE(K, 32, 1, 4) SC_SP_CASE(K, 32, 2, 1) SC_SP_CASE(K, 32, 2, 4)
 
-extern "C" int sc_conv3x3_sp(const sc_conv_args* a, sc_stream stream) {
+extern "C" int sc_conv3x3_sp(const sc_conv_args* a, sc_stream stream) { return sc_conv3x3_sp_dir(a, 0, stream); }
+
+extern "C" int sc_conv3x3_sp_dir(const sc_conv_args* a, int rev, sc_stream stream) {
   if (const int rc = conv3_sp_check(a)) return rc;
   ConvSPP p;
+  p.rev = rev ? 1 : 0;
   p.s0 = to_srcd(a->src[0]);
   p.s1 = a->nsrc == 2 ? to_srcd(a->src[1]) : p.s0;
   if (a->nsrc != 2) p.s1.C = 0;
@@ -764,9 +769,12 @@
   return conv3_spd_check(a) == SC_OK ? conv3_spd_variant_of(a) : -1;
 }
 
-extern "C" int sc_conv3x3_sp_dgrad(const sc_conv_args* a, sc_stream stream) {
+extern "C" int sc_conv3x3_sp_dgrad(const sc_conv_args* a, sc_stream stream) { return sc_conv3x3_sp_dgrad_dir(a, 0, stream); }
+
+extern "C" int sc_conv3x3_sp_dgrad_dir(const sc_conv_args* a, int rev, sc_stream stream) {
   if (const int rc = conv3_spd_check(a)) return rc;
   ConvSPD p;
+  p.rev = rev ? 1 : 0;
   p.dy = to_srcd(a->src[0]);
   p.wpk = reinterpret_cast<const uintx4*>(a->wpk);
   p.N = a->N; p.Hl = a->H / 2; p.Wl = a->W / 2; p.Cup = a->csplit;
diff --git a/starcop_amd/csrc/conv_valu.hip b/starcop_amd/csrc/conv_valu.hip
--- a/starcop_amd/csrc/conv_valu.hip
+++ b/starcop_amd/csrc/conv_valu.hip
@@ -1357,15 +1357,15 @@
 }
 
 __global__ __launch_bounds__(256, 4) void k_head_fwd16v(const SrcD in, const float* __restrict__ w, const float* __restrict__ bias,
-                                                      float* __restrict__ out, int H, int W) {
+                                                      float* __restrict__ out, int H, int W, int rev) {
   constexpr int CIN = 16, CP = 8, TR = 16, TC = 64, PR = TR + 2, PC = 68, NROW = CP * PR, QW = NROW / 16, NHALO = NROW * 2;
   static_assert(NROW % 16 == 0 && NHALO <= 512, "four waves x QW requests of four rows; two halo elements per thread");
   __shared__ __attribute__((aligned(16))) float s_in[NROW * PC + 4];
   __shared__ __attribute__((aligned(16))) float s_w[CIN * 12];
   __shared__ float s_sc[CIN * 2];
-  const int n = blockIdx.z;
+  const int n = rev ? gridDim.z - 1 - blockIdx.z : blockIdx.z, bx = rev ? gridDim.x - 1 - blockIdx.x : blockIdx.x;
   const int tiles_x = (W + TC - 1) / TC;
-  const int ty = blockIdx.x / tiles_x, tx = blockIdx.x - ty * tiles_x;
+  const int ty = bx / tiles_x, tx = bx - ty * tiles_x;
   const int y0 = ty * TR, x0 = tx * TC;
   const float lo = sc_act_lo(in.act), hi = sc_act_hi(in.act);
   const bool raw = in.mode == SC_SRC_RAW;
@@ -1845,9 +1845,10 @@
 template <bool BNS>
 __global__ __launch_bounds__(256) void k_head_bwd16(const float* __restrict__ dl, const SrcD in, const float* __restrict__ w,
                                                     float* __restrict__ gin, float* __restrict__ rows, int N, int H, int W,
-                                                    double* __restrict__ bn_sums, float* __restrict__ bn_absmax) {
+                                                    double* __restrict__ bn_sums, float* __restrict__ bn_absmax, int rev) {
   constexpr int CIN = 16, PR = HB_R + 2, PC = 64 + 2;
   __shared__ float s_dl[PR * PC];
+  const int wg = rev ? gridDim.x - 1 - blockIdx.x : blockIdx.x;
   const int wave = __builtin_amdgcn_readfirstlane(threadIdx.x >> 6), lane = threadIdx.x & 63;
   const int c0 = wave * 4;
   float wk[4][9], sc[4], sh[4], mu[4], is[4];
@@ -1869,7 +1870,8 @@
   const int tiles_x = (W + 63) / 64, tiles_y = (H + HB_R - 1) / HB_R;
   const int T = N * tiles_x * tiles_y;
   const size_t HW = (size_t)H * W;
-  for (int tile = blockIdx.x; tile < T; tile += gridDim.x) {
+  const int G = gridDim.x, tile_last = wg + ((T - 1 - wg) / G) * G;
+  for (int tile = rev ? tile_last : wg; rev ? tile >= 0 : tile < T; tile += rev ? -G : G) {
     const int n = tile / (tiles_x * tiles_y), tt = tile - n * tiles_x * tiles_y;
     const int y0 = (tt / tiles_x) * HB_R, x0 = (tt % tiles_x) * 64;
     __syncthreads();
@@ -1928,19 +1930,19 @@
 #pragma unroll
     for (int t = 0; t < 9; ++t) {
       const float v = wave_sum(prod[j][t]);
-      if (lane == 0) rows[(size_t)blockIdx.x * HB_ROW + (c0 + j) * 9 + t] = v;
+      if (lane == 0) rows[(size_t)wg * HB_ROW + (c0 + j) * 9 + t] = v;
     }
   if (wave == 0) {
     bsum = wave_sum(bsum);
-    if (lane == 0) rows[(size_t)blockIdx.x * HB_ROW + CIN * 9] = bsum;
+    if (lane == 0) rows[(size_t)wg * HB_ROW + CIN * 9] = bsum;
   }
   if (BNS) {
 #pragma unroll
     for (int j = 0; j < 4; ++j) {
       const float s1 = wave_sum(b1[j]), s2 = wave_sum(b2[j]);
       if (lane == 0) {
-        bn_sums[((size_t)blockIdx.x * CIN + c0 + j) * 2] = (double)s1;
-        bn_sums[((size_t)blockIdx.x * CIN + c0 + j) * 2 + 1] = (double)s2;
+        bn_sums[((size_t)wg * CIN + c0 + j) * 2] = (double)s1;
+        bn_sums[((size_t)wg * CIN + c0 + j) * 2 + 1] = (double)s2;
       }
     }
     if (bn_absmax) {
@@ -2149,6 +2151,12 @@
 extern "C" int sc_head_conv_bwd(const float* dlogits, const sc_src* in, const float* w, float* gin, float* part, size_t part_floats,
                                 float* dw, float* dbias, int N, int Cin, int H, int W, double* bn_sums, float* bn_absmax,
                                 sc_stream stream) {
+  return sc_head_conv_bwd_dir(dlogits, in, w, gin, part, part_floats, dw, dbias, N, Cin, H, W, bn_sums, bn_absmax, 0, stream);
+}
+
+extern "C" int sc_head_conv_bwd_dir(const float* dlogits, const sc_src* in, const float* w, float* gin, float* part, size_t part_floats,
+                                    float* dw, float* dbias, int N, int Cin, int H, int W, double* bn_sums, float* bn_absmax,
+                                    int rev, sc_stream stream) {
   SC_REQUIRE(dlogits && in && w && gin && part && dw && in->C == Cin, "sc_head_conv_bwd: bad argument");
   SC_REQUIRE(Cin == 16, "sc_head_conv_bwd: Cin must be 16 (use sc_head_conv_dgrad + sc_head_conv_wgrad otherwise)");
   SC_REQUIRE((in->mode == SC_SRC_RAW || in->mode == SC_SRC_AFFINE) && in->up == 0, "sc_head_conv_bwd: unsupported source mode");
@@ -2158,8 +2166,8 @@
   const long T = (long)N * ((W + 63) / 64) * ((H + HB_R - 1) / HB_R);
   const int nwg = (int)(T < HB_MAXWG ? T : HB_MAXWG);
   SC_REQUIRE(!bn_sums || in->mode == SC_SRC_AFFINE, "sc_head_conv_bwd: the fused BatchNorm-backward sums need the AFFINE source of that BatchNorm");
-  if (bn_sums) hipLaunchKernelGGL(k_head_bwd16<true>, dim3(nwg), dim3(256), 0, st, dlogits, to_srcd(*in), w, gin, part, N, H, W, bn_sums, bn_absmax);
-  else hipLaunchKernelGGL(k_head_bwd16<false>, dim3(nwg), dim3(256), 0, st, dlogits, to_srcd(*in), w, gin, part, N, H, W, (double*)nullptr, (float*)nullptr);
+  if (bn_sums) hipLaunchKernelGGL(k_head_bwd16<true>, dim3(nwg), dim3(256), 0, st, dlogits, to_srcd(*in), w, gin, part, N, H, W, bn_sums, bn_absmax, rev ? 1 : 0);
+  else hipLaunchKernelGGL(k_head_bwd16<false>, dim3(nwg), dim3(256), 0, st, dlogits, to_srcd(*in), w, gin, part, N, H, W, (double*)nullptr, (float*)nullptr, rev ? 1 : 0);
   SC_LAUNCH_OK("sc_head_conv_bwd");
   hipLaunchKernelGGL(k_head_bwd_reduce, dim3(HB_ROW), dim3(256), 0, st, part, nwg, dw, dbias);
   SC_LAUNCH_OK("sc_head_conv_bwd(reduce)");
@@ -2252,13 +2260,18 @@
 
 extern "C" int sc_head_conv_fwd(const sc_src* in, const float* w, const float* bias, float* out, int N, int Cin,
                                 int H, int W, sc_stream stream) {
+  return sc_head_conv_fwd_dir(in, w, bias, out, N, Cin, H, W, 0, stream);
+}
+
+extern "C" int sc_head_conv_fwd_dir(const sc_src* in, const float* w, const float* bias, float* out, int N, int Cin,
+                                    int H, int W, int rev, sc_stream stream) {
   SC_REQUIRE(in && in->C == Cin, "sc_head_conv_fwd: source channels != Cin");
   SC_REQUIRE(Cin >= 1 && Cin <= HEAD_MAXCI, "sc_head_conv_fwd: Cin must be in [1,%d]", HEAD_MAXCI);
   SC_REQUIRE((in->mode == SC_SRC_RAW || in->mode == SC_SRC_AFFINE) && in->up == 0, "sc_head_conv_fwd: unsupported source mode");
   dim3 grid(((W + HT_C - 1) / HT_C) * ((H + HT_R - 1) / HT_R), 1, N);
   dim3 g16(((W + 63) / 64) * ((H + 15) / 16), 1, N);
   switch (sc_head_fwd_kernel(Cin, W, ((uintptr_t)in->x & 15) == 0, ((uintptr_t)out & 15) == 0)) {
-    case SC_HEAD_K_FWD16V: hipLaunchKernelGGL(k_head_fwd16v, g16, dim3(256), 0, (hipStream_t)stream, to_srcd(*in), w, bias, out, H, W); break;
+    case SC_HEAD_K_FWD16V: hipLaunchKernelGGL(k_head_fwd16v, g16, dim3(256), 0, (hipStream_t)stream, to_srcd(*in), w, bias, out, H, W, rev ? 1 : 0); break;
     case SC_HEAD_K_FWD16: hipLaunchKernelGGL(k_head_fwd16, g16, dim3(256), 0, (hipStream_t)stream, to_srcd(*in), w, bias, out, H, W); break;
     default: hipLaunchKernelGGL((k_head_fwd<0>), grid, dim3(256), 0, (hipStream_t)stream, to_srcd(*in), w, bias, out, Cin, H, W); break;
   }
diff --git a/starcop_amd/csrc/elementwise.hip b/starcop_amd/csrc/elementwise.hip
--- a/starcop_amd/csrc/elementwise.hip
+++ b/starcop_amd/csrc/elementwise.hip
@@ -147,15 +147,16 @@
 
 __global__ __launch_bounds__(256) void k_bn_bwd_reduce(const float* __restrict__ g, const float* __restrict__ y,
                                                        const float* __restrict__ cst, int act, double* __restrict__ sums, int C, int HW,
-                                                       float* __restrict__ absmax, float* __restrict__ act_absmax) {
+                                                       float* __restrict__ absmax, float* __restrict__ act_absmax, int rev) {
   __shared__ double s_tmp[8];
   __shared__ float s_m[4];
-  const int c = blockIdx.y, n = blockIdx.z;
+  const int bx = rev ? gridDim.x - 1 - blockIdx.x : blockIdx.x;
+  const int c = rev ? gridDim.y - 1 - blockIdx.y : blockIdx.y, n = rev ? gridDim.z - 1 - blockIdx.z : blockIdx.z;
   const float scale = cst[(size_t)c * SC_CST], shift = cst[(size_t)c * SC_CST + 1];
   const float mean = cst[(size_t)c * SC_CST + 2], invstd = cst[(size_t)c * SC_CST + 3];
   const float lo = sc_act_lo(act), hi = sc_act_hi(act);
   const size_t base = ((size_t)n * C + c) * HW;
-  const int start = blockIdx.x * 4096;
+  const int start = bx * 4096;
   const int end = min(start + 4096, HW);
   float s1 = 0.f, s2 = 0.f, mx = 0.f, ax = 0.f;
   if ((HW & 3) == 0) {
@@ -186,7 +187,7 @@
   }
   double v[2] = {(double)s1, (double)s2};
   block_sum_d<2>(v, s_tmp);
-  if (threadIdx.x < 2) sums[(stat_row() * C + c) * 2 + threadIdx.x] = v[threadIdx.x];
+  if (threadIdx.x < 2) sums[(((size_t)n * gridDim.x + bx) * C + c) * 2 + threadIdx.x] = v[threadIdx.x];
   if (absmax) block_absmax_to(mx, scale, absmax, s_m);
   if (act_absmax) {
     __syncthreads();
@@ -625,13 +626,19 @@
   return SC_OK;
 }
 
+extern "C" int sc_bn_bwd_reduce_dir(const float* g, const float* y, const float* cst_fwd, int act, double* sums, int N, int C,
+                                    int HW, float* absmax, float* act_absmax, int rev, sc_stream stream) {
+  SC_REQUIRE(g && y && cst_fwd && sums && N > 0 && C > 0 && HW > 0, "sc_bn_bwd_reduce: bad argument");
+  dim3 grid((HW + 4095) / 4096, C, N);
+  hipLaunchKernelGGL(k_bn_bwd_reduce, grid, dim3(256), 0, (hipStream_t)stream, g, y, cst_fwd, act, sums, C, HW, absmax, act_absmax,
+                     rev ? 1 : 0);
+  SC_LAUNCH_OK("sc_bn_bwd_reduce");
+  return SC_OK;
+}
+
 extern "C" int sc_bn_bwd_reduce(const float* g, const float* y, const float* cst_fwd, int act, double* sums, int N, int C,
                                 int HW, float* absmax, float* act_absmax, sc_stream stream) {
-  SC_REQUIRE(g && y && cst_fwd && sums && N > 0 && C > 0 && HW > 0, "sc_bn_bwd_reduce: bad argument");
-  dim3 grid((HW + 4095) / 4096, C, N);
-  hipLaunchKernelGGL(k_bn_bwd_reduce, grid, dim3(256), 0, (hipStream_t)stream, g, y, cst_fwd, act, sums, C, HW, absmax, act_absmax);
-  SC_LAUNCH_OK("sc_bn_bwd_reduce");
-  return SC_OK;
+  return sc_bn_bwd_reduce_dir(g, y, cst_fwd, act, sums, N, C, HW, absmax, act_absmax, 0, stream);
 }
 
 extern "C" int sc_bn_bwd_small(const float* g, const float* y, const float* cst_fwd, int act, int N, int C, int HW,
diff --git a/starcop_amd/network.py b/starcop_amd/network.py
--- a/starcop_amd/network.py
+++ b/starcop_amd/network.py
@@ -765,6 +765,8 @@
         plan = self._get_plan(N, H, W, need_grad, want_logits=head == "logits", want_classes=head == "classes")
         plan.buf["x"] = x
         plan.x_cst = x_cst
+        if getattr(plan, "dirs_key", None) != self.direction_min_bytes:
+            plan.dirs, plan.dirs_key = self.direction_plan(N, H, W), self.direction_min_bytes
         plan.generation = getattr(plan, "generation", 0) + 1
         self._pack_all(need_grad)
         st = stream()
@@ -897,7 +899,8 @@
                     fconv = lib.sc_conv1x1_ksplit
                 else:
                     fconv = lib.sc_conv2d_mfma
-                check(fconv(C.byref(a), st))
+                fdir = self._dir_entry(lib, fconv) if plan.dirs["fwd"].get(i) else None
+                check(fdir(C.byref(a), 1, st) if fdir is not None else fconv(C.byref(a), st))
             elif ty == "add":
                 sa = self._src_of(plan, op["ins"][0])
                 sb = self._src_of(plan, op["ins"][1])
@@ -920,8 +923,8 @@
                         mosaic.fill_bits, mosaic.nodata, mosaic.win, mosaic.win_host,
                         N, conv.in_channels, Ho, Wo, st))
                 elif self.classes == 1 and head == "logits":
-                    check(lib.sc_head_conv_fwd(C.byref(s), ptr(conv.weight), ptr(conv.bias), ptr(plan.buf[o.name]),
-                                               N, conv.in_channels, Ho, Wo, st))
+                    check(lib.sc_head_conv_fwd_dir(C.byref(s), ptr(conv.weight), ptr(conv.bias), ptr(plan.buf[o.name]),
+                                                   N, conv.in_channels, Ho, Wo, plan.dirs["fwd"].get(i, 0), st))
                 else:
                     check(lib.sc_head_conv_fwd_k(C.byref(s), ptr(conv.weight), ptr(conv.bias),
                                                  ptr(plan.buf[o.name]) if head == "logits" else None,
@@ -1029,6 +1032,53 @@
     _side_stream = None
     _late_pack_stream = None
 
+    direction_min_bytes = 128 << 20
+
+    def direction_plan(self, N, H, W):
+        def nbytes(t):
+            return 4 * N * t.C * (H >> t.shift) * (W >> t.shift)
+
+        def big(t):
+            return nbytes(t) >= self.direction_min_bytes
+        last = {}
+        fwd, red, head_bwd = {}, {}, 0
+        for i, op in enumerate(self._ops):
+            r = 0
+            if op["type"] in ("conv3", "head"):
+                t = max(op["ins"], key=nbytes)
+                if big(t):
+                    r = 1 - last.get(t.name, 0)
+            if r:
+                fwd[i] = 1
+            for t in op["ins"] + [op["out"]]:
+                last[t.name] = r
+        for op in reversed(self._ops):
+            o = op["out"]
+            if op["type"] == "head":
+                tin = op["ins"][0]
+                head_bwd = 1 - last.get(tin.name, 0) if big(tin) else 0
+                last[tin.name] = last["g:" + tin.name] = head_bwd
+                if tin.bn is not None and tin.kind == "raw" and self._n_cons.get(tin.name, 0) == 1:
+                    last["sums:" + tin.name] = 1
+                continue
+            if op["type"] == "add":
+                last["g:" + op["ins"][1].name] = last.get("g:" + o.name, 0)
+                continue
+            if o.bn is not None and not last.get("sums:" + o.name):
+                if big(o) and not last.get("g:" + o.name, 0):
+                    red[o.name] = 1
+            last["g:" + o.name] = last[o.name] = 0
+            for t in op["ins"]:
+                last["g:" + t.name] = 0
+        return {"fwd": fwd, "head_bwd": head_bwd, "reduce": red}
+
+    @staticmethod
+    def _dir_entry(lib, fn):
+        for name in ("sc_conv3x3_sp", "sc_conv3x3_thin16", "sc_conv3x3_bx3", "sc_conv3x3_sp_dgrad"):
+            if fn is getattr(lib, name):
+                return getattr(lib, name + "_dir")
+        return None
+
     def _backward_impl(self, plan, dlogits, on_tail_ready=None, only_ops=None, exchange_follows=None):
         lib = _lib.load()
         st = stream()
@@ -1079,8 +1129,8 @@
                 check(lib.sc_bn_bwd_small(ptr(plan.grad[t.name]), ptr(plan.buf[t.name]), ptr(plan.cst[t.name]), t.act, N, t.C,
                                           Ho * Wo, ptr(gv(t.bn.weight)), ptr(gv(t.bn.bias)), ptr(plan.cstb[t.name]), amax, aact, st))
                 return
-            check(lib.sc_bn_bwd_reduce(ptr(plan.grad[t.name]), ptr(plan.buf[t.name]), ptr(plan.cst[t.name]), t.act,
-                                       ptr(plan.bsums_v[t.name]), N, t.C, Ho * Wo, amax, aact, st))
+            check(lib.sc_bn_bwd_reduce_dir(ptr(plan.grad[t.name]), ptr(plan.buf[t.name]), ptr(plan.cst[t.name]), t.act,
+                                           ptr(plan.bsums_v[t.name]), N, t.C, Ho * Wo, amax, aact, plan.dirs["reduce"].get(t.name, 0), st))
             check(lib.sc_bn_bwd_finalize(ptr(plan.bsums_v[t.name]), plan.brows[t.name], float(N * Ho * Wo), ptr(plan.cst[t.name]),
                                          ptr(gv(t.bn.weight)), ptr(gv(t.bn.bias)), ptr(plan.cstb[t.name]), t.C, st))
 
@@ -1153,9 +1203,9 @@
                     if half_bwd:
                         bna = plan.gmax.data_ptr() + 4 * prod_idx[tin.name]
                     reduced.add(tin.name)
-                check(lib.sc_head_conv_bwd(ptr(dlogits), C.byref(s), ptr(conv.weight), ptr(plan.grad[tin.name]), ptr(plan.ws),
-                                           plan.ws_floats, ptr(gv(conv.weight)), ptr(gv(conv.bias)), N, conv.in_channels, Ho, Wo,
-                                           bns, bna, st))
+                check(lib.sc_head_conv_bwd_dir(ptr(dlogits), C.byref(s), ptr(conv.weight), ptr(plan.grad[tin.name]), ptr(plan.ws),
+                                               plan.ws_floats, ptr(gv(conv.weight)), ptr(gv(conv.bias)), N, conv.in_channels, Ho, Wo,
+                                               bns, bna, plan.dirs["head_bwd"], st))
                 self._pe(tok)
                 written.add(tin.name)
                 continue
```
